# jac0626/Neighbor-Aware-Reinforcement-Learning-Fosters-Cooperation-in-Spatial-Public-Goods-Games-

Hardware: NVIDIA B200
Metric: site-updates/s (higher is better)
Workload: dtype f32

## Files before the change

### neighbor-aware-reinforcement-learning-fosters-cooperation-in-spatial-public-goods-games-_b200/csrc/spgg_capi.cu

```cuda
#include "../../include/spgg.h"
#include "spgg_kernels.cuh"
#include "spgg_dispatch.h"
#include "spgg_fast.cuh"
#include "spgg_resident.cuh"

#include <cudaTypedefs.h>

#include <algorithm>
#include <cmath>
#include <cstdarg>
#include <cstdio>
#include <cstdlib>
#include <cstring>
#include <string>
#include <vector>

using namespace spgg;

static thread_local std::string g_err;

static int fail(int code, const char *fmt, ...) {
  char buf[512];
  va_list ap;
  va_start(ap, fmt);
  vsnprintf(buf, sizeof(buf), fmt, ap);
  va_end(ap);
  g_err = buf;
  return code;
}

#define CUDA_TRY(expr)                                                                  \
  do {                                                                                  \
    cudaError_t e_ = (expr);                                                            \
    if (e_ != cudaSuccess)                                                              \
      return fail(SPGG_E_CUDA, "%s failed: %s (%s:%d)", #expr, cudaGetErrorString(e_),  \
                  __FILE__, __LINE__);                                                  \
  } while (0)


struct spgg_handle {
  int device = 0;
  int n_rep = 1;
  int mode = MODE_F32_I8;
  int M = 1;
  int action = 0;
  std::vector<spgg_params_t> params;
  std::vector<RepConst> rc_host;
  Geom g{};
  int threads = 256;
  int gmax_ctas = 1;
  size_t smem_step = 0, smem_gmax = 0;
  RepConst *d_rc = nullptr;
  double *d_valtab = nullptr;
  bool lean = false;
  int gmax_ctas_gen = 1;
  void *d_Qb[2] = {nullptr, nullptr};
  int qcur = 0;
  void *Qcur() const { return d_Qb[qcur]; }
  bool spec = false;
  bool carry_valid = false;
  float *d_gcarry = nullptr;
  int *d_bad = nullptr;
  CUtensorMap qmaps[2];
  bool spec_on = true;
  long long spec_launches = 0, spec_failures = 0;
  long long spec_iterations = 0;
  bool in_rerun = false;
  float *d_gvec = nullptr;
  void *peer_code[2][2] = {{nullptr, nullptr}, {nullptr, nullptr}};
  void *peer_R[2][2] = {{nullptr, nullptr}, {nullptr, nullptr}};
  uint32_t *peer_S[2][2] = {{nullptr, nullptr}, {nullptr, nullptr}};
  int peer_rows[2] = {0, 0};
  bool peer_on = false;
  std::vector<void *> ipc_opened;
  unsigned *d_ring = nullptr;
  unsigned *ring_peer[SPGG_MAX_RING] = {nullptr};
  int ring_world = 0;
  int gen = 0;
  int last_gen = -1;
  int last_rel = -1, last_upd = 0, last_spec = 0, last_sel = 0;
  int pend_qcur0 = 0;
  std::vector<char> pend_cur_after, pend_q_after;
  void *d_R[2] = {nullptr, nullptr};
  void *d_code[2] = {nullptr, nullptr};
  uint32_t *d_S[2] = {nullptr, nullptr};
  int cur = 0;
  void *d_gmax = nullptr;
  double *d_stats = nullptr;
  double *d_partials = nullptr;
  unsigned *d_tickets = nullptr;
  int *d_stop = nullptr;
  double *d_eps = nullptr;
  uint32_t *d_thr = nullptr;
  int cap = 0;
  double *d_u = nullptr;
  uint8_t *d_b = nullptr;
  uint8_t *d_sc_S = nullptr;
  double *d_sc_R = nullptr, *d_sc_Q = nullptr;
  unsigned long long *d_sc_info = nullptr;
  bool fast = false;
  bool r_wide = false;
  FastMaps fmaps[2];
  bool resident = false;
  ResGeom rgeo{};
  size_t smem_res = 0;
  bool pend_resident = false;
  bool res_grid = false;
  unsigned char *d_gimg = nullptr;
  double *d_gpart = nullptr;
  unsigned *d_gnsel = nullptr;
  int gnsel_cap = 0;
  std::vector<double> eps_host;
  std::vector<uint32_t> thr_host;
  int replay_pairs = 1;
  long long replay_first = 0, replay_n = 0;
  long long iter = 0;
  std::vector<double> eps_cur;
  std::vector<long long> stop_at;
  std::vector<char> stale;
  long long launches = 0;
  bool pending = false;
  long long pend_t0 = 0;
  int pend_n = 0, pend_cur0 = 0, pend_rel = 0;
  cudaStream_t pend_stream = nullptr;
  CclScratch ccl;
  bool ccl_valid = false;
  int64_t ccl_n = 0;
  size_t elem_code() const { return mode == MODE_F64 ? 4 : 1; }
  size_t elem_R() const { return mode == MODE_F64 ? 8 : (mode == MODE_F32_F ? 4 : 1); }
  size_t elem_Q() const { return mode == MODE_F64 ? 8 : 4; }
  size_t elem_val() const { return mode == MODE_F64 ? 8 : 4; }
  int nq() const { return params[0].algorithm == SPGG_ALGO_DOUBLE_QLEARNING ? 8 : 4; }
};

static bool int8_quantum(const spgg_params_t &p, double *rq, int *gi, int *li, int *mn, int *mx) {
  for (int k = 0; k <= 4; ++k) {
    const double s = (double)(1 << k);
    const double a = p.rep_gain_C * s, b = p.delta_R_D * s, c = p.R_min * s, d = p.R_max * s;
    if (a == std::floor(a) && b == std::floor(b) && c == std::floor(c) && d == std::floor(d) &&
        std::fabs(c) <= 127 && std::fabs(d) <= 127 && std::fabs(a) <= 127 && std::fabs(b) <= 127 &&
        c - b >= -128 && d + a <= 127) {
      *rq = 1.0 / s; *gi = (int)a; *li = (int)b; *mn = (int)c; *mx = (int)d;
      return true;
    }
  }
  return false;
}

static void build_repconst(const spgg_params_t &p, RepConst *rc) {
  memset(rc, 0, sizeof(*rc));
  rc->rc = p.r * p.c;
  for (int n = 0; n < 6; ++n) rc->g[n] = rc->rc * (double)n / 5.0;
  rc->cost = p.cost;
  rc->lo = p.r - 5.0;
  rc->span = 4.0 * p.r - rc->lo;
  rc->wP = p.wP;
  rc->wR = 1.0 - p.wP;
  rc->alpha = p.alpha; rc->gamma = p.gamma; rc->kappa = p.kappa; rc->leps = p.lambda_eps;
  rc->gainC = p.rep_gain_C; rc->lossD = p.delta_R_D; rc->rmin = p.R_min; rc->rmax = p.R_max;
  rc->alpha_f = (float)p.alpha; rc->gamma_f = (float)p.gamma; rc->kappa_f = (float)p.kappa;
  rc->leps_f = (float)p.lambda_eps;
  rc->gainC_f = (float)p.rep_gain_C; rc->lossD_f = (float)p.delta_R_D;
  rc->rmin_f = (float)p.R_min; rc->rmax_f = (float)p.R_max;
  rc->rq = 1.0;
  int8_quantum(p, &rc->rq, &rc->gain_i, &rc->loss_i, &rc->rmin_i, &rc->rmax_i);
  rc->seed_lo = (uint32_t)p.seed;
  rc->seed_hi = (uint32_t)(p.seed >> 32);
  for (uint32_t r = 0; r < 10; ++r) {
    rc->pkeys[2 * r] = rc->seed_lo + r * 0x9E3779B9u;
    rc->pkeys[2 * r + 1] = rc->seed_hi + r * 0xBB67AE85u;
  }
  rc->has_ratio = (rc->wR != 0.0);
  for (int code = 0; code < 128; ++code) {
    const int sn = code >> 2, C = (code >> 1) & 1, coop = code & 1;
    const double tot = rc->rc * (double)sn / 5.0 - (C ? 5.0 * p.cost : 0.0);
    const double P = (tot - rc->lo) / rc->span;
    const double rew = rc->wP * P + rc->wR * (coop ? 0.5 : 0.0);
    rc->rewtab[code] = (float)rew;
    rc->ratiotab[code] =
        coop ? (float)(std::fabs(rc->wR * 0.5) / (std::fabs(rew) + 1e-9) * 100.0) : 0.0f;
  }
}

static size_t step_smem(int mode, int TR) {
  switch (mode) {
    case MODE_F32_I8: return SmemLayout<ModeF32I8>(TR).total;
    case MODE_F32_F: return SmemLayout<ModeF32F>(TR).total;
    default: return SmemLayout<ModeF64>(TR).total;
  }
}

template <class... KArgsT, class... Args>
static cudaError_t launch_pdl(void (*kern)(KArgsT...), int grid, int block, size_t smem, cudaStream_t st,
                              Args... args) {
  static const bool use_pdl = getenv("SPGG_NO_PDL") == nullptr;
  cudaLaunchConfig_t cfg = {};
  cfg.gridDim = dim3((unsigned)grid);
  cfg.blockDim = dim3((unsigned)block);
  cfg.dynamicSmemBytes = smem;
  cfg.stream = st;
  cudaLaunchAttribute attr[1];
  attr[0].id = cudaLaunchAttributeProgrammaticStreamSerialization;
  attr[0].val.programmaticStreamSerializationAllowed = 1;
  cfg.attrs = attr;
  cfg.numAttrs = use_pdl ? 1 : 0;
  return cudaLaunchKernelEx(&cfg, kern, args...);
}

typedef void (*fast_fn_t)(const FastMaps, KArgs);
template <int M, bool ACTION, bool PART>
static fast_fn_t pick_fast3(int upd, int sel) {
  if (upd) return sel ? k_step_fast<M, ACTION, true, true, PART> : k_step_fast<M, ACTION, true, false, PART>;
  return k_step_fast<M, ACTION, false, true, PART>;
}
template <int M, bool ACTION>
static fast_fn_t pick_fast2(int upd, int sel, bool part) {
  return part ? pick_fast3<M, ACTION, true>(upd, sel) : pick_fast3<M, ACTION, false>(upd, sel);
}
static fast_fn_t pick_fast(int M, int action, int upd, int sel, bool part) {
  if (M == 2) return action ? pick_fast2<2, true>(upd, sel, part) : pick_fast2<2, false>(upd, sel, part);
  return action ? pick_fast2<1, true>(upd, sel, part) : pick_fast2<1, false>(upd, sel, part);
}
static size_t fast_smem(int M) { return M == 2 ? FastSmem<2>::kTotal : FastSmem<1>::kTotal; }
typedef void (*gfast_fn_t)(const CUtensorMap, GArgs);
static gfast_fn_t pick_gfast(int M) { return M == 2 ? k_gmax_fast<2> : k_gmax_fast<1>; }
static size_t gfast_smem(int M) { return M == 2 ? GmaxSmem<2>::kTotal : GmaxSmem<1>::kTotal; }

typedef void (*res_fn_t)(RArgs);
template <bool FULL>
static res_fn_t pick_res2(int M, int action) {
  if (M == 2) return action ? k_resident<2, true, FULL> : k_resident<2, false, FULL>;
  return action ? k_resident<1, true, FULL> : k_resident<1, false, FULL>;
}
static res_fn_t pick_res(int M, int action, int L) {
  return (L % 4 == 0) ? pick_res2<true>(M, action) : pick_res2<false>(M, action);
}
template <bool FULL>
static res_fn_t pick_resg2(int M, int action) {
  if (M == 2) return action ? k_resident<2, true, FULL, true> : k_resident<2, false, FULL, true>;
  return action ? k_resident<1, true, FULL, true> : k_resident<1, false, FULL, true>;
}
static res_fn_t pick_res_grid(int M, int action, int L) {
  return (L % 4 == 0) ? pick_resg2<true>(M, action) : pick_resg2<false>(M, action);
}
static ResGeom resident_geom(int L, int cs, size_t smem_limit, int grid = 0) {
  ResGeom rg{};
  rg.grid = grid;
  if (L < 2 * cs) cs = 1;
  rg.rows_max = (L + cs - 1) / cs;
  rg.prow = rg.rows_max + 4;
  rg.QR = (L + 3) / 4;
  rg.pitch = (RG + rg.QR * 4 + RG + 15) / 16 * 16;
  const int quads = rg.rows_max * rg.QR;
  int max_thr = RES_THREADS;
  if (const char *e = getenv("SPGG_RES_THREADS")) max_thr = std::max(64, std::min(RES_THREADS, atoi(e) / 32 * 32));
  rg.threads = std::max(64, std::min(max_thr, (quads + 31) / 32 * 32));
  rg.CS = (ResSmem(rg).total <= smem_limit) ? cs : 0;
  return rg;
}

static int make_map(CUtensorMap *map, void *base, uint64_t row_bytes, uint64_t n_rows, uint64_t n_rep,
                    uint64_t rep_stride_bytes, uint32_t box_bytes, uint32_t box_rows, uint64_t visible_bytes = 0) {
  static PFN_cuTensorMapEncodeTiled_v12000 encode = nullptr;
  if (!encode) {
    void *fn = nullptr;
    cudaDriverEntryPointQueryResult q;
    CUDA_TRY(cudaGetDriverEntryPoint("cuTensorMapEncodeTiled", &fn, cudaEnableDefault, &q));
    if (!fn || q != cudaDriverEntryPointSuccess) return fail(SPGG_E_CUDA, "cuTensorMapEncodeTiled not available");
    encode = (PFN_cuTensorMapEncodeTiled_v12000)fn;
  }
  const cuuint64_t dims[3] = {visible_bytes ? visible_bytes : row_bytes, n_rows, n_rep};
  const cuuint64_t strides[2] = {row_bytes, rep_stride_bytes};
  const cuuint32_t box[3] = {box_bytes, box_rows, 1};
  const cuuint32_t estr[3] = {1, 1, 1};
  CUresult r = encode(map, CU_TENSOR_MAP_DATA_TYPE_UINT8, 3, base, dims, strides, box, estr,
                      CU_TENSOR_MAP_INTERLEAVE_NONE, CU_TENSOR_MAP_SWIZZLE_NONE,
                      CU_TENSOR_MAP_L2_PROMOTION_L2_128B, CU_TENSOR_MAP_FLOAT_OOB_FILL_NONE);
  if (r != CUDA_SUCCESS) return fail(SPGG_E_CUDA, "cuTensorMapEncodeTiled failed (%d)", (int)r);
  return SPGG_OK;
}

static int make_map_q(CUtensorMap *map, void *base, uint64_t L, uint64_t n_rows, uint64_t n_rep) {
  static PFN_cuTensorMapEncodeTiled_v12000 encode = nullptr;
  if (!encode) {
    void *fn = nullptr;
    cudaDriverEntryPointQueryResult q;
    CUDA_TRY(cudaGetDriverEntryPoint("cuTensorMapEncodeTiled", &fn, cudaEnableDefault, &q));
    if (!fn || q != cudaDriverEntryPointSuccess) return fail(SPGG_E_CUDA, "cuTensorMapEncodeTiled not available");
    encode = (PFN_cuTensorMapEncodeTiled_v12000)fn;
  }
  const cuuint64_t dims[4] = {128, L / 8, n_rows, n_rep};
  const cuuint64_t strides[3] = {128, L * 16, n_rows * L * 16};
  const cuuint32_t box[4] = {128, TC / 8, (cuuint32_t)FastSmem<1>::kRowsPerWarp, 1};
  const cuuint32_t estr[4] = {1, 1, 1, 1};
  CUresult r = encode(map, CU_TENSOR_MAP_DATA_TYPE_UINT8, 4, base, dims, strides, box, estr,
                      CU_TENSOR_MAP_INTERLEAVE_NONE, CU_TENSOR_MAP_SWIZZLE_128B,
                      CU_TENSOR_MAP_L2_PROMOTION_L2_128B, CU_TENSOR_MAP_FLOAT_OOB_FILL_NONE);
  if (r != CUDA_SUCCESS) return fail(SPGG_E_CUDA, "cuTensorMapEncodeTiled (Q) failed (%d)", (int)r);
  return SPGG_OK;
}

extern "C" int spgg_abi_version(void) { return SPGG_ABI_VERSION; }
extern "C" const char *spgg_last_error(void) { return g_err.c_str(); }

static int free_all(spgg_handle *h) {
  for (void *p : h->ipc_opened) cudaIpcCloseMemHandle(p);
  h->ipc_opened.clear();
  cudaFree(h->d_rc); cudaFree(h->d_valtab); cudaFree(h->d_Qb[0]); cudaFree(h->d_Qb[1]); cudaFree(h->d_gcarry); cudaFree(h->d_bad); cudaFree(h->d_gvec); cudaFree(h->d_ring);
  for (int i = 0; i < 2; ++i) { cudaFree(h->d_R[i]); cudaFree(h->d_code[i]); cudaFree(h->d_S[i]); }
  cudaFree(h->d_gmax); cudaFree(h->d_stats); cudaFree(h->d_partials); cudaFree(h->d_tickets);
  cudaFree(h->d_stop); cudaFree(h->d_eps); cudaFree(h->d_thr); cudaFree(h->d_u); cudaFree(h->d_b);
  cudaFree(h->d_sc_S); cudaFree(h->d_sc_R); cudaFree(h->d_sc_Q); cudaFree(h->d_sc_info);
  cudaFree(h->d_gimg); cudaFree(h->d_gpart); cudaFree(h->d_gnsel);
  ccl_free(&h->ccl);
  return 0;
}

extern "C" void spgg_destroy(spgg_t *h) {
  if (!h) return;
  cudaSetDevice(h->device);
  cudaDeviceSynchronize();
  free_all(h);
  delete h;
}

extern "C" int spgg_create(const spgg_params_t *params, int n_replicas, int device, spgg_t **out) {
  if (!params || !out || n_replicas < 1) return fail(SPGG_E_INVALID, "spgg_create: null argument or n_replicas < 1");
  const spgg_params_t &p0 = params[0];
  if (p0.L < 4) return fail(SPGG_E_INVALID, "L must be >= 4 (got %d)", p0.L);
  if (p0.rows < 2 * GH || p0.rows > p0.L)
    return fail(SPGG_E_INVALID, "rows must be in [%d, L] (got %d)", 2 * GH, p0.rows);
  if (p0.M != 1 && p0.M != 2) return fail(SPGG_E_INVALID, "M must be 1 or 2 (got %d)", p0.M);
  if (p0.state_mode != SPGG_STATE_REPUTATION && p0.state_mode != SPGG_STATE_ACTION)
    return fail(SPGG_E_INVALID, "Unknown state_representation code %d", p0.state_mode);
  if (p0.precision != SPGG_PREC_FP32 && p0.precision != SPGG_PREC_FP64)
    return fail(SPGG_E_INVALID, "unknown precision %d", p0.precision);
  if (p0.algorithm != SPGG_ALGO_QLEARNING && p0.algorithm != SPGG_ALGO_SARSA &&
      p0.algorithm != SPGG_ALGO_EXPECTED_SARSA && p0.algorithm != SPGG_ALGO_DOUBLE_QLEARNING)
    return fail(SPGG_E_UNSUPPORTED, "algorithm code %d is not built into the fused kernel", p0.algorithm);
  if (p0.row0 < 0 || p0.row0 + p0.rows > p0.L) return fail(SPGG_E_INVALID, "row0/rows outside the lattice");
  for (int r = 1; r < n_replicas; ++r) {
    const spgg_params_t &p = params[r];
    if (p.L != p0.L || p.rows != p0.rows || p.row0 != p0.row0 || p.M != p0.M ||
        p.state_mode != p0.state_mode || p.precision != p0.precision ||
        p.algorithm != p0.algorithm || p.r_storage != p0.r_storage)
      return fail(SPGG_E_INVALID, "replica %d differs in a batch-invariant field (L, rows, M, state, precision)", r);
  }
  int ndev = 0;
  CUDA_TRY(cudaGetDeviceCount(&ndev));
  if (device < 0 || device >= ndev) return fail(SPGG_E_CUDA, "device %d not available (%d devices)", device, ndev);
  CUDA_TRY(cudaSetDevice(device));

  spgg_handle *h = new spgg_handle();
  h->device = device;
  h->n_rep = n_replicas;
  h->params.assign(params, params + n_replicas);
  h->M = p0.M;
  h->action = p0.state_mode == SPGG_STATE_ACTION;
  h->rc_host.resize(n_replicas);
  bool all_i8 = true;
  for (int r = 0; r < n_replicas; ++r) {
    build_repconst(params[r], &h->rc_host[r]);
    double rq; int a, b, c, d;
    all_i8 = all_i8 && int8_quantum(params[r], &rq, &a, &b, &c, &d);
  }
  if (p0.precision == SPGG_PREC_FP64) h->mode = MODE_F64;
  else if (p0.r_storage == SPGG_RSTORE_FP32) h->mode = MODE_F32_F;
  else if (p0.r_storage == SPGG_RSTORE_INT8) {
    if (!all_i8) { delete h; return fail(SPGG_E_INVALID, "reputation parameters are not representable in int8 units"); }
    h->mode = MODE_F32_I8;
  } else h->mode = all_i8 ? MODE_F32_I8 : MODE_F32_F;

  Geom &g = h->g;
  g.L = p0.L; g.rows = p0.rows; g.row0 = p0.row0; g.wrap_rows = (p0.rows == p0.L);
  g.pitchB = CPAD + (p0.L + 15) / 16 * 16 + CPAD;
  g.pitchW = WPAD + ((p0.L + 31) / 32 + 3) / 4 * 4 + WPAD;
  {
    const RepConst &r0 = h->rc_host[0];
    bool ok = (h->mode == MODE_F32_I8) && (g.L % 32 == 0) && (g.L >= TC) && (g.rows % FTR == 0) &&
              p0.algorithm == SPGG_ALGO_QLEARNING && getenv("SPGG_NO_FAST") == nullptr;
    for (int r = 0; r < n_replicas && ok; ++r)
      ok = h->rc_host[r].rmin_i >= -15 && h->rc_host[r].rmax_i <= 15 && h->rc_host[r].gain_i >= 0 &&
           h->rc_host[r].loss_i >= 0;
    (void)r0;
    h->fast = ok;
  }
  {
    cudaDeviceProp prop0;
    CUDA_TRY(cudaGetDeviceProperties(&prop0, device));
    res_fn_t rf = pick_res(h->M, h->action, h->g.L);
    cudaFuncAttributes fa;
    CUDA_TRY(cudaFuncGetAttributes(&fa, rf));
    const size_t lim = prop0.sharedMemPerBlockOptin - fa.sharedSizeBytes - 1024;
    const bool eligible = (h->mode == MODE_F32_I8) && g.wrap_rows && p0.row0 == 0 &&
                          p0.algorithm == SPGG_ALGO_QLEARNING && getenv("SPGG_NO_RESIDENT") == nullptr;
    ResGeom rg = resident_geom(g.L, 8, lim);
    if (eligible && g.L >= 32 && (rg.CS == 0 || n_replicas <= 4 || getenv("SPGG_RES_CS16") != nullptr) &&
        getenv("SPGG_RES_CS8") == nullptr) {
      const ResGeom rg16 = resident_geom(g.L, 16, lim);
      if (rg16.CS == 16 &&
          cudaFuncSetAttribute(rf, cudaFuncAttributeNonPortableClusterSizeAllowed, 1) == cudaSuccess &&
          cudaFuncSetAttribute(rf, cudaFuncAttributeMaxDynamicSharedMemorySize, (int)lim) == cudaSuccess) {
        cudaLaunchConfig_t cfg = {};
        cfg.gridDim = dim3(16u * (unsigned)n_replicas);
        cfg.blockDim = dim3((unsigned)rg16.threads);
        cfg.dynamicSmemBytes = ResSmem(rg16).total;
        cudaLaunchAttribute attr[1];
        attr[0].id = cudaLaunchAttributeClusterDimension;
        attr[0].val.clusterDim.x = 16; attr[0].val.clusterDim.y = 1; attr[0].val.clusterDim.z = 1;
        cfg.attrs = attr; cfg.numAttrs = 1;
        int n_clusters = 0;
        if (cudaOccupancyMaxActiveClusters(&n_clusters, rf, &cfg) == cudaSuccess && n_clusters >= 1) rg = rg16;
      }
      (void)cudaGetLastError();
    }
    h->resident = eligible && rg.CS > 0;
    if (h->resident) {
      h->rgeo = rg;
      h->smem_res = ResSmem(rg).total;
      CUDA_TRY(cudaFuncSetAttribute(rf, cudaFuncAttributeMaxDynamicSharedMemorySize, (int)lim));
    } else if (eligible && n_replicas == 1 && getenv("SPGG_NO_RESIDENT_GRID") == nullptr) {
      res_fn_t gf = pick_res_grid(h->M, h->action, h->g.L);
      cudaFuncAttributes gfa;
      CUDA_TRY(cudaFuncGetAttributes(&gfa, gf));
      const size_t glim = prop0.sharedMemPerBlockOptin - gfa.sharedSizeBytes - 1024;
      int coop = 0;
      CUDA_TRY(cudaDeviceGetAttribute(&coop, cudaDevAttrCooperativeLaunch, device));
      const int nb_ctas = std::min(prop0.multiProcessorCount, g.L / 2);
      ResGeom gg = resident_geom(g.L, nb_ctas, glim, 1);
      if (coop && nb_ctas >= RES_RING && gg.CS == nb_ctas &&
          cudaFuncSetAttribute(gf, cudaFuncAttributeMaxDynamicSharedMemorySize, (int)glim) == cudaSuccess) {
        int occ_g = 0;
        if (cudaOccupancyMaxActiveBlocksPerMultiprocessor(&occ_g, gf, gg.threads, ResSmem(gg).total) == cudaSuccess &&
            (long long)occ_g * prop0.multiProcessorCount >= nb_ctas) {
          h->resident = true;
          h->res_grid = true;
          h->rgeo = gg;
          h->smem_res = ResSmem(gg).total;
        }
      }
      (void)cudaGetLastError();
    }
  }
  g.TR = h->fast ? FTR : (g.rows >= 512 ? 16 : (g.rows >= 64 ? 8 : 4));
  h->threads = h->fast ? FTHREADS : 32 * std::min(8, g.TR);
  if (!h->fast && getenv("SPGG_GEN_TR") && getenv("SPGG_GEN_THREADS")) {
    g.TR = std::max(4, std::min(16, atoi(getenv("SPGG_GEN_TR"))));
    h->threads = std::max(32, std::min(256, atoi(getenv("SPGG_GEN_THREADS")) / 32 * 32));
  }
  g.n_tx = (g.L + TC - 1) / TC;
  g.n_ty = (g.rows + g.TR - 1) / g.TR;
  g.n_rep = n_replicas;
  g.plane_stride = (long long)(g.rows + 2 * GH) * g.pitchB;
  g.bits_stride = (long long)(g.rows + 2 * GH) * g.pitchW;
  g.site_stride = (long long)g.rows * g.L;
  h->smem_step = step_smem(h->mode, g.TR);
  h->smem_gmax = (h->elem_val() * (size_t)(g.TR + 2 * HR) * SMW + 15) / 16 * 16 + 512;

  cudaDeviceProp prop;
  CUDA_TRY(cudaGetDeviceProperties(&prop, device));
  int occ = 1;
  h->lean = !h->fast && p0.algorithm == 0 && getenv("SPGG_NO_LEAN") == nullptr;
  if (h->lean) h->smem_step = step_smem(h->mode, LEAN_TR_MAX);
  for (int replay = 0; replay < 2; ++replay) {
    step_fn_t f = pick_step(h->mode, h->M, h->action, replay);
    CUDA_TRY(cudaFuncSetAttribute(f, cudaFuncAttributeMaxDynamicSharedMemorySize, (int)h->smem_step));
    if (!replay)
      CUDA_TRY(cudaOccupancyMaxActiveBlocksPerMultiprocessor(&occ, f, h->threads, h->smem_step));
    if (h->lean) {
      step_fn_t fl = pick_lean(h->mode, h->M, h->action, replay);
      CUDA_TRY(cudaFuncSetAttribute(fl, cudaFuncAttributeMaxDynamicSharedMemorySize, (int)h->smem_step));
      if (!replay)
        CUDA_TRY(cudaOccupancyMaxActiveBlocksPerMultiprocessor(&occ, fl, h->threads, h->smem_step));
    }
  }
  if (h->fast) {
    for (int v = 0; v < 3; ++v) {
      fast_fn_t fv = pick_fast(h->M, h->action, v != 2, v != 1, g.L % TC != 0);
      CUDA_TRY(cudaFuncSetAttribute(fv, cudaFuncAttributeMaxDynamicSharedMemorySize, (int)fast_smem(h->M)));
    }
    fast_fn_t ff = pick_fast(h->M, h->action, 1, 1, g.L % TC != 0);
    CUDA_TRY(cudaOccupancyMaxActiveBlocksPerMultiprocessor(&occ, ff, FTHREADS, fast_smem(h->M)));
    CUDA_TRY(cudaFuncSetAttribute(pick_gfast(h->M), cudaFuncAttributeMaxDynamicSharedMemorySize, (int)gfast_smem(h->M)));
    int gocc = 1;
    CUDA_TRY(cudaOccupancyMaxActiveBlocksPerMultiprocessor(&gocc, pick_gfast(h->M), GWARPS * 32, gfast_smem(h->M)));
    const long long n_tiles_g = (long long)((p0.L + TC - 1) / TC) * (p0.rows / FTR);
    h->gmax_ctas = (int)std::max<long long>(1, std::min<long long>((n_tiles_g + GWARPS - 1) / GWARPS,
                       ((long long)prop.multiProcessorCount * std::max(1, gocc)) / n_replicas));
  }
  CUDA_TRY(cudaFuncSetAttribute(pick_gmax_lean(h->mode, h->M), cudaFuncAttributeMaxDynamicSharedMemorySize,
                                (int)h->smem_gmax));
  if (occ < 1) { delete h; return fail(SPGG_E_CUDA, "kernel does not fit on an SM (smem %zu)", h->smem_step); }
  const long long n_tiles = (long long)g.n_tx * g.n_ty;
  long long per_rep = std::max<long long>(1, ((long long)prop.multiProcessorCount * occ) / n_replicas);
  g.ctas_per_rep = (int)std::min<long long>(n_tiles, per_rep);
  {
    int gocc = 1;
    CUDA_TRY(cudaOccupancyMaxActiveBlocksPerMultiprocessor(&gocc, pick_gmax_lean(h->mode, h->M), h->threads, h->smem_gmax));
    h->gmax_ctas_gen = (int)std::min<long long>(n_tiles, std::max<long long>(1, ((long long)prop.multiProcessorCount * std::max(1, gocc)) / n_replicas));
  }
  if (h->fast && (g.site_stride / ((long long)g.ctas_per_rep * FTHREADS)) > 60000) h->fast = false;
  h->spec = h->fast && getenv("SPGG_NO_SPEC") == nullptr;

  const size_t nQ = (size_t)n_replicas * g.site_stride * h->nq() * h->elem_Q();
  const size_t nR = (size_t)n_replicas * g.plane_stride * h->elem_R();
  const size_t nC = (size_t)n_replicas * g.plane_stride * h->elem_code();
  const size_t nS = (size_t)n_replicas * g.bits_stride * 4;
#define ALLOC(ptr, bytes)                                                                   \
  do {                                                                                      \
    cudaError_t e_ = cudaMalloc((void **)&(ptr), (bytes));                                  \
    if (e_ != cudaSuccess) {                                                                \
      free_all(h); delete h;                                                                \
      return fail(SPGG_E_CUDA, "cudaMalloc(%zu bytes) failed: %s", (size_t)(bytes), cudaGetErrorString(e_)); \
    }                                                                                       \
    cudaMemset((ptr), 0, (bytes));                                                          \
  } while (0)
  ALLOC(h->d_rc, sizeof(RepConst) * n_replicas);
  ALLOC(h->d_Qb[0], nQ);
  if (h->spec) { ALLOC(h->d_Qb[1], nQ); ALLOC(h->d_gcarry, sizeof(float) * n_replicas); ALLOC(h->d_bad, sizeof(int)); }
  for (int i = 0; i < 2; ++i) { ALLOC(h->d_R[i], nR); ALLOC(h->d_code[i], nC); ALLOC(h->d_S[i], nS); }
  ALLOC(h->d_partials, sizeof(double) * (size_t)n_replicas * g.ctas_per_rep * NSTAT);
  ALLOC(h->d_tickets, sizeof(unsigned) * n_replicas);
  ALLOC(h->d_stop, sizeof(int) * n_replicas);
  if (h->res_grid) {
    ALLOC(h->d_gimg, (size_t)h->rgeo.CS * 6 * h->rgeo.prow * h->rgeo.pitch);
    ALLOC(h->d_gpart, sizeof(double) * (size_t)RES_RING * h->rgeo.CS * RES_NRED);
  }
#undef ALLOC
  if (h->fast) {
    const int rowsCR = FTR + 2 * h->M, rowsS = FTR + 4;
    const uint64_t nrows = (uint64_t)(g.rows + 2 * GH);
    for (int i = 0; i < 2; ++i) {
      FastMaps &fm = h->fmaps[i];
      int e = make_map(&fm.ld_code, h->d_code[i], (uint64_t)g.pitchB, nrows, n_replicas, (uint64_t)g.plane_stride, FROWB, rowsCR);
      if (!e) e = make_map(&fm.ld_R, h->d_R[i], (uint64_t)g.pitchB, nrows, n_replicas, (uint64_t)g.plane_stride, FROWB, rowsCR);
      if (!e) e = make_map(&fm.ld_S, h->d_S[i], (uint64_t)g.pitchW * 4, nrows, n_replicas, (uint64_t)g.bits_stride * 4, FSROWB, rowsS);
      if (!e) e = make_map(&fm.st_code, h->d_code[i ^ 1], (uint64_t)g.pitchB, nrows, n_replicas, (uint64_t)g.plane_stride, TC, FTR, (uint64_t)(CPAD + g.L));
      if (!e) e = make_map(&fm.st_R, h->d_R[i ^ 1], (uint64_t)g.pitchB, nrows, n_replicas, (uint64_t)g.plane_stride, TC, FTR, (uint64_t)(CPAD + g.L));
      if (!e) e = make_map(&fm.st_S, h->d_S[i ^ 1], (uint64_t)g.pitchW * 4, nrows, n_replicas, (uint64_t)g.bits_stride * 4, TC / 8, FTR);
      if (!e) e = make_map_q(&h->qmaps[i], h->d_Qb[(i == 1 && h->spec) ? 1 : 0], (uint64_t)g.L, (uint64_t)g.rows, (uint64_t)n_replicas);
      if (e) { free_all(h); delete h; return e; }
    }
  }
  CUDA_TRY(cudaMemcpy(h->d_rc, h->rc_host.data(), sizeof(RepConst) * n_replicas, cudaMemcpyHostToDevice));
  if (h->mode == MODE_F64) {
    const size_t vb = sizeof(double) * 2 * ((size_t)n_replicas << VALTAB_BITS);
    if (cudaMalloc((void **)&h->d_valtab, vb) != cudaSuccess) {
      free_all(h); delete h;
      return fail(SPGG_E_CUDA, "cudaMalloc(%zu bytes) failed (reward table)", vb);
    }
    CUDA_TRY(launch_build_valtab(h->d_rc, h->d_valtab, n_replicas));
  }
  std::vector<int> neg(n_replicas, -1);
  CUDA_TRY(cudaMemcpy(h->d_stop, neg.data(), sizeof(int) * n_replicas, cudaMemcpyHostToDevice));
  if (h->spec) {
    const int none = 0x7fffffff;
    CUDA_TRY(cudaMemcpy(h->d_bad, &none, sizeof(int), cudaMemcpyHostToDevice));
  }
  h->eps_cur.resize(n_replicas);
  for (int r = 0; r < n_replicas; ++r) h->eps_cur[r] = params[r].epsilon;
  h->stop_at.assign(n_replicas, -1);
  h->stale.assign(n_replicas, 0);
  *out = h;
  return SPGG_OK;
}

static int launch_step(spgg_handle *h, int do_update, int do_select, cudaStream_t st, bool allow_spec);

static int rewind_to_failed_launch(spgg_handle *h, int bad) {
  h->spec_failures += 1;
  if (h->spec_failures > 8 && h->spec_failures * 16 > h->spec_iterations) h->spec_on = false;
  const int none = 0x7fffffff;
  CUDA_TRY(cudaMemcpy(h->d_bad, &none, sizeof(int), cudaMemcpyHostToDevice));
  std::vector<int> stop(h->n_rep);
  CUDA_TRY(cudaMemcpy(stop.data(), h->d_stop, sizeof(int) * h->n_rep, cudaMemcpyDeviceToHost));
  for (int r = 0; r < h->n_rep; ++r)
    if (stop[r] == (int)(h->pend_t0 + bad) + 1) stop[r] = -1;
  CUDA_TRY(cudaMemcpy(h->d_stop, stop.data(), sizeof(int) * h->n_rep, cudaMemcpyHostToDevice));
  h->cur = h->pend_cur_after[bad - 1];
  h->qcur = h->pend_q_after[bad - 1];
  h->carry_valid = true;
  h->pend_rel = bad - 1;
  return SPGG_OK;
}

static int rerun_failed_speculation(spgg_handle *h) {
  for (;;) {
    int bad = 0x7fffffff;
    CUDA_TRY(cudaMemcpy(&bad, h->d_bad, sizeof(int), cudaMemcpyDeviceToHost));
    if (bad == 0x7fffffff) return SPGG_OK;
    if (getenv("SPGG_SPEC_DEBUG")) fprintf(stderr, "[spgg] speculation failed at launch %d of %d (t0 %lld), %lld speculative launches so far\n", bad, h->pend_n, h->pend_t0, h->spec_launches);
    if (bad < 1 || bad > h->pend_n) return fail(SPGG_E_STATE, "speculation bookkeeping out of range (%d of %d)", bad, h->pend_n);
    int rcode0 = rewind_to_failed_launch(h, bad);
    if (rcode0) return rcode0;
    h->in_rerun = true;
    const int n = h->pend_n;
    for (int s = bad; s <= n; ++s) {
      h->pend_rel += 1;
      int rcode = launch_step(h, 1, s < n ? 1 : 0, h->pend_stream, true);
      if (rcode) return rcode;
      if (!h->spec_on && s < n) {
        for (++s; s <= n; ++s) {
          rcode = spgg_phase_gmax(h, h->pend_stream);
          if (!rcode) rcode = launch_step(h, 1, s < n ? 1 : 0, h->pend_stream, false);
          if (rcode) return rcode;
        }
      }
    }
    h->in_rerun = false;
    CUDA_TRY(cudaStreamSynchronize(h->pend_stream));
    CUDA_TRY(cudaGetLastError());
  }
}

static int finish_pending(spgg_handle *h) {
  if (!h->pending) return SPGG_OK;
  CUDA_TRY(cudaSetDevice(h->device));
  CUDA_TRY(cudaStreamSynchronize(h->pend_stream));
  CUDA_TRY(cudaGetLastError());
  if (h->spec && h->g.wrap_rows && h->pend_rel == h->pend_n && !h->pend_resident) {
    int rcode = rerun_failed_speculation(h);
    if (rcode) return rcode;
  }
  std::vector<int> stop(h->n_rep);
  CUDA_TRY(cudaMemcpy(stop.data(), h->d_stop, sizeof(int) * h->n_rep, cudaMemcpyDeviceToHost));
  const long long t_end = h->pend_t0 + h->pend_rel;
  for (int r = 0; r < h->n_rep; ++r) {
    h->stop_at[r] = stop[r];
    const long long done = (stop[r] >= 0 && stop[r] < t_end) ? (long long)stop[r] : t_end;
    double e = h->eps_cur[r];
    for (long long t = h->pend_t0; t < done; ++t)
      e = std::max(e * h->params[r].epsilon_decay, h->params[r].epsilon_min);
    h->eps_cur[r] = e;
  }
  if (h->pend_resident) {
    h->iter = (h->n_rep == 1 && stop[0] >= 0 && stop[0] < t_end) ? (long long)stop[0] : t_end;
    h->pend_resident = false;
  } else if (h->n_rep == 1 && stop[0] >= 0 && stop[0] < t_end) {
    h->cur = h->pend_cur0 ^ (int)((stop[0] - h->pend_t0) & 1);
    h->qcur = h->pend_q_after[(size_t)(stop[0] - h->pend_t0)];
    h->iter = stop[0];
  } else {
    if (h->n_rep > 1) {
      for (int r = 0; r < h->n_rep; ++r) {
        if (stop[r] >= 0 && stop[r] < t_end) {
          const long long k = (long long)stop[r] - h->pend_t0;
          const int src = k >= 0 ? (h->pend_cur0 ^ (int)(k & 1)) : h->pend_cur0;
          if (src != h->cur) {
            const Geom &g = h->g;
            CUDA_TRY(cudaMemcpy((char *)h->d_R[h->cur] + (size_t)r * g.plane_stride * h->elem_R(),
                                (char *)h->d_R[src] + (size_t)r * g.plane_stride * h->elem_R(),
                                (size_t)g.plane_stride * h->elem_R(), cudaMemcpyDeviceToDevice));
            CUDA_TRY(cudaMemcpy(h->d_S[h->cur] + (size_t)r * g.bits_stride,
                                h->d_S[src] + (size_t)r * g.bits_stride,
                                (size_t)g.bits_stride * 4, cudaMemcpyDeviceToDevice));
          }
          const int qsrc = k >= 0 ? h->pend_q_after[(size_t)k] : h->pend_qcur0;
          if (qsrc != h->qcur) {
            const size_t qb = (size_t)h->g.site_stride * h->nq() * h->elem_Q();
            CUDA_TRY(cudaMemcpy((char *)h->d_Qb[h->qcur] + (size_t)r * qb, (char *)h->d_Qb[qsrc] + (size_t)r * qb, qb,
                                cudaMemcpyDeviceToDevice));
          }
        }
      }
    }
    h->iter = t_end;
  }
  h->pending = false;
  return SPGG_OK;
}

extern "C" int spgg_sync(spgg_t *h) {
  if (!h) return fail(SPGG_E_INVALID, "null handle");
  return finish_pending(h);
}

static int stage_rows(const spgg_handle *h) {
  const long long budget = 32ll << 20;
  return (int)std::max<long long>(1, std::min<long long>(h->g.rows, budget / h->g.L));
}

static int ensure_scratch(spgg_handle *h, bool want_q) {
  const size_t n = (size_t)stage_rows(h) * h->g.L;
  if (!h->d_sc_S) {
    CUDA_TRY(cudaMalloc((void **)&h->d_sc_S, n));
    CUDA_TRY(cudaMalloc((void **)&h->d_sc_R, n * sizeof(double)));
    CUDA_TRY(cudaMalloc((void **)&h->d_sc_info, 3 * sizeof(unsigned long long)));
  }
  if (want_q && !h->d_sc_Q) CUDA_TRY(cudaMalloc((void **)&h->d_sc_Q, n * h->nq() * sizeof(double)));
  return SPGG_OK;
}

static void begin_new_run(spgg_handle *h, int rep) {
  if (h->iter != 0) {
    h->iter = 0;
    std::fill(h->stale.begin(), h->stale.end(), 1);
  }
  h->stale[rep] = 0;
  h->carry_valid = false;
  if (h->d_ring) {
    cudaMemset(h->d_ring, 0, sizeof(unsigned) * RING_SLOTS * RING_WORDS);
    h->gen = 0;
    h->last_gen = -1;
  }
}

extern "C" int spgg_set_state(spgg_t *h, int rep, const uint8_t *S, const double *R, const double *Q) {
  if (!h || !S || !R || !Q) return fail(SPGG_E_INVALID, "spgg_set_state: null argument");
  if (rep < 0 || rep >= h->n_rep) return fail(SPGG_E_INVALID, "replica %d out of range", rep);
  int rcode = finish_pending(h);
  if (rcode) return rcode;
  h->ccl_valid = false;
  CUDA_TRY(cudaSetDevice(h->device));
  rcode = ensure_scratch(h, true);
  if (rcode) return rcode;
  const Geom &g = h->g;
  const RepConst &rc = h->rc_host[rep];
  CUDA_TRY(cudaMemset(h->d_sc_info, 0, 3 * sizeof(unsigned long long)));
  const int chunk = stage_rows(h);
  for (int i0 = 0; i0 < g.rows; i0 += chunk) {
    const int nr = std::min(chunk, g.rows - i0);
    const size_t n = (size_t)nr * g.L, off = (size_t)i0 * g.L;
    CUDA_TRY(cudaMemcpyAsync(h->d_sc_S, S + off, n, cudaMemcpyHostToDevice, 0));
    CUDA_TRY(cudaMemcpyAsync(h->d_sc_R, R + off, n * sizeof(double), cudaMemcpyHostToDevice, 0));
    CUDA_TRY(cudaMemcpyAsync(h->d_sc_Q, Q + off * h->nq(), n * h->nq() * sizeof(double), cudaMemcpyHostToDevice, 0));
    const int grid = (int)std::min<long long>(148 * 16, ((long long)nr * ((g.L + 31) / 32) * 32 + 255) / 256);
#define IMPORT(Md) k_import_rows<Md><<<std::max(1, grid), 256>>>(g, rep, i0, nr, h->d_sc_S, h->d_sc_R, h->d_sc_Q, \
                       h->Qcur(), h->d_R[h->cur], h->d_S[h->cur], rc.rq, h->d_sc_info, h->nq())
    if (h->mode == MODE_F32_I8) IMPORT(ModeF32I8);
    else if (h->mode == MODE_F32_F) IMPORT(ModeF32F);
    else IMPORT(ModeF64);
#undef IMPORT
    CUDA_TRY(cudaGetLastError());
    h->launches += 1;
  }
  unsigned long long info[3];
  CUDA_TRY(cudaMemcpy(info, h->d_sc_info, sizeof(info), cudaMemcpyDeviceToHost));
  if (info[0] == 1) return fail(SPGG_E_INVALID, "strategy array holds values other than 0/1");
  if (info[0] == 2)
    return fail(SPGG_E_INVALID, "R is not representable in int8 units of %g; use r_storage=FP32", rc.rq);
  if (info[2] && h->fast) {
    if (!g.wrap_rows)
      return fail(SPGG_E_INVALID, "R outside [%g, %g] (int8 units -16..15 of %g): a strip on the fast path "
                  "cannot hold it", -16.0 * rc.rq, 15.0 * rc.rq, rc.rq);
    h->r_wide = true;
  }
  begin_new_run(h, rep);
  h->eps_cur[rep] = h->params[rep].epsilon;
  int stop = -1;
  if (g.wrap_rows && (info[1] == 0 || info[1] == (unsigned long long)g.site_stride))
    stop = (int)h->iter;
  h->stop_at[rep] = stop;
  CUDA_TRY(cudaMemcpy(h->d_stop + rep, &stop, sizeof(int), cudaMemcpyHostToDevice));
  return SPGG_OK;
}

extern "C" int spgg_get_state(spgg_t *h, int rep, uint8_t *S, double *R, double *Q) {
  if (!h) return fail(SPGG_E_INVALID, "null handle");
  if (rep < 0 || rep >= h->n_rep) return fail(SPGG_E_INVALID, "replica %d out of range", rep);
  int rcode = finish_pending(h);
  if (rcode) return rcode;
  CUDA_TRY(cudaSetDevice(h->device));
  rcode = ensure_scratch(h, Q != nullptr);
  if (rcode) return rcode;
  const Geom &g = h->g;
  const RepConst &rc = h->rc_host[rep];
  const int chunk = stage_rows(h);
  for (int i0 = 0; i0 < g.rows; i0 += chunk) {
    const int nr = std::min(chunk, g.rows - i0);
    const size_t n = (size_t)nr * g.L, off = (size_t)i0 * g.L;
    const int grid = (int)std::min<long long>(148 * 16, ((long long)n + 255) / 256);
#define EXPORT(Md) k_export_rows<Md><<<std::max(1, grid), 256>>>(g, rep, i0, nr, S ? h->d_sc_S : nullptr, \
                       R ? h->d_sc_R : nullptr, Q ? h->d_sc_Q : nullptr, h->Qcur(), h->d_R[h->cur], h->d_S[h->cur], rc.rq, h->nq())
    if (h->mode == MODE_F32_I8) EXPORT(ModeF32I8);
    else if (h->mode == MODE_F32_F) EXPORT(ModeF32F);
    else EXPORT(ModeF64);
#undef EXPORT
    CUDA_TRY(cudaGetLastError());
    h->launches += 1;
    if (S) CUDA_TRY(cudaMemcpyAsync(S + off, h->d_sc_S, n, cudaMemcpyDeviceToHost, 0));
    if (R) CUDA_TRY(cudaMemcpyAsync(R + off, h->d_sc_R, n * sizeof(double), cudaMemcpyDeviceToHost, 0));
    if (Q) CUDA_TRY(cudaMemcpyAsync(Q + off * h->nq(), h->d_sc_Q, n * h->nq() * sizeof(double), cudaMemcpyDeviceToHost, 0));
    CUDA_TRY(cudaStreamSynchronize(0));
  }
  return SPGG_OK;
}

extern "C" int spgg_set_replay(spgg_t *h, int n_steps, const double *u, const uint8_t *b) {
  return spgg_set_replay_pairs(h, n_steps, 1, u, b);
}

extern "C" int spgg_set_replay_pairs(spgg_t *h, int n_steps, int n_pairs, const double *u, const uint8_t *b) {
  if (!h) return fail(SPGG_E_INVALID, "null handle");
  const int want_pairs = h->params[0].algorithm == SPGG_ALGO_SARSA ? 3
                         : (h->params[0].algorithm == SPGG_ALGO_DOUBLE_QLEARNING ? 2 : 1);
  if (n_steps > 0 && n_pairs != want_pairs)
    return fail(SPGG_E_INVALID, "this TD rule consumes %d draw pair(s) per iteration, got %d", want_pairs, n_pairs);
  if (h->n_rep != 1) return fail(SPGG_E_UNSUPPORTED, "replay draws are supported for a single replica");
  int rcode = finish_pending(h);
  if (rcode) return rcode;
  CUDA_TRY(cudaSetDevice(h->device));
  cudaFree(h->d_u); cudaFree(h->d_b);
  h->d_u = nullptr; h->d_b = nullptr; h->replay_n = 0;
  if (n_steps <= 0) return SPGG_OK;
  if (!u || !b) return fail(SPGG_E_INVALID, "spgg_set_replay: null draw arrays");
  const size_t n = (size_t)n_steps * n_pairs * h->g.site_stride;
  h->replay_pairs = n_pairs;
  CUDA_TRY(cudaMalloc((void **)&h->d_u, n * sizeof(double)));
  CUDA_TRY(cudaMalloc((void **)&h->d_b, n));
  CUDA_TRY(cudaMemcpy(h->d_u, u, n * sizeof(double), cudaMemcpyHostToDevice));
  CUDA_TRY(cudaMemcpy(h->d_b, b, n, cudaMemcpyHostToDevice));
  h->replay_first = h->iter;
// ... 711 lines not shown
```

### neighbor-aware-reinforcement-learning-fosters-cooperation-in-spatial-public-goods-games-_b200/csrc/spgg_fast.cuh

```cuda
#pragma once
#include <cuda.h>

#include "spgg_kernels.cuh"

namespace spgg {

#ifndef SPGG_FTR
#define SPGG_FTR 16
#endif
#ifndef SPGG_FTHREADS
#define SPGG_FTHREADS 256
#endif
constexpr int FTR = SPGG_FTR;
constexpr int FROWB = 160;
constexpr int FROWW = FROWB / 4;
constexpr int FSROWB = 48;
constexpr int FTHREADS = SPGG_FTHREADS;

template <int M>
struct FastSmem {
  static constexpr int kRowsCR = FTR + 2 * M;
  static constexpr int kRowsS = FTR + 4;
  static constexpr int kStageCode = 0;
  static constexpr int kStageR = (kRowsCR * FROWB + 127) / 128 * 128;
  static constexpr int kStageS = kStageR + (kRowsCR * FROWB + 127) / 128 * 128;
  static constexpr int kStageBytes = kStageS + (kRowsS * FSROWB + 127) / 128 * 128;
  static constexpr int kTxBytes = 2 * kRowsCR * FROWB + kRowsS * FSROWB;
  static constexpr int kOutCode = 2 * kStageBytes;
  static constexpr int kOutR = kOutCode + FTR * TC;
  static constexpr int kOutS = kOutR + FTR * TC;
  static constexpr int kOffC = kOutS + 256 + FROWB;
  static constexpr int kOffVal = kOffC + (FTR + 4) * FROWB + FROWB;
  static constexpr int kOffTab = kOffVal + kRowsCR * FROWB * 4;
  static constexpr int kOffBar = kOffTab + 256 * 4;
  static constexpr int kOffFlag = kOffBar + 40 * 8;
  static constexpr int kOffRc = kOffFlag + 16;
  static constexpr int kOffRed = (kOffRc + (int)sizeof(RepConst) + 127) / 128 * 128;
  static constexpr int kRowsPerWarp = FTR / (FTHREADS / 32);
  static constexpr int kQBufs = 2;
  static constexpr int kQBufBytes = kRowsPerWarp * TC * 16;
  static constexpr int kOffQ = (kOffRed + 8 * NSTAT * 8 + 1023) / 1024 * 1024;
  static constexpr int kTotal = kOffQ + (FTHREADS / 32) * kQBufs * kQBufBytes + 1024;
};

__device__ __forceinline__ uint32_t smem_u32(const void *p) {
  return (uint32_t)__cvta_generic_to_shared(p);
}
__device__ __forceinline__ void mbar_init(uint64_t *bar, uint32_t count) {
  asm volatile("mbarrier.init.shared::cta.b64 [%0], %1;" ::"r"(smem_u32(bar)), "r"(count));
}
__device__ __forceinline__ void mbar_expect_tx(uint64_t *bar, uint32_t bytes) {
  asm volatile("mbarrier.arrive.expect_tx.shared::cta.b64 _, [%0], %1;" ::"r"(smem_u32(bar)), "r"(bytes)
               : "memory");
}
__device__ __forceinline__ void mbar_wait(uint64_t *bar, uint32_t parity) {
  uint32_t done;
  uint32_t spins = 0;
  do {
    asm volatile(
        "{\n"
        ".reg .pred p;\n"
        "mbarrier.try_wait.parity.shared::cta.b64 p, [%1], %2;\n"
        "selp.u32 %0, 1, 0, p;\n"
        "}\n"
        : "=r"(done)
        : "r"(smem_u32(bar)), "r"(parity)
        : "memory");
    if (!done && ++spins > (1u << 28)) __trap();
  } while (!done);
}
__device__ __forceinline__ void tma_load_3d(void *dst, const CUtensorMap *map, uint64_t *bar, int c0,
                                            int c1, int c2) {
  asm volatile(
      "cp.async.bulk.tensor.3d.shared::cluster.global.mbarrier::complete_tx::bytes [%0], [%1, {%3, %4, %5}], [%2];"
      ::"r"(smem_u32(dst)), "l"(map), "r"(smem_u32(bar)), "r"(c0), "r"(c1), "r"(c2)
      : "memory");
}

__device__ __forceinline__ void bulk_load_1d(void *dst, const void *src, uint32_t bytes, uint64_t *bar) {
  asm volatile(
      "cp.async.bulk.shared::cluster.global.mbarrier::complete_tx::bytes [%0], [%1], %2, [%3];"
      ::"r"(smem_u32(dst)), "l"(src), "r"(bytes), "r"(smem_u32(bar))
      : "memory");
}
__device__ __forceinline__ void tma_store_3d(const CUtensorMap *map, const void *src, int c0, int c1, int c2) {
  asm volatile("cp.async.bulk.tensor.3d.global.shared::cta.bulk_group [%0, {%2, %3, %4}], [%1];"
               ::"l"(map), "r"(smem_u32(src)), "r"(c0), "r"(c1), "r"(c2)
               : "memory");
}
__device__ __forceinline__ uint64_t l2_evict_first_policy() {
  uint64_t pol;
  asm volatile("createpolicy.fractional.L2::evict_first.b64 %0, 1.0;" : "=l"(pol));
  return pol;
}
__device__ __forceinline__ void tma_load_4d_hint(void *dst, const CUtensorMap *map, uint64_t *bar, int c0,
                                                 int c1, int c2, int c3, uint64_t pol) {
  asm volatile(
      "cp.async.bulk.tensor.4d.shared::cluster.global.mbarrier::complete_tx::bytes.L2::cache_hint"
      " [%0], [%1, {%3, %4, %5, %6}], [%2], %7;"
      ::"r"(smem_u32(dst)), "l"(map), "r"(smem_u32(bar)), "r"(c0), "r"(c1), "r"(c2), "r"(c3), "l"(pol)
      : "memory");
}
__device__ __forceinline__ void tma_store_4d_hint(const CUtensorMap *map, const void *src, int c0, int c1,
                                                  int c2, int c3, uint64_t pol) {
  asm volatile(
      "cp.async.bulk.tensor.4d.global.shared::cta.bulk_group.L2::cache_hint [%0, {%2, %3, %4, %5}], [%1], %6;"
      ::"l"(map), "r"(smem_u32(src)), "r"(c0), "r"(c1), "r"(c2), "r"(c3), "l"(pol)
      : "memory");
}
template <int N>
__device__ __forceinline__ void tma_store_wait_read_n() {
  asm volatile("cp.async.bulk.wait_group.read %0;" ::"n"(N) : "memory");
}
__device__ __forceinline__ void tma_store_commit() { asm volatile("cp.async.bulk.commit_group;" ::: "memory"); }
__device__ __forceinline__ void tma_store_wait_read() { asm volatile("cp.async.bulk.wait_group.read 0;" ::: "memory"); }
__device__ __forceinline__ void tma_store_wait_all() { asm volatile("cp.async.bulk.wait_group 0;" ::: "memory"); }
__device__ __forceinline__ void fence_proxy_async() { asm volatile("fence.proxy.async.shared::cta;" ::: "memory"); }

__device__ __forceinline__ uint32_t sh_l1(uint32_t prev, uint32_t cur) { return __byte_perm(prev, cur, 0x6543); }
__device__ __forceinline__ uint32_t sh_r1(uint32_t cur, uint32_t next) { return __byte_perm(cur, next, 0x4321); }
__device__ __forceinline__ uint32_t sh_2(uint32_t a, uint32_t b) { return __byte_perm(a, b, 0x5432); }

struct FastMaps {
  CUtensorMap ld_code, ld_R, ld_S;
  CUtensorMap st_code, st_R, st_S;
  CUtensorMap q_ld, q_st;
};

#ifndef SPGG_FAST_MINBLOCKS
#define SPGG_FAST_MINBLOCKS 2
#endif
template <int M, bool ACTION, bool UPD, bool SEL, bool PART = false>
__device__ __forceinline__ void step_fast_body(const FastMaps &tm, const KArgs &a) {
  typedef FastSmem<M> SM;
  constexpr int NK = (M == 2) ? 12 : 4;
  constexpr bool upd = UPD, sel = SEL;
  const Geom &g = a.g;
  const int rep = blockIdx.x / g.ctas_per_rep, cta = blockIdx.x % g.ctas_per_rep;

  extern __shared__ __align__(1024) unsigned char smem_fast[];
  unsigned char *smem = smem_fast + ((1024u - (smem_u32(smem_fast) & 1023u)) & 1023u);
  uint32_t *wC = reinterpret_cast<uint32_t *>(smem + SM::kOffC);
  float *sm_val = reinterpret_cast<float *>(smem + SM::kOffVal);
  float *sm_tab = reinterpret_cast<float *>(smem + SM::kOffTab);
  float *sm_ratio = sm_tab + 128;
  double *sm_red = reinterpret_cast<double *>(smem + SM::kOffRed);
  uint64_t *bars = reinterpret_cast<uint64_t *>(smem + SM::kOffBar);
  uint8_t *out_code = smem + SM::kOutCode;
  int8_t *out_R = reinterpret_cast<int8_t *>(smem + SM::kOutR);
  uint32_t *out_S = reinterpret_cast<uint32_t *>(smem + SM::kOutS);
  RepConst &s_rc = *reinterpret_cast<RepConst *>(smem + SM::kOffRc);
  int &s_is_last = *reinterpret_cast<int *>(smem + SM::kOffFlag);

  const int tid = threadIdx.x, lane = tid & 31, warp = tid >> 5;
#ifdef SPGG_TRACE
  unsigned long long t_start = 0;
  if (tid == 0) asm volatile("mov.u64 %0, %%globaltimer;" : "=l"(t_start));
#endif
  for (int i = tid; i < (int)(sizeof(RepConst) / 4); i += FTHREADS)
    reinterpret_cast<uint32_t *>(&s_rc)[i] = reinterpret_cast<const uint32_t *>(a.rc + rep)[i];
  if (tid == 0) {
    mbar_init(&bars[0], 1);
    mbar_init(&bars[1], 1);
    asm volatile("fence.mbarrier_init.release.cluster;" ::: "memory");
  }
  __syncthreads();
  for (int i = tid; i < 128; i += FTHREADS) {
    sm_tab[i] = s_rc.rewtab[i];
    sm_ratio[i] = s_rc.ratiotab[i];
  }
  const RepConst &rc = s_rc;

  float4 *Qp = reinterpret_cast<float4 *>(a.Q) + (long long)rep * g.site_stride;

  float inv_den = 0.f, gm_used = 0.f;
  if (upd) {
    gm_used = a.spec ? a.gcarry[rep] : reinterpret_cast<const float *>(a.gmax)[(long long)rep * a.cap + a.rel];
    if (a.spec == 2) gm_used = 123.0f;
    inv_den = __fdiv_rn(1.0f, __fadd_rn(gm_used, rc.leps_f));
  }
  float gbest = 0.f;
  const uint32_t thr = sel ? a.thr_tab[(long long)(a.rel + 1) * g.n_rep + rep] : 0u;
  const float alpha = rc.alpha_f, gamma = rc.gamma_f, kappa = rc.kappa_f;
  const int g31 = min(rc.gain_i, 31), l31 = min(rc.loss_i, 31);
  const uint32_t r_dsum = (uint32_t)(g31 + l31);
  const uint32_t r_k = (uint32_t)(32 - l31) * 0x01010101u;
  const uint32_t r_lo = (uint32_t)(rc.rmin_i + 48) * 0x01010101u, r_hi = (uint32_t)(rc.rmax_i + 48) * 0x01010101u;
  const bool has_ratio = rc.has_ratio != 0;

  uint32_t cls_n[4] = {0, 0, 0, 0}, cls_sn[4] = {0, 0, 0, 0};
  uint32_t grp[6] = {0, 0, 0, 0, 0, 0};
  uint32_t pk_best = 0;
  uint32_t n_sel = 0;
  int sum_r = 0;
  float sq0 = 0.f, sq1 = 0.f, sq2 = 0.f, sq3 = 0.f, sc0 = 0.f, sc1 = 0.f, sc2 = 0.f, sc3 = 0.f;
  float s_ni = 0.f, s_ratio = 0.f;

  const int n_tiles = g.n_tx * g.n_ty;
  const int d_ty = g.ctas_per_rep / g.n_tx, d_tx = g.ctas_per_rep - d_ty * g.n_tx;
  const int d_skew = (d_tx + d_ty) % g.n_tx;
  auto issue = [&](int ty_, int tx_, int st) {
    const int r0 = ty_ * FTR, c0 = tx_ * TC;
    unsigned char *base = smem + st * SM::kStageBytes;
    mbar_expect_tx(&bars[st], SM::kTxBytes);
    tma_load_3d(base + SM::kStageCode, &tm.ld_code, &bars[st], c0, r0 + GH - M, rep);
    tma_load_3d(base + SM::kStageR, &tm.ld_R, &bars[st], c0, r0 + GH - M, rep);
    tma_load_3d(base + SM::kStageS, &tm.ld_S, &bars[st], c0 >> 3, r0 + GH - 2, rep);
  };
  int ty = cta / g.n_tx, txs = cta - ty * g.n_tx;
  int tx = (txs + ty) % g.n_tx;
  if (tid == 0 && cta < n_tiles) issue(ty, tx, 0);

  uint64_t *qbar = bars + 2 + warp * SM::kQBufs;
  unsigned char *sQ = smem + SM::kOffQ + warp * (SM::kQBufs * SM::kQBufBytes);
  const uint64_t pol = l2_evict_first_policy();
  if (lane == 0) {
#pragma unroll
    for (int b = 0; b < SM::kQBufs; ++b) mbar_init(&qbar[b], 1);
    asm volatile("fence.mbarrier_init.release.cluster;" ::: "memory");
  }
  __syncwarp();
  auto q_issue = [&](int col8, int row, int buf) {
    mbar_expect_tx(&qbar[buf], SM::kQBufBytes);
    tma_load_4d_hint(sQ + buf * SM::kQBufBytes, &tm.q_ld, &qbar[buf], 0, col8, row, rep, pol);
  };
  int qoff[4];
#pragma unroll
  for (int k = 0; k < 4; ++k)
    qoff[k] = (lane >> 1) * 128 + ((((lane & 1) * 4 + k) ^ ((lane >> 1) & 7)) << 4);
  if (lane == 0 && cta < n_tiles) q_issue((tx * TC) >> 3, ty * FTR + warp * SM::kRowsPerWarp, 0);

  int tiles_done = 0, stage = 0;
  for (int tile = cta; tile < n_tiles; tile += g.ctas_per_rep, ++tiles_done, stage ^= 1) {
    const int r0 = ty * FTR, c0 = tx * TC;
    int nty = ty + d_ty, ntxs = txs + d_tx, ntx = tx + d_skew;
    if (ntxs >= g.n_tx) { ntxs -= g.n_tx; ++nty; ++ntx; }
    if (ntx >= g.n_tx) ntx -= g.n_tx;
    const bool has_next = tile + g.ctas_per_rep < n_tiles;
    if (tid == 0) {
      if (has_next) issue(nty, ntx, stage ^ 1);
      if (sel) tma_store_wait_read();
    }
    mbar_wait(&bars[stage], (uint32_t)(tiles_done >> 1) & 1u);
    const bool lv = !PART || (c0 + 4 * lane < g.L);
    const uint32_t vm = lv ? 0x01010101u : 0u;
    const unsigned char *st_base = smem + stage * SM::kStageBytes;
    const uint32_t *st_code = reinterpret_cast<const uint32_t *>(st_base + SM::kStageCode);
    const uint32_t *st_R = reinterpret_cast<const uint32_t *>(st_base + SM::kStageR);
    const uint32_t *st_S = reinterpret_cast<const uint32_t *>(st_base + SM::kStageS);

    const int t1 = tid - (FTHREADS - 128);
    if (t1 >= 0 && t1 < (FTR + 4) * 6) {
      const int row = t1 / 6, bw = t1 - row * 6 + 3;
      const uint32_t bits = ~st_S[row * (FSROWB / 4) + bw];
      uint32_t *dst = wC + row * FROWW + (bw - 4) * 8 + 4;
      if (bw == 3) {
        dst[7] = ((bits >> 28) * 0x00204081u) & 0x01010101u;
      } else if (bw == 8) {
        dst[0] = ((bits & 0xFu) * 0x00204081u) & 0x01010101u;
      } else {
        uint4 lo, hi;
        lo.x = (((bits >> 0) & 0xFu) * 0x00204081u) & 0x01010101u;
        lo.y = (((bits >> 4) & 0xFu) * 0x00204081u) & 0x01010101u;
        lo.z = (((bits >> 8) & 0xFu) * 0x00204081u) & 0x01010101u;
        lo.w = (((bits >> 12) & 0xFu) * 0x00204081u) & 0x01010101u;
        hi.x = (((bits >> 16) & 0xFu) * 0x00204081u) & 0x01010101u;
        hi.y = (((bits >> 20) & 0xFu) * 0x00204081u) & 0x01010101u;
        hi.z = (((bits >> 24) & 0xFu) * 0x00204081u) & 0x01010101u;
        hi.w = ((bits >> 28) * 0x00204081u) & 0x01010101u;
        *reinterpret_cast<uint4 *>(dst) = lo;
        *reinterpret_cast<uint4 *>(dst + 4) = hi;
      }
    }
    if (upd) {
      for (int e = tid; e < SM::kRowsCR * FROWW; e += FTHREADS) {
        const uint32_t cw = st_code[e];
        float4 v;
        v.x = sm_tab[(cw >> 1) & 0x7Fu];
        v.y = sm_tab[(cw >> 9) & 0x7Fu];
        v.z = sm_tab[(cw >> 17) & 0x7Fu];
        v.w = sm_tab[(cw >> 25) & 0x7Fu];
        *reinterpret_cast<float4 *>(sm_val + e * 4) = v;
      }
    }
    if (upd) {
      const int t2 = tid - 64;
      if (t2 >= 0 && t2 < FTR * 4 && (!PART || (c0 >> 5) + (t2 & 3) < ((g.L + 31) >> 5))) {
        const int row = (t2 >> 2) + 2, bw = (t2 & 3) + 4;
        const uint32_t *bp = st_S + row * (FSROWB / 4) + bw;
        const uint32_t c = bp[0], u = bp[-(FSROWB / 4)], d = bp[FSROWB / 4];
        const uint32_t l = (c << 1) | (bp[-1] >> 31), r = (c >> 1) | (bp[1] << 31);
        const uint32_t s1 = c ^ u ^ d, c1 = (c & u) | (d & (c | u));
        const uint32_t b0 = s1 ^ l ^ r, c2 = (s1 & l) | (r & (s1 | l));
        const uint32_t b1 = c1 ^ c2, b2 = c1 & c2;
        grp[0] += __popc(~b0 & ~b1 & ~b2); grp[1] += __popc(b0 & ~b1 & ~b2);
        grp[2] += __popc(~b0 & b1 & ~b2);  grp[3] += __popc(b0 & b1 & ~b2);
        grp[4] += __popc(~b0 & ~b1 & b2);  grp[5] += __popc(b0 & ~b1 & b2);
      }
    }
    __syncthreads();
    const uint8_t *bCode = reinterpret_cast<const uint8_t *>(st_code);
    const int qb = stage;
    __syncwarp();
    if (lane == 0) {
      if (upd) tma_store_wait_read_n<0>();
      if (has_next) q_issue((ntx * TC) >> 3, nty * FTR + warp * SM::kRowsPerWarp, qb ^ 1);
    }
    mbar_wait(&qbar[qb], (uint32_t)(tiles_done >> 1) & 1u);
#pragma unroll
    for (int r2 = 0; r2 < SM::kRowsPerWarp; ++r2) {
      const int rr = warp * SM::kRowsPerWarp + r2;
      uint32_t w4[4] = {0, 0, 0, 0};
      if (sel) {
        philox4x32_10_keys((uint32_t)((c0 >> 2) + lane), (uint32_t)(g.row0 + r0 + rr),
                           (uint32_t)(a.j + 1), 0u, s_rc.pkeys, w4);
      }
      const int wo = rr * FROWW + (CPAD / 4) + lane;
      const uint32_t RW = st_R[wo + M * FROWW];
      const uint32_t CW = wC[wo + 2 * FROWW];
      uint32_t StW;
      if constexpr (ACTION) {
        StW = CW;
      } else {
        const uint32_t *rp = st_R + wo + M * FROWW;
        auto bias = [](uint32_t x) { return (x ^ 0x10101010u) & 0x1F1F1F1Fu; };
        const uint32_t c = bias(RW), l = bias(rp[-1]), r = bias(rp[1]);
        const uint32_t u1 = bias(rp[-FROWW]), d1 = bias(rp[FROWW]);
        uint32_t sumA = c + u1 + d1 + sh_l1(l, c) + sh_r1(c, r);
        if constexpr (M == 1) {
          StW = ((sumA + 0x2F2F2F2Fu) >> 7) & 0x01010101u;
        } else {
          const uint32_t ul = bias(rp[-FROWW - 1]), ur = bias(rp[-FROWW + 1]);
          const uint32_t dl = bias(rp[FROWW - 1]), dr = bias(rp[FROWW + 1]);
          const uint32_t sumB = bias(rp[-2 * FROWW]) + bias(rp[2 * FROWW]) + sh_2(l, c) + sh_2(c, r) +
                                sh_l1(ul, u1) + sh_r1(u1, ur) + sh_l1(dl, d1);
          sumA += sh_r1(d1, dr);
          const uint32_t lo = (sumA & 0x00FF00FFu) + (sumB & 0x00FF00FFu);
          const uint32_t hi = ((sumA >> 8) & 0x00FF00FFu) + ((sumB >> 8) & 0x00FF00FFu);
          const uint32_t flo = ((lo + (0x8000u - 209u) * 0x00010001u) >> 15) & 0x00010001u;
          const uint32_t fhi = ((hi + (0x8000u - 209u) * 0x00010001u) >> 15) & 0x00010001u;
          StW = flo | (fhi << 8);
        }
      }
      sum_r = __dp4a((int)RW, (int)vm, sum_r);
      uint32_t codeW = 0;
      float vc[4], vu[4], vd[4], vl[2], vr[2], vu2[4], vd2[4], vul = 0.f, vur = 0.f, vdl = 0.f, vdr = 0.f;
      const int vb = (rr + M) * FROWB + CPAD + 4 * lane;
      if (upd) {
        codeW = st_code[wo + M * FROWW];
        {
          const uint32_t Cb = (codeW >> 2) & 0x01010101u, Ab = (codeW >> 1) & 0x01010101u;
          const uint32_t m3 = Cb & Ab & vm, m2 = (Cb & vm) ^ m3, m1 = (Ab & vm) ^ m3, m0 = vm & ~(Cb | Ab);
          const uint32_t sn = (codeW >> 3) & 0x1F1F1F1Fu;
          cls_n[0] = __dp4a(m0, 0x01010101u, cls_n[0]); cls_sn[0] = __dp4a(sn, m0, cls_sn[0]);
          cls_n[1] = __dp4a(m1, 0x01010101u, cls_n[1]); cls_sn[1] = __dp4a(sn, m1, cls_sn[1]);
          cls_n[2] = __dp4a(m2, 0x01010101u, cls_n[2]); cls_sn[2] = __dp4a(sn, m2, cls_sn[2]);
          cls_n[3] = __dp4a(m3, 0x01010101u, cls_n[3]); cls_sn[3] = __dp4a(sn, m3, cls_sn[3]);
        }
        const float4 c4 = *reinterpret_cast<const float4 *>(sm_val + vb);
        const float4 u4 = *reinterpret_cast<const float4 *>(sm_val + vb - FROWB);
        const float4 d4 = *reinterpret_cast<const float4 *>(sm_val + vb + FROWB);
        vc[0] = c4.x; vc[1] = c4.y; vc[2] = c4.z; vc[3] = c4.w;
        vu[0] = u4.x; vu[1] = u4.y; vu[2] = u4.z; vu[3] = u4.w;
        vd[0] = d4.x; vd[1] = d4.y; vd[2] = d4.z; vd[3] = d4.w;
        if constexpr (M == 2) {
          const float2 l2 = *reinterpret_cast<const float2 *>(sm_val + vb - 2);
          const float2 r2 = *reinterpret_cast<const float2 *>(sm_val + vb + 4);
          vl[0] = l2.x; vl[1] = l2.y; vr[0] = r2.x; vr[1] = r2.y;
          const float4 uu = *reinterpret_cast<const float4 *>(sm_val + vb - 2 * FROWB);
          const float4 dd = *reinterpret_cast<const float4 *>(sm_val + vb + 2 * FROWB);
          vu2[0] = uu.x; vu2[1] = uu.y; vu2[2] = uu.z; vu2[3] = uu.w;
          vd2[0] = dd.x; vd2[1] = dd.y; vd2[2] = dd.z; vd2[3] = dd.w;
          vul = sm_val[vb - FROWB - 1]; vur = sm_val[vb - FROWB + 4];
          vdl = sm_val[vb + FROWB - 1]; vdr = sm_val[vb + FROWB + 4];
        } else {
          vl[0] = 0.f; vl[1] = sm_val[vb - 1]; vr[0] = sm_val[vb + 4]; vr[1] = 0.f;
        }
      }
      unsigned char *qbuf = sQ + qb * SM::kQBufBytes + r2 * (TC * 16);
      uint32_t coopW = 0, rnewW = 0;
      float qfin[4];
      int eidx[4];
      const uint32_t rowoffW = StW << 3;
      const uint32_t coopCW = (codeW >> 1) & 0x01010101u;
      const uint32_t hitW = ~(StW ^ codeW) & 0x01010101u;
      const uint32_t hitCW = hitW & coopCW, hitDW = hitW ^ hitCW;
      if (upd) {
        float qe[4], na[4], nb_[4];
        const uint32_t eoffW = ((codeW & 0x01010101u) << 3) | ((((codeW >> 1) & 0x01010101u) ^ 0x01010101u) << 2);
#pragma unroll
        for (int k = 0; k < 4; ++k) {
          const unsigned char *qs = qbuf + qoff[k];
          eidx[k] = (int)__byte_perm(eoffW, 0, 0x4440 + k);
          qe[k] = *reinterpret_cast<const float *>(qs + eidx[k]);
          const float2 nrow = *reinterpret_cast<const float2 *>(qs + __byte_perm(rowoffW, 0, 0x4440 + k));
          na[k] = nrow.x; nb_[k] = nrow.y;
        }
#pragma unroll
        for (int k = 0; k < 4; ++k) {
          const uint32_t code = (codeW >> (8 * k)) & 0xFFu;
          const float vx = vc[k];
          float nv[NK];
          int no[NK];
          nv[0] = vu[k]; no[0] = -FROWB;
          nv[1] = vd[k]; no[1] = FROWB;
          nv[2] = (k == 0) ? vl[1] : vc[(k + 3) & 3]; no[2] = -1;
          nv[3] = (k == 3) ? vr[0] : vc[(k + 1) & 3]; no[3] = 1;
          if constexpr (M == 2) {
            nv[4] = vu2[k]; no[4] = -2 * FROWB;
            nv[5] = vd2[k]; no[5] = 2 * FROWB;
            nv[6] = (k == 0) ? vl[0] : (k == 1) ? vl[1] : vc[(k + 2) & 3]; no[6] = -2;
            nv[7] = (k == 2) ? vr[0] : (k == 3) ? vr[1] : vc[(k + 2) & 3]; no[7] = 2;
            nv[8] = (k == 0) ? vul : vu[(k + 3) & 3]; no[8] = -FROWB - 1;
            nv[9] = (k == 3) ? vur : vu[(k + 1) & 3]; no[9] = -FROWB + 1;
            nv[10] = (k == 0) ? vdl : vd[(k + 3) & 3]; no[10] = FROWB - 1;
            nv[11] = (k == 3) ? vdr : vd[(k + 1) & 3]; no[11] = FROWB + 1;
          }
          float best = __fsub_rn(nv[0], vx);
          int boff = no[0];
          bool second = false;
#pragma unroll
          for (int q = 1; q < NK; ++q) {
            const float d = __fsub_rn(nv[q], vx);
            if (d > best) { best = d; boff = no[q]; if constexpr (M == 2) second = (q >= 4); }
          }
          if (lv) gbest = fmaxf(gbest, best);
          const bool same = ((((uint32_t)bCode[vb + k + boff] ^ code) >> 1) & 1u) == 0u;
          const float td = __fsub_rn(__fmaf_rn(gamma, fmaxf(na[k], nb_[k]), vx), qe[k]);
          const float qtd = __fmaf_rn(alpha, td, qe[k]);
          const float lam = __fmul_rn(__fmul_rn(kappa, fmaxf(0.0f, best)), inv_den);
          const float nu = same ? lam : -lam;
          const float na2 = ((hitCW >> (8 * k)) & 1u) ? qtd : na[k];
          const float nb2 = ((hitDW >> (8 * k)) & 1u) ? qtd : nb_[k];
          const float td2 = __fsub_rn(__fmaf_rn(gamma, fmaxf(na2, nb2), vx), qtd);
          qfin[k] = __fadd_rn(qtd, nu);
          const float an = fabsf(nu);
          if (lv) {
            s_ni += __fdividef(an, fabsf(alpha * td2) + an + 1e-8f);
            if (has_ratio) s_ratio += sm_ratio[code >> 1];
            if (best > 0.f) pk_best += second ? 0x10001u : 1u;
          }
        }
#pragma unroll
        for (int k = 0; k < 4; ++k) *reinterpret_cast<float *>(qbuf + qoff[k] + eidx[k]) = qfin[k];
#pragma unroll
        for (int k = 0; k < 4; ++k) {
          const float4 qn = *reinterpret_cast<const float4 *>(qbuf + qoff[k]);
          const float m = ((codeW >> (8 * k + 2)) & 1u) ? 1.0f : 0.0f;
          if (lv) {
            sq0 += qn.x; sq1 += qn.y; sq2 += qn.z; sq3 += qn.w;
            sc0 = fmaf(m, qn.x, sc0); sc1 = fmaf(m, qn.y, sc1); sc2 = fmaf(m, qn.z, sc2); sc3 = fmaf(m, qn.w, sc3);
          }
        }
      }
      if (sel) {
#pragma unroll
        for (int k = 0; k < 4; ++k) {
          const float2 grow = *reinterpret_cast<const float2 *>(
              qbuf + qoff[k] + __byte_perm(rowoffW, 0, 0x4440 + k));
          const bool explore = (w4[k] >> 8) < thr;
          const int rnd = (int)(w4[k] & 1u);
          const int greedy = (grow.y > grow.x) ? 1 : 0;
          const int a_new = explore ? rnd : greedy;
          coopW |= (uint32_t)(a_new ^ 1) << (8 * k);
        }
        uint32_t x = ((RW ^ 0x10101010u) & 0x1F1F1F1Fu) + coopW * r_dsum + r_k;
        uint32_t m = ((((x | 0x80808080u) - r_lo) >> 7) & 0x01010101u) * 0xFFu;
        x = (x & m) | (r_lo & ~m);
        m = ((((r_hi | 0x80808080u) - x) >> 7) & 0x01010101u) * 0xFFu;
        x = (x & m) | (r_hi & ~m);
        rnewW = (x + 0x50505050u) ^ 0x80808080u;
      }
      if (sel) {
        const uint32_t *cp = wC + wo + 2 * FROWW;
        const uint32_t cl = cp[-1], cr = cp[1];
        const uint32_t u1 = cp[-FROWW], ul = cp[-FROWW - 1], ur = cp[-FROWW + 1];
        const uint32_t d1 = cp[FROWW], dl = cp[FROWW - 1], dr = cp[FROWW + 1];
        const uint32_t ring = u1 + d1 + sh_l1(cl, CW) + sh_r1(CW, cr) + sh_l1(ul, u1) + sh_r1(u1, ur) +
                              sh_l1(dl, d1) + sh_r1(d1, dr);
        const uint32_t far4 = cp[-2 * FROWW] + cp[2 * FROWW] + sh_2(cl, CW) + sh_2(CW, cr);
        const uint32_t SNW = 5u * CW + 2u * ring + far4;
        const int oo = rr * (TC / 4) + lane;
        reinterpret_cast<uint32_t *>(out_code)[oo] = (SNW << 3) | (CW << 2) | (coopW << 1) | StW;
        reinterpret_cast<uint32_t *>(out_R)[oo] = rnewW;
        const uint32_t nib = lv ? (((coopW * 0x01020408u) >> 24) & 0xFu) : 0u;
        uint32_t coopbits = nib << ((lane & 7) * 4);
        coopbits |= __shfl_xor_sync(0xffffffffu, coopbits, 1);
        coopbits |= __shfl_xor_sync(0xffffffffu, coopbits, 2);
        coopbits |= __shfl_xor_sync(0xffffffffu, coopbits, 4);
        if ((lane & 7) == 0) {
          out_S[rr * 4 + (lane >> 3)] = ~coopbits;
          n_sel += __popc(coopbits);
        }
      }
    }
    if (upd) {
      fence_proxy_async();
      __syncwarp();
      if (lane == 0) {
        tma_store_4d_hint(&tm.q_st, sQ + qb * SM::kQBufBytes, 0, c0 >> 3, r0 + warp * SM::kRowsPerWarp, rep, pol);
        tma_store_commit();
      }
    }
    if (sel) fence_proxy_async();
    __syncthreads();
    if (sel) {
      if (tid == 0) {
        tma_store_3d(&tm.st_code, out_code, CPAD + c0, r0 + GH, rep);
        tma_store_3d(&tm.st_R, out_R, CPAD + c0, r0 + GH, rep);
        if (!PART || c0 + TC <= g.L) tma_store_3d(&tm.st_S, out_S, (WPAD * 4) + (c0 >> 3), r0 + GH, rep);
        tma_store_commit();
      }
      const bool ecol0 = tx == 0, ecol1 = tx == g.n_tx - 1;
      const bool erow0 = g.wrap_rows && ty == 0, erow1 = g.wrap_rows && ty == g.n_ty - 1;
      const bool prow0 = a.peer_code[0] != nullptr && ty == 0, prow1 = a.peer_code[1] != nullptr && ty == g.n_ty - 1;
      const bool edge = ecol0 || ecol1 || erow0 || erow1 || prow0 || prow1;
      if (edge) {
        uint8_t *code_out = reinterpret_cast<uint8_t *>(a.code_out) + (long long)rep * g.plane_stride;
        int8_t *R_out = reinterpret_cast<int8_t *>(a.R_out) + (long long)rep * g.plane_stride;
        uint32_t *S_out = a.S_out + (long long)rep * g.bits_stride;
        for (int e = tid; e < 2 * FTR * GC + 2 * GH * TC; e += FTHREADS) {
          int rr, cc;
          bool on, peer = false;
          int side = 0;
          if (e < 2 * FTR * GC) {
            side = e >= FTR * GC;
            const int q = side ? e - FTR * GC : e;
            rr = q / GC;
            const int wl = PART ? min(TC, g.L - c0) : TC;
            cc = side ? wl - GC + (q % GC) : q % GC;
            on = side ? ecol1 : ecol0;
          } else {
            const int q0 = e - 2 * FTR * GC;
            side = q0 >= GH * TC;
            const int q = side ? q0 - GH * TC : q0;
            rr = side ? FTR - GH + q / TC : q / TC;
            cc = q % TC;
            const bool exists = !PART || c0 + cc < g.L;
            on = exists && (side ? erow1 : erow0);
            peer = exists && (side ? prow1 : prow0);
          }
          const int o = rr * TC + cc;
          if (on) {
            store_cell<uint8_t>(code_out, g, r0 + rr, c0 + cc, out_code[o]);
            store_cell<int8_t>(R_out, g, r0 + rr, c0 + cc, out_R[o]);
          }
          if (peer) {
            const int pi = side ? (rr - FTR) : (a.peer_rows[0] + rr);
            store_cell<uint8_t>(reinterpret_cast<uint8_t *>(a.peer_code[side]), g, pi, c0 + cc, out_code[o]);
            store_cell<int8_t>(reinterpret_cast<int8_t *>(a.peer_R[side]), g, pi, c0 + cc, out_R[o]);
          }
        }
        for (int e = tid; e < FTR * 4; e += FTHREADS) {
          const int rr = e >> 2, wi = (c0 >> 5) + (e & 3);
          if (PART && wi >= ((g.L + 31) >> 5)) continue;
          if (ecol0 || ecol1 || erow0 || erow1) store_bits_word(S_out, g, r0 + rr, wi, out_S[e]);
          if (prow0 && rr < GH) store_bits_word(a.peer_S[0], g, a.peer_rows[0] + rr, wi, out_S[e]);
          if (prow1 && rr >= FTR - GH) store_bits_word(a.peer_S[1], g, rr - FTR, wi, out_S[e]);
        }
        __syncthreads();
      }
    }
    ty = nty; txs = ntxs; tx = ntx;
  }

#ifdef SPGG_TRACE
  if (tid == 0 && a.trace) {
    unsigned long long t_end; unsigned smid;
    asm volatile("mov.u64 %0, %%globaltimer;" : "=l"(t_end));
    asm volatile("mov.u32 %0, %%smid;" : "=r"(smid));
    unsigned long long *tr = a.trace + (size_t)blockIdx.x * 4;
    tr[0] = t_start; tr[1] = t_end; tr[2] = smid; tr[3] = (unsigned long long)tiles_done;
  }
#endif
  double v[NSTAT];
#pragma unroll
  for (int z = 0; z < NSTAT; ++z) v[z] = 0.0;
  const double n0 = (double)cls_n[0], n1 = (double)cls_n[1], n2 = (double)cls_n[2], n3 = (double)cls_n[3];
  v[ST_NC_OLD] = n2 + n3; v[ST_N_CD] = n2; v[ST_N_DC] = n1; v[ST_NC_NEW] = n1 + n3;
  v[ST_SUM_P] = n0; v[ST_SUM_P_C] = n1; v[ST_SUM_P_D] = n2; v[ST_SUM_WP_P] = n3;
#pragma unroll
  for (int z = 0; z < 4; ++z) v[ST_X_SN0 + z] = (double)cls_sn[z];
  v[ST_SUM_RATIO] = (double)s_ratio;
#pragma unroll
  for (int z = 0; z < 6; ++z) v[ST_GROUP0 + z] = (double)grp[z];
  v[ST_SUM_R] = (double)sum_r;
  v[ST_SUM_Q + 0] = (double)sq0; v[ST_SUM_Q + 1] = (double)sq1; v[ST_SUM_Q + 2] = (double)sq2; v[ST_SUM_Q + 3] = (double)sq3;
  v[ST_SUM_Q_C + 0] = (double)sc0; v[ST_SUM_Q_C + 1] = (double)sc1; v[ST_SUM_Q_C + 2] = (double)sc2; v[ST_SUM_Q_C + 3] = (double)sc3;
  v[ST_SUM_NI] = (double)s_ni * 100.0;
  v[ST_N_BEST_POS] = (double)(pk_best & 0xffffu);
  v[ST_N_BEST_2ND] = (double)(pk_best >> 16);
  v[ST_X_NSEL] = (double)n_sel;
  __syncthreads();
  block_reduce_bfly<NSTAT>(v, sm_red);
  double *part = a.partials + ((long long)rep * g.ctas_per_rep + cta) * NSTAT;
  if (tid < NSTAT) part[tid] = sm_red[tid];
  if (a.peer_code[0] != nullptr || a.peer_code[1] != nullptr) __threadfence_system();
  if (upd) {
#pragma unroll
    for (int o = 16; o > 0; o >>= 1) gbest = fmaxf(gbest, __shfl_down_sync(0xffffffffu, gbest, o));
    if (lane == 0) atomicMax(reinterpret_cast<unsigned int *>(const_cast<void *>(a.gmax)) + (long long)rep * a.cap + a.rel,
                             __float_as_uint(gbest));
  }
  __threadfence();
  if (lane == 0 && (upd || (tid == 0 && sel))) tma_store_wait_all();
  __syncthreads();
  if (tid == 0) {
    const unsigned t = atomicInc(a.tickets + rep, (unsigned)g.ctas_per_rep - 1u);
    s_is_last = (t == (unsigned)g.ctas_per_rep - 1u);
  }
  __syncthreads();
  if (!s_is_last) return;
// ... 190 lines not shown
```

### neighbor-aware-reinforcement-learning-fosters-cooperation-in-spatial-public-goods-games-_b200/csrc/spgg_kernels.cuh

```cuda
#pragma once
#include <cuda_runtime.h>
#include <stdint.h>

namespace spgg {

constexpr int GH = 2;
constexpr int CPAD = 16;
constexpr int WPAD = 4;
constexpr int GC = 2;
constexpr int TC = 128;
constexpr int HP = 4;
constexpr int SMW = TC + 2 * HP;
constexpr int HR = 2;
constexpr int NSTAT = 40;
constexpr int MAX_THREADS = 256;

enum {
  ST_NC_OLD = 0, ST_N_CD = 1, ST_N_DC = 2, ST_NC_NEW = 3, ST_SUM_P = 4, ST_SUM_P_C = 5,
  ST_SUM_P_D = 6, ST_SUM_WP_P = 7, ST_SUM_REW_C = 8, ST_SUM_REW_D = 9, ST_SUM_RATIO = 10,
  ST_GROUP0 = 11, ST_SUM_R = 17, ST_SUM_Q = 18, ST_SUM_Q_C = 22, ST_SUM_Q_D = 26,
  ST_SUM_NI = 30, ST_N_BEST_POS = 31, ST_N_BEST_2ND = 32, ST_GMAX = 33,
  ST_X_SN0 = 34,
  ST_X_NSEL = 38
};

__device__ __constant__ const int8_t c_off[12][2] = {
    {1, 0}, {-1, 0}, {0, 1}, {0, -1}, {2, 0}, {-2, 0},
    {0, 2}, {0, -2}, {1, 1}, {1, -1}, {-1, 1}, {-1, -1}};

struct RepConst {
  float rewtab[128];
  float ratiotab[128];
  uint32_t pkeys[20];
  double g[6];
  double cost, lo, span, wP, wR, rc;
  double alpha, gamma, kappa, leps;
  double gainC, lossD, rmin, rmax;
  double rq;
  float alpha_f, gamma_f, kappa_f, leps_f;
  float gainC_f, lossD_f, rmin_f, rmax_f;
  int gain_i, loss_i, rmin_i, rmax_i;
  uint32_t seed_lo, seed_hi;
  int has_ratio;
  int pad_;
};

struct Geom {
  int L, rows, row0, wrap_rows;
  int pitchB;
  int pitchW;
  int n_tx, n_ty, TR;
  int ctas_per_rep, n_rep;
  long long plane_stride;
  long long bits_stride;
  long long site_stride;
};

#ifndef SPGG_MAX_RING
#define SPGG_MAX_RING 16
#endif
constexpr int RING_SLOTS = 4, RING_WORDS = 4;

struct KArgs {
  Geom g;
  const RepConst *rc;
  void *Q;
  const void *R_in;
  void *R_out;
  const void *code_in;
  void *code_out;
  const uint32_t *S_in;
  uint32_t *S_out;
  const void *gmax;
  const double *valtab;
  double *stats;
  double *partials;
  unsigned *tickets;
  int *stop_at;
  const double *eps_tab;
  const uint32_t *thr_tab;
  const double *u;
  const uint8_t *b;
  int algo;
  const double *u2, *u3;
  const uint8_t *b2, *b3;
  int j;
  int rel;
  int cap;
  int do_update, do_select;
  int spec;
  float *gcarry;
  int *bad_at;
  float *gvec;
  void *peer_code[2];
  void *peer_R[2];
  uint32_t *peer_S[2];
  int peer_rows[2];
  unsigned *ring_peer[SPGG_MAX_RING];
  int ring_world, gen;
#ifdef SPGG_TRACE
  unsigned long long *trace;
#endif
};

__device__ __forceinline__ void pdl_launch_dependents() { asm volatile("griddepcontrol.launch_dependents;" ::: "memory"); }
__device__ __forceinline__ void pdl_wait() { asm volatile("griddepcontrol.wait;" ::: "memory"); }

__device__ __forceinline__ void philox4x32_10(uint32_t c0, uint32_t c1, uint32_t c2, uint32_t c3,
                                              uint32_t k0, uint32_t k1, uint32_t (&out)[4]) {
#pragma unroll
  for (int r = 0; r < 10; ++r) {
    const uint32_t hi0 = __umulhi(0xD2511F53u, c0), lo0 = 0xD2511F53u * c0;
    const uint32_t hi1 = __umulhi(0xCD9E8D57u, c2), lo1 = 0xCD9E8D57u * c2;
    c0 = hi1 ^ c1 ^ k0;
    c1 = lo1;
    c2 = hi0 ^ c3 ^ k1;
    c3 = lo0;
    k0 += 0x9E3779B9u;
    k1 += 0xBB67AE85u;
  }
  out[0] = c0; out[1] = c1; out[2] = c2; out[3] = c3;
}

__device__ __forceinline__ void philox4x32_10_keys(uint32_t c0, uint32_t c1, uint32_t c2, uint32_t c3,
                                                   const uint32_t *keys, uint32_t (&out)[4]) {
  uint32_t k[20];
#pragma unroll
  for (int q = 0; q < 5; ++q) {
    const uint4 v = reinterpret_cast<const uint4 *>(keys)[q];
    k[4 * q] = v.x; k[4 * q + 1] = v.y; k[4 * q + 2] = v.z; k[4 * q + 3] = v.w;
  }
#pragma unroll
  for (int r = 0; r < 10; ++r) {
    const uint32_t hi0 = __umulhi(0xD2511F53u, c0), lo0 = 0xD2511F53u * c0;
    const uint32_t hi1 = __umulhi(0xCD9E8D57u, c2), lo1 = 0xCD9E8D57u * c2;
    c0 = hi1 ^ c1 ^ k[2 * r];
    c1 = lo1;
    c2 = hi0 ^ c3 ^ k[2 * r + 1];
    c3 = lo0;
  }
  out[0] = c0; out[1] = c1; out[2] = c2; out[3] = c3;
}

struct ModeF32I8 {
  typedef float Q; typedef int8_t R; typedef uint8_t Code; typedef float Val;
  static constexpr bool kFp64 = false;
};
struct ModeF32F {
  typedef float Q; typedef float R; typedef uint8_t Code; typedef float Val;
  static constexpr bool kFp64 = false;
};
struct ModeF64 {
  typedef double Q; typedef double R; typedef uint32_t Code; typedef double Val;
  static constexpr bool kFp64 = true;
};

template <class Md>
__device__ __forceinline__ typename Md::Code pack_code(const int (&n)[5], int C, int coop, int s) {
  if constexpr (Md::kFp64) {
    return (typename Md::Code)((n[0] << 15) | (n[1] << 12) | (n[2] << 9) | (n[3] << 6) |
                               (n[4] << 3) | (C << 2) | (coop << 1) | s);
  } else {
    return (typename Md::Code)(((n[0] + n[1] + n[2] + n[3] + n[4]) << 3) | (C << 2) |
                               (coop << 1) | s);
  }
}

__device__ __forceinline__ double payoff_f64(uint32_t code, const RepConst &rc) {
  const double C = (double)((code >> 2) & 1u), D = 1.0 - C;
  double tot = 0.0;
#pragma unroll
  for (int q = 0; q < 5; ++q) {
    const double share = rc.g[(code >> (15 - 3 * q)) & 7u];
    const double term =
        __dadd_rn(__dmul_rn(__dsub_rn(share, rc.cost), C), __dmul_rn(share, D));
    tot = (q == 0) ? term : __dadd_rn(tot, term);
  }
  return __ddiv_rn(__dsub_rn(tot, rc.lo), rc.span);
}
__device__ __forceinline__ double reward_f64(uint32_t code, double P, const RepConst &rc) {
  const double rr = ((code >> 1) & 1u) ? 0.5 : 0.0;
  return __dadd_rn(__dmul_rn(rc.wP, P), __dmul_rn(rc.wR, rr));
}

constexpr int VALTAB_BITS = 17;

__device__ __forceinline__ uint32_t sigma_n_of_code(uint32_t code) {
  const uint32_t x = code >> 3;
  const uint32_t a = x & 070707u, b = (x >> 3) & 0707u;
  return (((a * 010101u) >> 12) & 63u) + (((b * 0101u) >> 6) & 63u);
}

template <class Md>
__device__ __forceinline__ typename Md::Val val_of_code(typename Md::Code code, const RepConst &rc,
                                                        const float *sm_tab, const double *valtab = nullptr) {
  if constexpr (Md::kFp64) {
    if (valtab) return __ldg(valtab + 2 * (size_t)(code >> 1));
    return reward_f64(code, payoff_f64(code, rc), rc);
  } else {
    return sm_tab[code >> 1];
  }
}

__device__ __forceinline__ double opaque(double x) {
  asm("" : "+d"(x));
  return x;
}
__device__ __forceinline__ double ddiv_zero_safe(double num, double den) {
  const bool z = (num == 0.0) && (den > 0.0);
  const double q = __ddiv_rn(opaque(z ? 1.0 : num), den);
  return z ? num : q;
}

template <class RT, int M>
__device__ __forceinline__ int rep_state(const RT *smR, int sr, int sc) {
  constexpr int NK = (M == 2) ? 12 : 4;
  if constexpr (sizeof(RT) == 1) {
    int acc = smR[sr * SMW + sc];
#pragma unroll
    for (int k = 0; k < NK; ++k) acc += smR[(sr - c_off[k][0]) * SMW + (sc - c_off[k][1])];
    return acc > 0;
  } else if constexpr (sizeof(RT) == 4) {
    float acc = smR[sr * SMW + sc];
#pragma unroll
    for (int k = 0; k < NK; ++k)
      acc = __fadd_rn(acc, smR[(sr - c_off[k][0]) * SMW + (sc - c_off[k][1])]);
    return __fdiv_rn(acc, (float)(NK + 1)) > 0.0f;
  } else {
    double acc = smR[sr * SMW + sc];
#pragma unroll
    for (int k = 0; k < NK; ++k)
      acc = __dadd_rn(acc, smR[(sr - c_off[k][0]) * SMW + (sc - c_off[k][1])]);
    const bool plain = fabs(acc) > 1e-300 || acc == 0.0;
    int st = acc > 0.0;
    if (!plain) {
      asm volatile("");
      st = __ddiv_rn(acc, (double)(NK + 1)) > 0.0;
    }
    return st;
  }
}

__device__ __forceinline__ int wrap_col(int col, int L) {
  if (col < 0) {
    col += L;
    if (col < 0) col = ((col % L) + L) % L;
  } else if (col >= L) {
    col -= L;
    if (col >= L) col %= L;
  }
  return col;
}

template <class T, int H>
__device__ __forceinline__ void load_tile(T *sm, const T *plane, const Geom &g, int r0, int c0,
                                          int TR) {
  constexpr int NC = TC + 2 * H;
  const int nr = TR + 2 * H;
  for (int e = threadIdx.x; e < nr * NC; e += blockDim.x) {
    const int rr = e / NC - H, cc = e % NC - H;
    const int prow = r0 + rr + GH;
    T v = T(0);
    if (prow >= 0 && prow < g.rows + 2 * GH) {
      const int col = wrap_col(c0 + cc, g.L);
      v = plane[(long long)prow * g.pitchB + CPAD + col];
    }
    sm[(rr + HR) * SMW + cc + HP] = v;
  }
}

__device__ __forceinline__ void load_coop_tile(uint8_t *sm, const uint32_t *bits, const Geom &g,
                                               int r0, int c0, int TR) {
  constexpr int H = 2, NC = TC + 2 * H;
  const int nr = TR + 2 * H;
  for (int e = threadIdx.x; e < nr * NC; e += blockDim.x) {
    const int rr = e / NC - H, cc = e % NC - H;
    const int prow = r0 + rr + GH;
    uint8_t v = 0;
    if (prow >= 0 && prow < g.rows + 2 * GH) {
      const int col = wrap_col(c0 + cc, g.L);
      const uint32_t w = bits[(long long)prow * g.pitchW + WPAD + (col >> 5)];
      v = (uint8_t)(((w >> (col & 31)) & 1u) ^ 1u);
    }
    sm[(rr + HR) * SMW + cc + HP] = v;
  }
}

template <int NV>
__device__ __forceinline__ void block_reduce_bfly(double (&v)[NV], double *sm_red ) {
  const int lane = threadIdx.x & 31, warp = threadIdx.x >> 5, nw = blockDim.x >> 5;
  constexpr int NG = NV / 32;
#pragma unroll
  for (int gI = 0; gI < NG; ++gI) {
    double w[32];
#pragma unroll
    for (int i = 0; i < 32; ++i) w[i] = v[32 * gI + i];
#pragma unroll
    for (int lvl = 0; lvl < 5; ++lvl) {
      const int o = 16 >> lvl, half = 16 >> lvl;
      const bool hi = (lane & o) != 0;
#pragma unroll
      for (int i = 0; i < half; ++i) {
        const double keep = hi ? w[i + half] : w[i];
        const double send = hi ? w[i] : w[i + half];
        w[i] = keep + __shfl_xor_sync(0xffffffffu, send, o);
      }
    }
// ... 250 lines not shown
  if (threadIdx.x == 0) {
    const unsigned tk = atomicInc(a.tickets + rep, (unsigned)g.ctas_per_rep - 1u);
    *s_is_last = (tk == (unsigned)g.ctas_per_rep - 1u);
  }
  __syncthreads();
  if (!*s_is_last) return;
  __threadfence();
  fold_partials(a.partials + (long long)rep * g.ctas_per_rep * NSTAT, g.ctas_per_rep, sm_red);
  if (threadIdx.x == 0) {
    double *row = a.stats + ((long long)rep * a.cap + a.rel) * NSTAT;
    double *s = sm_red;
    if constexpr (kI8) s[ST_SUM_R] *= rc.rq;
    if (upd) {
      double Pc[4];
      const double nc[4] = {s[ST_SUM_P], s[ST_SUM_P_C], s[ST_SUM_P_D], s[ST_SUM_WP_P]};
      for (int z = 0; z < 4; ++z) {
        const double C = (z >> 1) ? 1.0 : 0.0;
        Pc[z] = ((rc.rc * s[ST_X_SN0 + z] / 5.0 - 5.0 * rc.cost * C * nc[z]) - rc.lo * nc[z]) /
                rc.span;
      }
      s[ST_SUM_P] = Pc[0] + Pc[1] + Pc[2] + Pc[3];
      s[ST_SUM_P_C] = Pc[2] + Pc[3];
      s[ST_SUM_P_D] = Pc[0] + Pc[1];
      s[ST_SUM_WP_P] = rc.wP * s[ST_SUM_P];
      s[ST_SUM_REW_C] = rc.wP * (Pc[1] + Pc[3]) + rc.wR * 0.5 * (nc[1] + nc[3]);
      s[ST_SUM_REW_D] = rc.wP * (Pc[0] + Pc[2]);
      for (int z = 0; z < 4; ++z) s[ST_SUM_Q_D + z] = s[ST_SUM_Q + z] - s[ST_SUM_Q_C + z];
      s[ST_GMAX] = (double)reinterpret_cast<const Val *>(a.gmax)[(long long)rep * a.cap + a.rel];
      for (int z = 0; z < ST_X_SN0; ++z) row[z] = s[z];
    } else {
      row[ST_SUM_R] = s[ST_SUM_R];
    }
    if (sel && g.wrap_rows) {
      const double nsel = s[ST_X_NSEL];
      if (nsel == 0.0 || nsel == (double)g.site_stride) a.stop_at[rep] = a.j + 1;
    }
  }
}


template <int NTAB>
__device__ __forceinline__ void load_rep_const(RepConst &s_rc, const RepConst *src, float *sm_tab) {
  for (int i = threadIdx.x; i < (int)(sizeof(RepConst) / 4); i += blockDim.x)
    reinterpret_cast<uint32_t *>(&s_rc)[i] = reinterpret_cast<const uint32_t *>(src)[i];
  __syncthreads();
  if constexpr (NTAB > 0) {
    for (int i = threadIdx.x; i < 128; i += blockDim.x) {
      sm_tab[i] = s_rc.rewtab[i];
      if constexpr (NTAB > 1) sm_tab[128 + i] = s_rc.ratiotab[i];
    }
  }
}

template <class Md>
__device__ __forceinline__ void lambda_den(const KArgs &a, int rep, const RepConst &rc, typename Md::Val &den,
                                           typename Md::Val &inv_den) {
  const typename Md::Val gm = reinterpret_cast<const typename Md::Val *>(a.gmax)[(long long)rep * a.cap + a.rel];
  if constexpr (Md::kFp64) den = __dadd_rn(gm, rc.leps);
  else inv_den = __fdiv_rn(1.0f, __fadd_rn(gm, rc.leps_f));
}

__device__ __forceinline__ void philox_row(int c0, int row, uint32_t ctr2, uint32_t ctr3, const RepConst &rc, int lane,
                                           uint32_t w4[4]) {
  uint32_t wc[4];
  philox4x32_10((uint32_t)((c0 >> 2) + lane), (uint32_t)row, ctr2, ctr3, rc.seed_lo, rc.seed_hi, wc);
#pragma unroll
  for (int k4 = 0; k4 < 4; ++k4) {
    const int src = 8 * k4 + (lane >> 2);
    const uint32_t x0 = __shfl_sync(0xffffffffu, wc[0], src), x1 = __shfl_sync(0xffffffffu, wc[1], src);
    const uint32_t x2 = __shfl_sync(0xffffffffu, wc[2], src), x3 = __shfl_sync(0xffffffffu, wc[3], src);
    w4[k4] = sel4<uint32_t>(lane & 3, x0, x1, x2, x3);
  }
}

template <class Val>
struct BestNeighbour {
  Val d;
  int idx, k;
};
template <class Md, int M>
__device__ __forceinline__ BestNeighbour<typename Md::Val> best_neighbour(const typename Md::Val *sm_val, int sr, int sc,
                                                                          typename Md::Val vx) {
  typedef typename Md::Val Val;
  constexpr int NK = (M == 2) ? 12 : 4;
  Val best = Val(0);
  int bidx = sr * SMW + sc, kstar = 0;
#pragma unroll
  for (int k = 0; k < NK; ++k) {
    const int nidx = (sr - c_off[k][0]) * SMW + (sc - c_off[k][1]);
    const Val vk = sm_val[nidx];
    Val d;
    if constexpr (Md::kFp64) d = __dsub_rn(vk, vx);
    else d = __fsub_rn(vk, vx);
    if (k == 0 || d > best) { best = d; bidx = nidx; kstar = k; }
  }
  return {best, bidx, kstar};
}

template <class NextF>
__device__ __forceinline__ float td_update_f32(const RepConst &rc, float vx, float qe, float na, float nb, int s,
                                               int s_new, int act, float best, bool same, float inv_den, NextF next,
                                               float &tni) {
  const float mx = next(na, nb, false);
  const float td = __fsub_rn(__fmaf_rn(rc.gamma_f, mx, vx), qe);
  const float qtd = __fmaf_rn(rc.alpha_f, td, qe);
  const float lam = __fmul_rn(__fmul_rn(rc.kappa_f, fmaxf(0.0f, best)), inv_den);
  const float nu = same ? lam : -lam;
  const float na2 = (s_new == s && act == 0) ? qtd : na;
  const float nb2 = (s_new == s && act == 1) ? qtd : nb;
  const float td2 = __fsub_rn(__fmaf_rn(rc.gamma_f, next(na2, nb2, true), vx), qtd);
  const float qfin = __fadd_rn(qtd, nu);
  const float an = fabsf(nu);
  tni = __fmaf_rn(__fdividef(an, __fadd_rn(__fadd_rn(fabsf(__fmul_rn(rc.alpha_f, td2)), an), 1e-8f)), 100.0f, tni);
  return qfin;
}


#ifndef SPGG_GEN_MINBLOCKS
#define SPGG_GEN_MINBLOCKS 3
#endif
template <class Md, int M, bool ACTION, bool REPLAY>
__global__ void __launch_bounds__(MAX_THREADS, SPGG_GEN_MINBLOCKS) k_step(KArgs a) {
  typedef typename Md::Q QT;
  typedef typename Md::R RT;
  typedef typename Md::Code Code;
  typedef typename Md::Val Val;
  constexpr bool kI8 = (sizeof(RT) == 1);
  const Geom &g = a.g;
  const int rep = blockIdx.x / g.ctas_per_rep, cta = blockIdx.x % g.ctas_per_rep;
  pdl_launch_dependents();
  pdl_wait();
  const int stop = a.stop_at[rep];
  if (stop >= 0 && a.j > stop) return;
  const bool upd = a.do_update != 0;
  const bool sel = (a.do_select != 0) && !(stop >= 0 && a.j == stop);

  extern __shared__ __align__(16) unsigned char smem[];
  const SmemLayout<Md> lay(g.TR);
  Val *sm_val = reinterpret_cast<Val *>(smem + lay.off_val);
  RT *sm_R = reinterpret_cast<RT *>(smem + lay.off_R);
  Code *sm_code = reinterpret_cast<Code *>(smem + lay.off_code);
  uint8_t *sm_C = smem + lay.off_C;
  uint8_t *sm_N = smem + lay.off_N;
  float *sm_tab = reinterpret_cast<float *>(smem + lay.off_tab);
  float *sm_ratio = sm_tab + 128;
  double *sm_red = reinterpret_cast<double *>(smem + lay.off_red);
  __shared__ RepConst s_rc;
  __shared__ int s_is_last;
  load_rep_const<2>(s_rc, a.rc + rep, sm_tab);
  const RepConst &rc = s_rc;

  const double *vtab = a.valtab ? a.valtab + ((size_t)rep << (VALTAB_BITS + 1)) : nullptr;
  const bool dq = (a.algo == 3);
  QT *Qp = reinterpret_cast<QT *>(a.Q) + (long long)rep * g.site_stride * (dq ? 8 : 4);
  const RT *R_in = reinterpret_cast<const RT *>(a.R_in) + (long long)rep * g.plane_stride;
  RT *R_out = reinterpret_cast<RT *>(a.R_out) + (long long)rep * g.plane_stride;
  const Code *code_in = reinterpret_cast<const Code *>(a.code_in) + (long long)rep * g.plane_stride;
  Code *code_out = reinterpret_cast<Code *>(a.code_out) + (long long)rep * g.plane_stride;
  const uint32_t *S_in = a.S_in + (long long)rep * g.bits_stride;
  uint32_t *S_out = a.S_out + (long long)rep * g.bits_stride;
  auto q_add = [](QT x, QT y) -> QT { if constexpr (Md::kFp64) return __dadd_rn(x, y); else return __fadd_rn(x, y); };
  auto q_sub = [](QT x, QT y) -> QT { if constexpr (Md::kFp64) return __dsub_rn(x, y); else return __fsub_rn(x, y); };
  auto q_mul = [](QT x, QT y) -> QT { if constexpr (Md::kFp64) return __dmul_rn(x, y); else return __fmul_rn(x, y); };
  auto q_div = [](QT x, QT y) -> QT { if constexpr (Md::kFp64) return __ddiv_rn(x, y); else return __fdiv_rn(x, y); };
  auto q_max = [](QT x, QT y) -> QT { return x > y ? x : (y > x ? y : x); };
  auto q_mean = [&](QT x, QT y) -> QT { return q_div(q_add(x, y), QT(2)); };

  Val inv_den = Val(0), den = Val(1);
  if (upd) lambda_den<Md>(a, rep, rc, den, inv_den);
  const long long tab_idx = (long long)(a.rel + 1) * g.n_rep + rep;
  const double eps_u = (upd && a.algo != 0) ? a.eps_tab[(long long)a.rel * g.n_rep + rep] : 0.0;
  const uint32_t thr_u = (upd && a.algo == 1) ? a.thr_tab[(long long)a.rel * g.n_rep + rep] : 0u;
  const uint32_t thr = sel ? a.thr_tab[tab_idx] : 0u;
  const double eps = (sel && REPLAY) ? a.eps_tab[tab_idx] : 0.0;

  const int lane = threadIdx.x & 31, warp = threadIdx.x >> 5, nw = blockDim.x >> 5;

  unsigned long long cls_n[4] = {0, 0, 0, 0};
  unsigned long long cls_sn[4] = {0, 0, 0, 0};
  unsigned long long grp[6] = {0, 0, 0, 0, 0, 0};
  unsigned long long n_best = 0, n_best2 = 0, n_sel_coop = 0;
  double sumQ[4] = {0, 0, 0, 0}, sumQC[4] = {0, 0, 0, 0};
  double sumNI = 0.0, sumR = 0.0, sumRatio = 0.0;

  const int n_tiles = g.n_tx * g.n_ty;
  for (int tile = cta; tile < n_tiles; tile += g.ctas_per_rep) {
    const int r0 = (tile / g.n_tx) * g.TR, c0 = (tile % g.n_tx) * TC;
    __syncthreads();
    stage_tile<Md, M, true>(g, r0, c0, code_in, R_in, S_in, rc, sm_tab, vtab, sm_val, sm_code, sm_R, sm_C);
    __syncthreads();
    {
      const int nr = g.TR + 2;
      for (int r = warp; r < nr; r += nw) {
        const int base = (r - 1 + HR) * SMW + HP;
#pragma unroll
        for (int q = 0; q < (TC + 2 + 31) / 32; ++q) {
          const int cc = q * 32 + lane - 1;
          if (cc < TC + 1) {
            const int idx = base + cc;
            sm_N[idx] = (uint8_t)(sm_C[idx] + sm_C[idx + SMW] + sm_C[idx - SMW] + sm_C[idx + 1] + sm_C[idx - 1]);
          }
        }
      }
    }
    __syncthreads();

    unsigned pk_n = 0;
    unsigned long long pk_sn = 0, pk_grp = 0;
    float tq[4] = {0.f, 0.f, 0.f, 0.f}, tqc[4] = {0.f, 0.f, 0.f, 0.f};
    float tni = 0.f, tratio = 0.f, trf = 0.f;
    int tri = 0;

    for (int rr = warp; rr < g.TR; rr += nw) {
      const int i = r0 + rr;
      if (i >= g.rows) break;
      const int sr = rr + HR;
      uint32_t w4[4] = {0, 0, 0, 0};
      if (sel && !REPLAY) philox_row(c0, g.row0 + i, (uint32_t)(a.j + 1), 0u, rc, lane, w4);
      uint32_t wS1[4] = {0, 0, 0, 0}, wS2[4] = {0, 0, 0, 0};
      if (upd && (a.algo == 1 || a.algo == 3) && a.u2 == nullptr) {
        philox_row(c0, g.row0 + i, (uint32_t)a.j, 1u, rc, lane, wS1);
        philox_row(c0, g.row0 + i, (uint32_t)a.j, 2u, rc, lane, wS2);
      }
#pragma unroll
      for (int k4 = 0; k4 < 4; ++k4) {
        const int cc = k4 * 32 + lane;
        const int col = c0 + cc;
        const bool valid = col < g.L;
        const int sc = cc + HP;
        const int sidx = sr * SMW + sc;
        int a_new = 0;
        if (valid) {
          const long long site = (long long)i * g.L + col;
          QT q0_, q1_, q2_, q3_;
          QT t1[4], t2[4];
          if (dq) {
#pragma unroll
            for (int z = 0; z < 4; ++z) { t1[z] = Qp[site * 8 + z]; t2[z] = Qp[site * 8 + 4 + z]; }
            q0_ = q_mean(t1[0], t2[0]); q1_ = q_mean(t1[1], t2[1]);
            q2_ = q_mean(t1[2], t2[2]); q3_ = q_mean(t1[3], t2[3]);
          } else if constexpr (Md::kFp64) {
            const double2 lo2 = reinterpret_cast<const double2 *>(Qp)[site * 2];
            const double2 hi2 = reinterpret_cast<const double2 *>(Qp)[site * 2 + 1];
            q0_ = lo2.x; q1_ = lo2.y; q2_ = hi2.x; q3_ = hi2.y;
          } else {
            const float4 v = reinterpret_cast<const float4 *>(Qp)[site];
            q0_ = v.x; q1_ = v.y; q2_ = v.z; q3_ = v.w;
          }
          const RT r_old = sm_R[sidx];
          const int Ccur = sm_C[sidx];
          const int s_new = ACTION ? Ccur : rep_state<RT, M>(sm_R, sr, sc);
          if constexpr (kI8) tri += (int)r_old;
          else if constexpr (sizeof(RT) == 4) trf += r_old;
          else sumR += r_old;

          if (upd) {
            const Code code = sm_code[sidx];
            const int s = code & 1u, coop = (code >> 1) & 1u, wasC = (code >> 2) & 1u;
            const int act = coop ^ 1;
            const Val vx = sm_val[sidx];
            const auto bn = best_neighbour<Md, M>(sm_val, sr, sc, vx);
            const Val best = bn.d;
            const bool same = (((sm_code[bn.idx] >> 1) & 1u) == (unsigned)coop);
            const int e = 2 * s + act;
            const QT qe = sel4<QT>(e, q0_, q1_, q2_, q3_);
            const QT na = s_new ? q2_ : q0_, nb = s_new ? q3_ : q1_;
            QT qtd, qfin;
            bool ex1 = false, ex2 = false;
            int rn1 = 0, rn2 = 0;
            if (a.algo == 1) {
              if (a.u2 != nullptr) {
                ex1 = a.u2[site] < eps_u; rn1 = a.b2[site];
                ex2 = a.u3[site] < eps_u; rn2 = a.b3[site];
              } else {
                ex1 = (wS1[k4] >> 8) < thr_u; rn1 = (int)(wS1[k4] & 1u);
                ex2 = (wS2[k4] >> 8) < thr_u; rn2 = (int)(wS2[k4] & 1u);
              }
            }
            bool dq_done = false;
            if (dq) {
              const bool upd1 = (a.u2 != nullptr) ? (a.u2[site] < 0.5) : ((wS1[k4] >> 8) < (1u << 23));
              const int r0i = 2 * s_new;
              const QT nx1 = q_max(t2[r0i], t2[r0i + 1]), nx2 = q_max(t1[r0i], t1[r0i + 1]);
              const QT g_ = Md::kFp64 ? (QT)rc.gamma : (QT)rc.gamma_f, al_ = Md::kFp64 ? (QT)rc.alpha : (QT)rc.alpha_f;
              if (upd1) t1[e] = q_add(t1[e], q_mul(al_, q_sub(q_add(vx, q_mul(g_, nx1)), t1[e])));
              else t2[e] = q_add(t2[e], q_mul(al_, q_sub(q_add(vx, q_mul(g_, nx2)), t2[e])));
              QT cq[4];
#pragma unroll
              for (int z = 0; z < 4; ++z) cq[z] = q_mean(t1[z], t2[z]);
              qtd = cq[e];
              const QT td2 = q_sub(q_add(vx, q_mul(g_, q_max(cq[r0i], cq[r0i + 1]))), qtd);
              QT lam;
              if constexpr (Md::kFp64) lam = ddiv_zero_safe(__dmul_rn(rc.kappa, fmax(0.0, best)), den);
              else lam = __fmul_rn(__fmul_rn(rc.kappa_f, fmaxf(0.0f, best)), inv_den);
              const QT nu = same ? lam : -lam;
              t1[e] = q_add(t1[e], nu);
              t2[e] = q_add(t2[e], nu);
              q0_ = q_mean(t1[0], t2[0]); q1_ = q_mean(t1[1], t2[1]);
              q2_ = q_mean(t1[2], t2[2]); q3_ = q_mean(t1[3], t2[3]);
              qfin = sel4<QT>(e, q0_, q1_, q2_, q3_);
              const QT an = nu < QT(0) ? -nu : nu;
              const QT atd = q_mul(al_, td2);
              const QT pct = q_mul(q_div(an, q_add(q_add(atd < QT(0) ? -atd : atd, an), (QT)1e-8)), (QT)100.0);
              if constexpr (Md::kFp64) {
                sumNI += pct;
                pk_sn += (unsigned long long)sigma_n_of_code(code) << (16 * (wasC * 2 + coop));
                if (coop)
                  sumRatio += __dmul_rn(
                      __ddiv_rn(fabs(__dmul_rn(rc.wR, 0.5)), __dadd_rn(fabs(vx), 1e-9)), 100.0);
              } else {
                tni += pct;
                pk_sn += (unsigned long long)(code >> 3) << (16 * (wasC * 2 + coop));
                if (rc.has_ratio && coop) tratio += sm_ratio[code >> 1];
              }
              dq_done = true;
            }
            if (dq_done) {
            } else if constexpr (Md::kFp64) {
              auto next_value = [&](double x0, double x1, bool ex, int rn) -> double {
                if (a.algo == 0) return fmax(x0, x1);
                const int greedy = (x1 > x0) ? 1 : 0;
                if (a.algo == 1) return (ex ? rn : greedy) ? x1 : x0;
                const double po = __ddiv_rn(eps_u, 2.0);
                const double pg = __dadd_rn(__dsub_rn(1.0, eps_u), po);
                return __dadd_rn(__dmul_rn(greedy ? po : pg, x0), __dmul_rn(greedy ? pg : po, x1));
              };
              const double mx = next_value(na, nb, ex1, rn1);
              const double td = __dsub_rn(__dadd_rn(vx, __dmul_rn(rc.gamma, mx)), qe);
              qtd = __dadd_rn(qe, __dmul_rn(rc.alpha, td));
              const double lam = ddiv_zero_safe(__dmul_rn(rc.kappa, fmax(0.0, best)), den);
              const double nu = same ? lam : -lam;
              const double na2 = (s_new == s && act == 0) ? qtd : na;
              const double nb2 = (s_new == s && act == 1) ? qtd : nb;
              const double td2 = __dsub_rn(__dadd_rn(vx, __dmul_rn(rc.gamma, next_value(na2, nb2, ex2, rn2))), qtd);
              qfin = __dadd_rn(qtd, nu);
              const double an = fabs(nu);
              sumNI += __dmul_rn(
                  ddiv_zero_safe(an, __dadd_rn(__dadd_rn(fabs(__dmul_rn(rc.alpha, td2)), an), 1e-8)),
                  100.0);
              pk_sn += (unsigned long long)sigma_n_of_code(code) << (16 * (wasC * 2 + coop));
              if (coop)
                sumRatio += __dmul_rn(
                    __ddiv_rn(fabs(__dmul_rn(rc.wR, 0.5)), __dadd_rn(fabs(vx), 1e-9)), 100.0);
            } else {
              auto next_value = [&](float x0, float x1, bool after) -> float {
                if (a.algo == 0) return fmaxf(x0, x1);
                const int greedy = (x1 > x0) ? 1 : 0;
                if (a.algo == 1) return ((after ? ex2 : ex1) ? (after ? rn2 : rn1) : greedy) ? x1 : x0;
                const float e = (float)eps_u, po = __fmul_rn(e, 0.5f), pg = __fadd_rn(__fsub_rn(1.0f, e), po);
                return __fmaf_rn(greedy ? pg : po, x1, __fmul_rn(greedy ? po : pg, x0));
              };
              qfin = td_update_f32(rc, vx, qe, na, nb, s, s_new, act, best, same, inv_den, next_value, tni);
              pk_sn += (unsigned long long)(code >> 3) << (16 * (wasC * 2 + coop));
              if (rc.has_ratio && coop) tratio += sm_ratio[code >> 1];
            }
            if (!dq) {
              q0_ = (e == 0) ? qfin : q0_;
              q1_ = (e == 1) ? qfin : q1_;
              q2_ = (e == 2) ? qfin : q2_;
              q3_ = (e == 3) ? qfin : q3_;
            }
            pk_n += 1u << (8 * (wasC * 2 + coop));
            if (best > Val(0)) { n_best += 1u; n_best2 += (bn.k >= 4); }
            pk_grp += 1ull << (10 * (5 - (int)sm_N[sidx]));
            if constexpr (Md::kFp64) {
              sumQ[0] += q0_; sumQ[1] += q1_; sumQ[2] += q2_; sumQ[3] += q3_;
              if (wasC) { sumQC[0] += q0_; sumQC[1] += q1_; sumQC[2] += q2_; sumQC[3] += q3_; }
            } else {
              const float m = wasC ? 1.0f : 0.0f;
              tq[0] += q0_; tq[1] += q1_; tq[2] += q2_; tq[3] += q3_;
              tqc[0] = fmaf(m, q0_, tqc[0]); tqc[1] = fmaf(m, q1_, tqc[1]);
              tqc[2] = fmaf(m, q2_, tqc[2]); tqc[3] = fmaf(m, q3_, tqc[3]);
            }
          }

          if (sel) {
            int explore, rnd;
            if constexpr (REPLAY) {
              explore = a.u[site] < eps;
              rnd = a.b[site];
            } else {
              explore = (w4[k4] >> 8) < thr;
              rnd = (int)(w4[k4] & 1u);
            }
            const QT ga = s_new ? q2_ : q0_, gb = s_new ? q3_ : q1_;
            const int greedy = (gb > ga) ? 1 : 0;
            a_new = explore ? rnd : greedy;
            n_sel_coop += (a_new == 0);
            RT r_new;
            if constexpr (kI8) {
              int t = (int)r_old + (a_new == 0 ? rc.gain_i : -rc.loss_i);
              t = max(t, rc.rmin_i);
              t = min(t, rc.rmax_i);
              r_new = (RT)t;
            } else if constexpr (sizeof(RT) == 4) {
              const float t = __fadd_rn(r_old, a_new == 0 ? rc.gainC_f : -rc.lossD_f);
              r_new = fminf(fmaxf(t, rc.rmin_f), rc.rmax_f);
            } else {
              const double t = __dadd_rn(r_old, a_new == 0 ? rc.gainC : -rc.lossD);
              r_new = fmin(fmax(t, rc.rmin), rc.rmax);
            }
            const int n5[5] = {sm_N[sidx], sm_N[sidx - SMW], sm_N[sidx + SMW], sm_N[sidx - 1],
                               sm_N[sidx + 1]};
            const Code cnew = pack_code<Md>(n5, Ccur, a_new ^ 1, s_new);
            store_cell<Code>(code_out, g, i, col, cnew);
            store_cell<RT>(R_out, g, i, col, r_new);
          }
          if (upd) {
            if (dq) {
#pragma unroll
              for (int z = 0; z < 4; ++z) { Qp[site * 8 + z] = t1[z]; Qp[site * 8 + 4 + z] = t2[z]; }
            } else if constexpr (Md::kFp64) {
              reinterpret_cast<double2 *>(Qp)[site * 2] = make_double2(q0_, q1_);
              reinterpret_cast<double2 *>(Qp)[site * 2 + 1] = make_double2(q2_, q3_);
            } else {
              reinterpret_cast<float4 *>(Qp)[site] = make_float4(q0_, q1_, q2_, q3_);
            }
          }
        }
        if (sel) {
          const uint32_t word = __ballot_sync(0xffffffffu, valid && a_new);
          const int wi = (c0 >> 5) + k4;
          if (lane == 0 && wi * 32 < g.L) store_bits_word(S_out, g, i, wi, word);
        }
      }
    }
#pragma unroll
    for (int z = 0; z < 4; ++z) {
      cls_n[z] += (pk_n >> (8 * z)) & 0xffu;
      cls_sn[z] += (pk_sn >> (16 * z)) & 0xffffull;
      sumQ[z] += (double)tq[z];
      sumQC[z] += (double)tqc[z];
    }
#pragma unroll
    for (int z = 0; z < 6; ++z) grp[z] += (pk_grp >> (10 * z)) & 0x3ffull;
    sumNI += (double)tni;
    sumRatio += (double)tratio;
    sumR += (double)tri + (double)trf;
  }

  StepSums sums;
#pragma unroll
  for (int z = 0; z < 4; ++z) { sums.cls_n[z] = cls_n[z]; sums.cls_sn[z] = cls_sn[z]; sums.sumQ[z] = sumQ[z]; sums.sumQC[z] = sumQC[z]; }
#pragma unroll
  for (int z = 0; z < 6; ++z) sums.grp[z] = grp[z];
  sums.n_best = n_best; sums.n_best2 = n_best2; sums.n_sel_coop = n_sel_coop;
  sums.sumNI = sumNI; sums.sumR = sumR; sums.sumRatio = sumRatio;
  step_epilogue<Md>(a, rep, cta, rc, sums, sm_red, &s_is_last, upd, sel);
}

template <class Md>
__global__ void k_halo_pack(Geom g, const void *code, const void *R, const uint32_t *S,
                            unsigned char *to_up, unsigned char *to_down, long long rep_bytes) {
  typedef typename Md::Code Code;
  typedef typename Md::R RT;
  const int rep = blockIdx.y;
  const long long nB = (long long)GH * g.pitchB, nW = (long long)GH * g.pitchW;
  const Code *cp = reinterpret_cast<const Code *>(code) + (long long)rep * g.plane_stride;
  const RT *rp = reinterpret_cast<const RT *>(R) + (long long)rep * g.plane_stride;
  const uint32_t *sp = S + (long long)rep * g.bits_stride;
  unsigned char *up = to_up + rep * rep_bytes, *dn = to_down + rep * rep_bytes;
  Code *upc = reinterpret_cast<Code *>(up), *dnc = reinterpret_cast<Code *>(dn);
  RT *upr = reinterpret_cast<RT *>(up + sizeof(Code) * nB), *dnr = reinterpret_cast<RT *>(dn + sizeof(Code) * nB);
  uint32_t *ups = reinterpret_cast<uint32_t *>(up + (sizeof(Code) + sizeof(RT)) * nB);
  uint32_t *dns = reinterpret_cast<uint32_t *>(dn + (sizeof(Code) + sizeof(RT)) * nB);
  const long long top = (long long)GH * g.pitchB, bot = (long long)g.rows * g.pitchB;
  for (long long e = blockIdx.x * (long long)blockDim.x + threadIdx.x; e < nB;
       e += (long long)gridDim.x * blockDim.x) {
    upc[e] = cp[top + e]; upr[e] = rp[top + e];
    dnc[e] = cp[bot + e]; dnr[e] = rp[bot + e];
  }
  const long long topw = (long long)GH * g.pitchW, botw = (long long)g.rows * g.pitchW;
  for (long long e = blockIdx.x * (long long)blockDim.x + threadIdx.x; e < nW;
       e += (long long)gridDim.x * blockDim.x) {
    ups[e] = sp[topw + e];
    dns[e] = sp[botw + e];
  }
}

template <class Md>
__global__ void k_halo_unpack(Geom g, void *code, void *R, uint32_t *S, const unsigned char *from_up,
                              const unsigned char *from_down, long long rep_bytes) {
  typedef typename Md::Code Code;
  typedef typename Md::R RT;
  const int rep = blockIdx.y;
  const long long nB = (long long)GH * g.pitchB, nW = (long long)GH * g.pitchW;
  Code *cp = reinterpret_cast<Code *>(code) + (long long)rep * g.plane_stride;
  RT *rp = reinterpret_cast<RT *>(R) + (long long)rep * g.plane_stride;
  uint32_t *sp = S + (long long)rep * g.bits_stride;
  const unsigned char *up = from_up + rep * rep_bytes, *dn = from_down + rep * rep_bytes;
  const Code *upc = reinterpret_cast<const Code *>(up), *dnc = reinterpret_cast<const Code *>(dn);
  const RT *upr = reinterpret_cast<const RT *>(up + sizeof(Code) * nB);
  const RT *dnr = reinterpret_cast<const RT *>(dn + sizeof(Code) * nB);
  const uint32_t *ups = reinterpret_cast<const uint32_t *>(up + (sizeof(Code) + sizeof(RT)) * nB);
  const uint32_t *dns = reinterpret_cast<const uint32_t *>(dn + (sizeof(Code) + sizeof(RT)) * nB);
  const long long botg = (long long)(g.rows + GH) * g.pitchB;
  for (long long e = blockIdx.x * (long long)blockDim.x + threadIdx.x; e < nB;
       e += (long long)gridDim.x * blockDim.x) {
    cp[e] = upc[e]; rp[e] = upr[e];
    cp[botg + e] = dnc[e]; rp[botg + e] = dnr[e];
  }
  const long long botgw = (long long)(g.rows + GH) * g.pitchW;
  for (long long e = blockIdx.x * (long long)blockDim.x + threadIdx.x; e < nW;
       e += (long long)gridDim.x * blockDim.x) {
    sp[e] = ups[e];
    sp[botgw + e] = dns[e];
  }
}

template <class Md>
__global__ void k_init_random(Geom g, int rep, void *Q, void *R, uint32_t *S, uint32_t seed_lo,
                              uint32_t seed_hi, int nq) {
  typedef typename Md::Q QT;
  typedef typename Md::R RT;
  QT *Qp = reinterpret_cast<QT *>(Q) + (long long)rep * g.site_stride * nq;
  RT *Rp = reinterpret_cast<RT *>(R) + (long long)rep * g.plane_stride;
  uint32_t *Sp = S + (long long)rep * g.bits_stride;
  const long long n_sites = g.site_stride;
  for (long long x = blockIdx.x * (long long)blockDim.x + threadIdx.x; x < n_sites;
       x += (long long)gridDim.x * blockDim.x) {
    const int i = (int)(x / g.L), j = (int)(x % g.L);
    for (int t = 0; t < nq / 4; ++t) {
      uint32_t w[4];
      philox4x32_10((uint32_t)j, (uint32_t)(g.row0 + i), (uint32_t)t, 1u, seed_lo, seed_hi, w);
#pragma unroll
      for (int z = 0; z < 4; ++z) {
        const double uu = (double)(w[z] >> 8) * (1.0 / 16777216.0);
        Qp[x * nq + 4 * t + z] = (QT)(-0.01 + 0.02 * uu);
      }
    }
  }
  const int nW = (g.L + 31) >> 5;
  const long long n_words = (long long)g.rows * nW;
  for (long long e = blockIdx.x * (long long)blockDim.x + threadIdx.x; e < n_words;
       e += (long long)gridDim.x * blockDim.x) {
    const int i = (int)(e / nW), wi = (int)(e % nW);
    uint32_t w[4];
    philox4x32_10((uint32_t)(wi >> 2), (uint32_t)(g.row0 + i), 0u, 2u, seed_lo, seed_hi, w);
    uint32_t word = w[wi & 3];
    const int rem = g.L - wi * 32;
    if (rem < 32) word &= (1u << rem) - 1u;
    store_bits_word(Sp, g, i, wi, word);
  }
  const long long n_plane = (long long)(g.rows + 2 * GH) * g.pitchB;
  for (long long e = blockIdx.x * (long long)blockDim.x + threadIdx.x; e < n_plane;
       e += (long long)gridDim.x * blockDim.x)
    Rp[e] = RT(0);
}

template <class Md>
__global__ void k_import_rows(Geom g, int rep, int i0, int nrows, const uint8_t *S, const double *R,
                              const double *Q, void *Qd, void *Rd, uint32_t *Sd, double rq,
                              unsigned long long *info, int nq) {
  typedef typename Md::Q QT;
  typedef typename Md::R RT;
  QT *Qp = reinterpret_cast<QT *>(Qd) + (long long)rep * g.site_stride * nq;
  RT *Rp = reinterpret_cast<RT *>(Rd) + (long long)rep * g.plane_stride;
  uint32_t *Sp = Sd + (long long)rep * g.bits_stride;
  const int lane = threadIdx.x & 31;
  const int words = (g.L + 31) / 32;
  const long long n_items = (long long)nrows * words;
  const long long warp0 = (blockIdx.x * (long long)blockDim.x + threadIdx.x) >> 5;
  const long long n_warps = ((long long)gridDim.x * blockDim.x) >> 5;
  unsigned long long coop = 0;
  bool wide = false;
  for (long long it = warp0; it < n_items; it += n_warps) {
    const int ii = (int)(it / words), w = (int)(it % words);
    const int i = i0 + ii, col = w * 32 + lane;
    const bool valid = col < g.L;
    int bit = 0;
    RT rv = RT(0);
    if (valid) {
      const long long src = (long long)ii * g.L + col;
      const uint8_t sv = S[src];
      if (sv > 1) atomicExch(info, 1ull);
      bit = sv & 1;
      const double r = R[src];
      if constexpr (sizeof(RT) == 1) {
        const double q = r / rq;
        if (q != floor(q) || q < -128.0 || q > 127.0) atomicExch(info, 2ull);
        wide = wide || q < -16.0 || q > 15.0;
        rv = (RT)(int)q;
      } else {
        rv = (RT)r;
      }
      const long long site = (long long)i * g.L + col;
      for (int z = 0; z < nq; ++z) Qp[site * nq + z] = (QT)Q[src * nq + z];
    }
    const uint32_t word = __ballot_sync(0xffffffffu, valid && bit);
    const uint32_t vmask = __ballot_sync(0xffffffffu, valid);
    if (lane == 0) coop += __popc(vmask & ~word);
    if (valid) store_cell<RT>(Rp, g, i, col, rv);
    if (lane == 0) store_bits_word(Sp, g, i, w, word);
  }
  if (lane == 0 && coop) atomicAdd(info + 1, coop);
  if (wide) atomicExch(info + 2, 1ull);
}

template <class Md>
__global__ void k_export_rows(Geom g, int rep, int i0, int nrows, uint8_t *S, double *R, double *Q,
                              const void *Qd, const void *Rd, const uint32_t *Sd, double rq, int nq) {
  typedef typename Md::Q QT;
  typedef typename Md::R RT;
  const QT *Qp = reinterpret_cast<const QT *>(Qd) + (long long)rep * g.site_stride * nq;
  const RT *Rp = reinterpret_cast<const RT *>(Rd) + (long long)rep * g.plane_stride;
  const uint32_t *Sp = Sd + (long long)rep * g.bits_stride;
  const long long n = (long long)nrows * g.L;
  for (long long e = blockIdx.x * (long long)blockDim.x + threadIdx.x; e < n;
       e += (long long)gridDim.x * blockDim.x) {
    const int ii = (int)(e / g.L), col = (int)(e % g.L);
    const int i = i0 + ii;
    if (S) S[e] = (uint8_t)((Sp[(long long)(i + GH) * g.pitchW + WPAD + (col >> 5)] >> (col & 31)) & 1u);
    if (R) {
      const RT rv = Rp[(long long)(i + GH) * g.pitchB + CPAD + col];
      R[e] = (sizeof(RT) == 1) ? (double)rv * rq : (double)rv;
    }
    if (Q) {
      const long long site = (long long)i * g.L + col;
      for (int z = 0; z < nq; ++z) Q[e * nq + z] = (double)Qp[site * nq + z];
    }
  }
}

__device__ __forceinline__ unsigned long long digest_mix(unsigned long long x) {
  x ^= x >> 33; x *= 0xff51afd7ed558ccdull; x ^= x >> 33; x *= 0xc4ceb9fe1a85ec53ull; x ^= x >> 33;
  return x;
}
template <class Md>
__global__ void k_state_digest(Geom g, int rep, const void *Qd, const void *Rd, const uint32_t *Sd, int nq,
                               double rq, unsigned long long *out) {
  typedef typename Md::Q QT;
  typedef typename Md::R RT;
  const QT *Qp = reinterpret_cast<const QT *>(Qd) + (long long)rep * g.site_stride * nq;
  const RT *Rp = reinterpret_cast<const RT *>(Rd) + (long long)rep * g.plane_stride;
  const uint32_t *Sp = Sd + (long long)rep * g.bits_stride;
  unsigned long long dS = 0, dR = 0, dQ = 0;
  const long long n = g.site_stride;
  for (long long e = blockIdx.x * (long long)blockDim.x + threadIdx.x; e < n;
       e += (long long)gridDim.x * blockDim.x) {
    const int i = (int)(e / g.L), col = (int)(e % g.L);
    const unsigned long long key = ((unsigned long long)(unsigned)(g.row0 + i) << 32) | (unsigned)col;
    const unsigned long long hS = digest_mix(key * 3 + 1), hR = digest_mix(key * 3 + 2);
    const unsigned bit = (Sp[(long long)(i + GH) * g.pitchW + WPAD + (col >> 5)] >> (col & 31)) & 1u;
    dS += hS * (unsigned long long)(bit + 1u);
    double rv = (double)Rp[(long long)(i + GH) * g.pitchB + CPAD + col];
    if (sizeof(RT) == 1) rv *= rq;
    dR += hR * ((unsigned long long)__double_as_longlong(rv) + 1ull);
    for (int z = 0; z < nq; ++z) {
      const double qv = (double)Qp[e * nq + z];
      dQ += digest_mix(key * 3 + 3 + ((unsigned long long)(z + 1) << 58)) * ((unsigned long long)__double_as_longlong(qv) + 1ull);
    }
  }
  for (int o = 16; o > 0; o >>= 1) {
    dS += __shfl_down_sync(0xffffffffu, dS, o);
    dR += __shfl_down_sync(0xffffffffu, dR, o);
    dQ += __shfl_down_sync(0xffffffffu, dQ, o);
  }
  if ((threadIdx.x & 31) == 0) {
    atomicAdd(out + 0, dS);
    atomicAdd(out + 1, dR);
    atomicAdd(out + 2, dQ);
  }
}

static __global__ void k_strip_verify(float *gvec, int rel, int j, int was_upd, int was_spec, int was_sel, float *gcarry,
                               float *gmax_tab, int *bad_at, int *stop_at) {
  if (threadIdx.x != 0 || blockIdx.x != 0) return;
  if (*bad_at < rel) return;
  if (stop_at[0] >= 0 && (j > stop_at[0] || (j == stop_at[0] && !was_upd))) return;
  if (was_upd) {
    const float g_exact = gvec[4 * rel + 0];
    const float guess = gcarry[0];
    gmax_tab[rel] = g_exact;
    gcarry[0] = g_exact;
    if (was_spec == 2 || (was_spec && g_exact != guess)) { atomicMin(bad_at, rel); return; }
  }
  if (was_sel && (gvec[4 * rel + 1] == 0.0f || gvec[4 * rel + 2] == 0.0f) && stop_at[0] < 0) stop_at[0] = j + 1;
}

template <class Md>
__global__ void k_r_histogram(Geom g, int rep, const void *Rd, double rq, int nb, const double *edges,
                              unsigned long long *counts) {
  typedef typename Md::R RT;
  __shared__ unsigned int s_cnt[64];
  __shared__ double s_edge[65];
  const RT *Rp = reinterpret_cast<const RT *>(Rd) + (long long)rep * g.plane_stride;
  if (threadIdx.x < 64) s_cnt[threadIdx.x] = 0u;
  if (threadIdx.x <= nb) s_edge[threadIdx.x] = edges[threadIdx.x];
  __syncthreads();
  const double lo = s_edge[0], hi = s_edge[nb];
  const double norm = (double)nb / (hi - lo);
  const long long n = g.site_stride;
  for (long long e = blockIdx.x * (long long)blockDim.x + threadIdx.x; e < n;
       e += (long long)gridDim.x * blockDim.x) {
    const int i = (int)(e / g.L), col = (int)(e % g.L);
    double v = (double)Rp[(long long)(i + GH) * g.pitchB + CPAD + col];
    if (sizeof(RT) == 1) v *= rq;
    if (!(v >= lo && v <= hi)) continue;
    int idx = (int)((v - lo) * norm);
    if (idx == nb) idx -= 1;
    if (v < s_edge[idx]) idx -= 1;
    else if (v >= s_edge[idx + 1] && idx != nb - 1) idx += 1;
    atomicAdd(&s_cnt[idx], 1u);
  }
  __syncthreads();
  if (threadIdx.x < nb && s_cnt[threadIdx.x]) atomicAdd(counts + threadIdx.x, (unsigned long long)s_cnt[threadIdx.x]);
}

static __global__ void k_ring_verify(unsigned *ring, int gen, int world, float *gvec, int rel, int j, int was_upd, int was_spec,
                              int was_sel, float *gcarry, float *gmax_tab, int *bad_at, int *stop_at) {
  if (threadIdx.x != 0 || blockIdx.x != 0) return;
  if (*bad_at < rel) return;
  if (stop_at[0] >= 0 && (j > stop_at[0] || (j == stop_at[0] && !was_upd))) return;
  volatile unsigned *slot = ring + (gen & (RING_SLOTS - 1)) * RING_WORDS;
  const long long t0 = clock64();
  while (slot[3] < (unsigned)world) {
    if (clock64() - t0 > 20000000000ll) __trap();
    __nanosleep(200);
  }
  __threadfence_system();
  const float g_exact = __uint_as_float(slot[0]);
  const float anyD = slot[1] ? 1.0f : 0.0f, anyC = slot[2] ? 1.0f : 0.0f;
  gvec[4 * rel + 0] = g_exact; gvec[4 * rel + 1] = anyD; gvec[4 * rel + 2] = anyC;
  unsigned *nxt = ring + ((gen + 2) & (RING_SLOTS - 1)) * RING_WORDS;
  nxt[0] = 0u; nxt[1] = 0u; nxt[2] = 0u; nxt[3] = 0u;
  __threadfence_system();
  if (was_upd) {
    const float guess = gcarry[0];
    gmax_tab[rel] = g_exact;
    gcarry[0] = g_exact;
    if (was_spec == 2 || (was_spec && g_exact != guess)) { atomicMin(bad_at, rel); return; }
  }
  if (was_sel && (anyD == 0.0f || anyC == 0.0f) && stop_at[0] < 0) stop_at[0] = j + 1;
}

}
```

### neighbor-aware-reinforcement-learning-fosters-cooperation-in-spatial-public-goods-games-_b200/csrc/spgg_lean.cuh

```cuda
#pragma once
#include "spgg_dispatch.h"
#include "spgg_kernels.cuh"

namespace spgg {

__global__ void k_build_valtab(const RepConst *rc_all, double *tab) {
  const int rep = blockIdx.y;
  const uint32_t idx = blockIdx.x * blockDim.x + threadIdx.x;
  if (idx >= (1u << VALTAB_BITS)) return;
  const RepConst &rc = rc_all[rep];
  const uint32_t code = idx << 1;
  double v = 0.0, ratio = 0.0;
  bool ok = true;
#pragma unroll
  for (int q = 0; q < 5; ++q) ok = ok && (((code >> (15 - 3 * q)) & 7u) <= 5u);
  if (ok) {
    v = reward_f64(code, payoff_f64(code, rc), rc);
    if ((code >> 1) & 1u)
      ratio = __dmul_rn(__ddiv_rn(fabs(__dmul_rn(rc.wR, 0.5)), __dadd_rn(fabs(v), 1e-9)), 100.0);
  }
  double *dst = tab + (((size_t)rep << VALTAB_BITS) + idx) * 2;
  dst[0] = v;
  dst[1] = ratio;
}

template <bool B>
struct BoolC { static constexpr bool value = B; };

template <class Md, int M>
__global__ void __launch_bounds__(MAX_THREADS) k_gmax_lean(GArgs a) {
  typedef typename Md::Code Code;
  typedef typename Md::Val Val;
  const Geom &g = a.g;
  const int rep = blockIdx.x / g.ctas_per_rep, cta = blockIdx.x % g.ctas_per_rep;
  pdl_launch_dependents();
  pdl_wait();
  const int stop = a.stop_at[rep];
  if (stop >= 0 && a.j > stop) return;

  extern __shared__ __align__(16) unsigned char smem[];
  Val *sm_val = reinterpret_cast<Val *>(smem);
  float *sm_tab = reinterpret_cast<float *>(smem + align_up(sizeof(Val) * (g.TR + 2 * HR) * SMW, 16));
  __shared__ RepConst s_rc;
  load_rep_const<Md::kFp64 ? 0 : 1>(s_rc, a.rc + rep, sm_tab);

  const Code *code_in = reinterpret_cast<const Code *>(a.code_in) + (long long)rep * g.plane_stride;
  const double *vtab = a.valtab ? a.valtab + ((size_t)rep << (VALTAB_BITS + 1)) : nullptr;
  const int lane = threadIdx.x & 31, warp = threadIdx.x >> 5, nw = blockDim.x >> 5;
  Val lmax = Val(0);
  constexpr int NP = (M == 2) ? 6 : 2;
  constexpr int kPair[6] = {1, 3, 5, 7, 11, 10};

  const int n_tiles = g.n_tx * g.n_ty;
  for (int tile = cta; tile < n_tiles; tile += g.ctas_per_rep) {
    const int ty = tile / g.n_tx, tx = tile - ty * g.n_tx;
    const int r0 = ty * g.TR, c0 = tx * TC;
    __syncthreads();
    stage_tile<Md, M, false>(g, r0, c0, code_in, nullptr, nullptr, s_rc, sm_tab, vtab, sm_val, nullptr, nullptr, nullptr);
    __syncthreads();
    for (int rr = warp; rr < g.TR; rr += nw) {
      if (r0 + rr >= g.rows) break;
#pragma unroll
      for (int k4 = 0; k4 < 4; ++k4) {
        const int cc = k4 * 32 + lane;
        if (c0 + cc >= g.L) continue;
        const int sr = rr + HR, sc = cc + HP;
        const Val vx = sm_val[sr * SMW + sc];
#pragma unroll
        for (int k = 0; k < NP; ++k) {
          const Val vk = sm_val[(sr - c_off[kPair[k]][0]) * SMW + (sc - c_off[kPair[k]][1])];
          Val d;
          if constexpr (Md::kFp64) d = fabs(__dsub_rn(vk, vx));
          else d = fabsf(__fsub_rn(vk, vx));
          lmax = d > lmax ? d : lmax;
        }
      }
    }
  }
#pragma unroll
  for (int o = 16; o > 0; o >>= 1) {
    const Val other = __shfl_down_sync(0xffffffffu, lmax, o);
    lmax = other > lmax ? other : lmax;
  }
  __shared__ Val s_wmax[MAX_THREADS / 32];
  if (lane == 0) s_wmax[warp] = lmax;
  __syncthreads();
  if (threadIdx.x == 0) {
    Val m = s_wmax[0];
    for (int w = 1; w < nw; ++w) m = s_wmax[w] > m ? s_wmax[w] : m;
    Val *dst = reinterpret_cast<Val *>(a.gmax) + (long long)rep * a.cap + a.rel;
    if constexpr (Md::kFp64)
      atomicMax(reinterpret_cast<unsigned long long *>(dst), (unsigned long long)__double_as_longlong(m));
    else
      atomicMax(reinterpret_cast<unsigned int *>(dst), __float_as_uint(m));
  }
}

#ifndef SPGG_LEAN_MINBLOCKS
#define SPGG_LEAN_MINBLOCKS 2
#endif

template <class Md, int M, bool ACTION, bool REPLAY>
__global__ void __launch_bounds__(MAX_THREADS, SPGG_LEAN_MINBLOCKS) k_step_lean(KArgs a) {
  typedef typename Md::Q QT;
  typedef typename Md::R RT;
  typedef typename Md::Code Code;
  typedef typename Md::Val Val;
  constexpr bool kI8 = (sizeof(RT) == 1);
  const Geom &g = a.g;
  const int rep = blockIdx.x / g.ctas_per_rep, cta = blockIdx.x % g.ctas_per_rep;
  pdl_launch_dependents();
  pdl_wait();
  const int stop = a.stop_at[rep];
  if (stop >= 0 && a.j > stop) return;
  constexpr bool upd = true;
  const bool sel = (a.do_select != 0) && !(stop >= 0 && a.j == stop);

  extern __shared__ __align__(16) unsigned char smem[];
  constexpr SmemLayout<Md> lay(LEAN_TR_MAX);
  Val *sm_val = reinterpret_cast<Val *>(smem + lay.off_val);
  RT *sm_R = reinterpret_cast<RT *>(smem + lay.off_R);
  Code *sm_code = reinterpret_cast<Code *>(smem + lay.off_code);
  uint8_t *sm_C = smem + lay.off_C;
  uint8_t *sm_N = smem + lay.off_N;
  float *sm_tab = reinterpret_cast<float *>(smem + lay.off_tab);
  float *sm_ratio = sm_tab + 128;
  double *sm_red = reinterpret_cast<double *>(smem + lay.off_red);
  __shared__ RepConst s_rc;
  __shared__ int s_is_last;

  load_rep_const<2>(s_rc, a.rc + rep, sm_tab);
  const RepConst &rc = s_rc;
  const double *vtab = a.valtab ? a.valtab + ((size_t)rep << (VALTAB_BITS + 1)) : nullptr;

  QT *Qp = reinterpret_cast<QT *>(a.Q) + (long long)rep * g.site_stride * 4;
  const RT *R_in = reinterpret_cast<const RT *>(a.R_in) + (long long)rep * g.plane_stride;
  RT *R_out = reinterpret_cast<RT *>(a.R_out) + (long long)rep * g.plane_stride;
  const Code *code_in = reinterpret_cast<const Code *>(a.code_in) + (long long)rep * g.plane_stride;
  Code *code_out = reinterpret_cast<Code *>(a.code_out) + (long long)rep * g.plane_stride;
  const uint32_t *S_in = a.S_in + (long long)rep * g.bits_stride;
  uint32_t *S_out = a.S_out + (long long)rep * g.bits_stride;

  Val inv_den = Val(0), den = Val(1);
  lambda_den<Md>(a, rep, rc, den, inv_den);
  const long long tab_idx = (long long)(a.rel + 1) * g.n_rep + rep;
  const uint32_t thr = sel ? a.thr_tab[tab_idx] : 0u;
  const double eps = (sel && REPLAY) ? a.eps_tab[tab_idx] : 0.0;

  const int lane = threadIdx.x & 31, warp = threadIdx.x >> 5, nw = blockDim.x >> 5;

  uint32_t cls_n[4] = {0, 0, 0, 0}, cls_sn[4] = {0, 0, 0, 0};
  uint32_t grp[6] = {0, 0, 0, 0, 0, 0};
  uint32_t n_best = 0, n_best2 = 0, n_sel_coop = 0;
  double sumQ[4] = {0, 0, 0, 0}, sumQC[4] = {0, 0, 0, 0};
  double sumNI = 0.0, sumR = 0.0, sumRatio = 0.0;

  const int n_tiles = g.n_tx * g.n_ty;
  for (int tile = cta; tile < n_tiles; tile += g.ctas_per_rep) {
    const int ty = tile / g.n_tx, tx = tile - ty * g.n_tx;
    const int r0 = ty * g.TR, c0 = tx * TC;
    const bool full = (c0 + TC <= g.L) && (r0 + g.TR <= g.rows);
    const bool interior = full && c0 >= GC && c0 + TC <= g.L - GC &&
                          (!g.wrap_rows || (r0 >= GH && r0 + g.TR <= g.rows - GH));
    __syncthreads();
    {
      const int nt = tile + g.ctas_per_rep;
      if (nt < n_tiles) {
        const int nty = nt / g.n_tx, ntx = nt - nty * g.n_tx;
        const int nrow = nty * g.TR, ncol = ntx * TC;
        constexpr int kLineSites = 128 / (int)(4 * sizeof(QT));
        const int lines = TC / kLineSites;
        for (int e = threadIdx.x; e < g.TR * lines; e += blockDim.x) {
          const int rr = e / lines, cs = ncol + (e - rr * lines) * kLineSites;
          if (nrow + rr < g.rows && cs < g.L)
            asm volatile("prefetch.global.L2 [%0];" ::"l"(Qp + ((long long)(nrow + rr) * g.L + cs) * 4));
        }
      }
    }
    stage_tile<Md, M, true>(g, r0, c0, code_in, R_in, S_in, rc, sm_tab, vtab, sm_val, sm_code, sm_R, sm_C);
    __syncthreads();
    {
      const int nr = g.TR + 2;
      for (int r = warp; r < nr; r += nw) {
        const int base = (r - 1 + HR) * SMW + HP;
#pragma unroll
        for (int q = 0; q < (TC + 2 + 31) / 32; ++q) {
          const int cc = q * 32 + lane - 1;
          if (cc < TC + 1) {
            const int idx = base + cc;
            sm_N[idx] = (uint8_t)(sm_C[idx] + sm_C[idx + SMW] + sm_C[idx - SMW] + sm_C[idx + 1] + sm_C[idx - 1]);
          }
        }
      }
    }
    __syncthreads();

    unsigned pk_n = 0;
    unsigned long long pk_sn = 0, pk_grp = 0;
    float tq[4] = {0.f, 0.f, 0.f, 0.f}, tqc[4] = {0.f, 0.f, 0.f, 0.f};
    float tni = 0.f, tratio = 0.f, trf = 0.f;
    int tri = 0;

    auto do_row = [&](auto fullc, auto interiorc, int rr) {
      constexpr bool FULL = decltype(fullc)::value;
      constexpr bool INTERIOR = decltype(interiorc)::value;
      const int i = r0 + rr;
      const int sr = rr + HR;
      uint32_t w4[4] = {0, 0, 0, 0};
      if (sel && !REPLAY) philox_row(c0, g.row0 + i, (uint32_t)(a.j + 1), 0u, rc, lane, w4);
#ifndef SPGG_LEAN_BATCH
#define SPGG_LEAN_BATCH 2
#endif
#pragma unroll
      for (int kb = 0; kb < 4; kb += SPGG_LEAN_BATCH) {
      QT q[4][4];
      [[maybe_unused]] double ru[4] = {0, 0, 0, 0};
      [[maybe_unused]] uint8_t rb[4] = {0, 0, 0, 0};
      [[maybe_unused]] double rat[4] = {0, 0, 0, 0};
      const long long site_row = (long long)i * g.L + c0 + lane;
#pragma unroll
      for (int k4 = kb; k4 < kb + SPGG_LEAN_BATCH; ++k4) {
        const bool valid = FULL || (c0 + 32 * k4 + lane < g.L);
        const long long site = site_row + 32 * k4;
        if (valid) {
          if constexpr (Md::kFp64) {
            const double2 lo2 = reinterpret_cast<const double2 *>(Qp)[site * 2];
            const double2 hi2 = reinterpret_cast<const double2 *>(Qp)[site * 2 + 1];
            q[k4][0] = lo2.x; q[k4][1] = lo2.y; q[k4][2] = hi2.x; q[k4][3] = hi2.y;
          } else {
            const float4 v = reinterpret_cast<const float4 *>(Qp)[site];
            q[k4][0] = v.x; q[k4][1] = v.y; q[k4][2] = v.z; q[k4][3] = v.w;
          }
          if constexpr (REPLAY) {
            if (sel) { ru[k4] = a.u[site]; rb[k4] = a.b[site]; }
          }
          if constexpr (Md::kFp64)
            rat[k4] = __ldg(vtab + 2 * (size_t)(sm_code[sr * SMW + 32 * k4 + lane + HP] >> 1) + 1);
        } else {
          q[k4][0] = q[k4][1] = q[k4][2] = q[k4][3] = QT(0);
        }
      }
#pragma unroll
      for (int k4 = kb; k4 < kb + SPGG_LEAN_BATCH; ++k4) {
        const int cc = k4 * 32 + lane;
        const int col = c0 + cc;
        const bool valid = FULL || (col < g.L);
        const int sc = cc + HP;
        const int sidx = sr * SMW + sc;
        int a_new = 0;
        if (valid) {
          const long long site = site_row + 32 * k4;
          QT q0_ = q[k4][0], q1_ = q[k4][1], q2_ = q[k4][2], q3_ = q[k4][3];
          const RT r_old = sm_R[sidx];
          const int Ccur = sm_C[sidx];
          const int s_new = ACTION ? Ccur : rep_state<RT, M>(sm_R, sr, sc);
          if constexpr (kI8) tri += (int)r_old;
          else if constexpr (sizeof(RT) == 4) trf += r_old;
          else sumR += r_old;

          const Code code = sm_code[sidx];
          const int s = code & 1u, coop = (code >> 1) & 1u, wasC = (code >> 2) & 1u;
          const int act = coop ^ 1;
          const Val vx = sm_val[sidx];
          const auto bn = best_neighbour<Md, M>(sm_val, sr, sc, vx);
          const Val best = bn.d;
          const int bidx = bn.idx, kstar = bn.k;
          const bool same = (((sm_code[bidx] >> 1) & 1u) == (unsigned)coop);
          const int e = 2 * s + act;
          const QT qe = sel4<QT>(e, q0_, q1_, q2_, q3_);
          const QT na = s_new ? q2_ : q0_, nb = s_new ? q3_ : q1_;
          QT qfin;
          if constexpr (Md::kFp64) {
            const double mx = fmax(na, nb);
            const double td = __dsub_rn(__dadd_rn(vx, __dmul_rn(rc.gamma, mx)), qe);
            const double qtd = __dadd_rn(qe, __dmul_rn(rc.alpha, td));
            const double num = __dmul_rn(rc.kappa, fmax(0.0, best));
            const double na2 = (s_new == s && act == 0) ? qtd : na;
            const double nb2 = (s_new == s && act == 1) ? qtd : nb;
            const double td2 = __dsub_rn(__dadd_rn(vx, __dmul_rn(rc.gamma, fmax(na2, nb2))), qtd);
            double lam = num;
            if (!(num == 0.0 && den > 0.0)) {
              asm volatile("");
              lam = __ddiv_rn(num, den);
              const double an = fabs(lam);
              sumNI += __dmul_rn(ddiv_zero_safe(an, __dadd_rn(__dadd_rn(fabs(__dmul_rn(rc.alpha, td2)), an), 1e-8)), 100.0);
            }
            const double nu = same ? lam : -lam;
            qfin = __dadd_rn(qtd, nu);
            pk_sn += (unsigned long long)sigma_n_of_code(code) << (16 * (wasC * 2 + coop));
            if (coop) sumRatio += rat[k4];
          } else {
            auto next_value = [](float x0, float x1, bool) { return fmaxf(x0, x1); };
            qfin = td_update_f32(rc, vx, qe, na, nb, s, s_new, act, best, same, inv_den, next_value, tni);
            pk_sn += (unsigned long long)(code >> 3) << (16 * (wasC * 2 + coop));
            if (rc.has_ratio && coop) tratio += sm_ratio[code >> 1];
          }
          q0_ = (e == 0) ? qfin : q0_;
          q1_ = (e == 1) ? qfin : q1_;
          q2_ = (e == 2) ? qfin : q2_;
          q3_ = (e == 3) ? qfin : q3_;
          pk_n += 1u << (8 * (wasC * 2 + coop));
          if (best > Val(0)) { n_best += 1u; n_best2 += (kstar >= 4); }
          pk_grp += 1ull << (10 * (5 - (int)sm_N[sidx]));
          if constexpr (Md::kFp64) {
            sumQ[0] += q0_; sumQ[1] += q1_; sumQ[2] += q2_; sumQ[3] += q3_;
            if (wasC) { sumQC[0] += q0_; sumQC[1] += q1_; sumQC[2] += q2_; sumQC[3] += q3_; }
          } else {
            const float m = wasC ? 1.0f : 0.0f;
            tq[0] += q0_; tq[1] += q1_; tq[2] += q2_; tq[3] += q3_;
            tqc[0] = fmaf(m, q0_, tqc[0]); tqc[1] = fmaf(m, q1_, tqc[1]);
            tqc[2] = fmaf(m, q2_, tqc[2]); tqc[3] = fmaf(m, q3_, tqc[3]);
          }

          if (sel) {
            int explore, rnd;
            if constexpr (REPLAY) {
              explore = ru[k4] < eps;
              rnd = rb[k4];
            } else {
              explore = (w4[k4] >> 8) < thr;
              rnd = (int)(w4[k4] & 1u);
            }
            const QT ga = s_new ? q2_ : q0_, gb = s_new ? q3_ : q1_;
            const int greedy = (gb > ga) ? 1 : 0;
            a_new = explore ? rnd : greedy;
            n_sel_coop += (a_new == 0);
            RT r_new;
            if constexpr (kI8) {
              int t = (int)r_old + (a_new == 0 ? rc.gain_i : -rc.loss_i);
              t = max(t, rc.rmin_i);
              t = min(t, rc.rmax_i);
              r_new = (RT)t;
            } else if constexpr (sizeof(RT) == 4) {
              const float t = __fadd_rn(r_old, a_new == 0 ? rc.gainC_f : -rc.lossD_f);
              r_new = fminf(fmaxf(t, rc.rmin_f), rc.rmax_f);
            } else {
              const double t = __dadd_rn(r_old, a_new == 0 ? rc.gainC : -rc.lossD);
              r_new = fmin(fmax(t, rc.rmin), rc.rmax);
            }
            const int n5[5] = {sm_N[sidx], sm_N[sidx - SMW], sm_N[sidx + SMW], sm_N[sidx - 1], sm_N[sidx + 1]};
            const Code cnew = pack_code<Md>(n5, Ccur, a_new ^ 1, s_new);
            if constexpr (INTERIOR) {
              const long long o = (long long)(i + GH) * g.pitchB + CPAD + col;
              code_out[o] = cnew;
              R_out[o] = r_new;
            } else {
              store_cell<Code>(code_out, g, i, col, cnew);
              store_cell<RT>(R_out, g, i, col, r_new);
            }
          }
          if constexpr (Md::kFp64) {
            reinterpret_cast<double2 *>(Qp)[site * 2] = make_double2(q0_, q1_);
            reinterpret_cast<double2 *>(Qp)[site * 2 + 1] = make_double2(q2_, q3_);
          } else {
            reinterpret_cast<float4 *>(Qp)[site] = make_float4(q0_, q1_, q2_, q3_);
          }
        }
        if (sel) {
          const uint32_t word = __ballot_sync(0xffffffffu, valid && a_new);
          const int wi = (c0 >> 5) + k4;
          if (lane == 0) {
            if constexpr (INTERIOR) S_out[(long long)(i + GH) * g.pitchW + WPAD + wi] = word;
            else if (wi * 32 < g.L) store_bits_word(S_out, g, i, wi, word);
          }
        }
      }
      }
    };

    if (interior) {
      for (int rr = warp; rr < g.TR; rr += nw) do_row(BoolC<true>{}, BoolC<true>{}, rr);
    } else {
      for (int rr = warp; rr < g.TR; rr += nw) {
        if (r0 + rr >= g.rows) break;
        do_row(BoolC<false>{}, BoolC<false>{}, rr);
      }
    }
#pragma unroll
    for (int z = 0; z < 4; ++z) {
      cls_n[z] += (pk_n >> (8 * z)) & 0xffu;
      cls_sn[z] += (uint32_t)((pk_sn >> (16 * z)) & 0xffffull);
      sumQ[z] += (double)tq[z];
      sumQC[z] += (double)tqc[z];
    }
#pragma unroll
    for (int z = 0; z < 6; ++z) grp[z] += (uint32_t)((pk_grp >> (10 * z)) & 0x3ffull);
    sumNI += (double)tni;
    sumRatio += (double)tratio;
    sumR += (double)tri + (double)trf;
  }

  StepSums sums;
#pragma unroll
  for (int z = 0; z < 4; ++z) { sums.cls_n[z] = cls_n[z]; sums.cls_sn[z] = cls_sn[z]; sums.sumQ[z] = sumQ[z]; sums.sumQC[z] = sumQC[z]; }
#pragma unroll
  for (int z = 0; z < 6; ++z) sums.grp[z] = grp[z];
  sums.n_best = n_best; sums.n_best2 = n_best2; sums.n_sel_coop = n_sel_coop;
  sums.sumNI = sumNI; sums.sumR = sumR; sums.sumRatio = sumRatio;
  step_epilogue<Md>(a, rep, cta, rc, sums, sm_red, &s_is_last, upd, sel);
}

}
```

### neighbor-aware-reinforcement-learning-fosters-cooperation-in-spatial-public-goods-games-_b200/csrc/spgg_resident.cuh

```cuda
#pragma once
#include <cooperative_groups.h>

#include <type_traits>

#include "spgg_kernels.cuh"

namespace spgg {
namespace cg = cooperative_groups;

#ifdef SPGG_RES_TRACE
#define RES_STAMP(slot)                                                     \
  do {                                                                      \
    if (tid == 0) {                                                         \
      const long long now_ = clock64();                                     \
      trace_acc[slot] += now_ - trace_t;                                    \
      trace_t = now_;                                                       \
    }                                                                       \
  } while (0)
#else
#define RES_STAMP(slot) do {} while (0)
#endif

constexpr int RES_THREADS = 512;
constexpr int RES_CS_MAX = 16;
// ... 39 lines not shown
  }
};

struct RArgs {
  Geom g;
  ResGeom rg;
  const RepConst *rc;
  void *Q;
  void *R;
  uint32_t *S;
  double *stats;
  int *stop_at;
  const uint32_t *thr_tab;
  int t0;
  int n_steps;
  int cap;
  unsigned char *gimg;
  double *gpart;
  unsigned *gnsel;
  float *gmaxtab;
#ifdef SPGG_RES_TRACE
  long long *trace;
#endif
};

template <int M>
struct ValWin {
  float c[8], u[6], d[6], u2[4], d2[4];
};
template <int M, bool BELOW>
__device__ __forceinline__ void load_win(ValWin<M> &w, const float *V, int base, int pitch) {
  const float4 c4 = *reinterpret_cast<const float4 *>(V + base);
  w.c[2] = c4.x; w.c[3] = c4.y; w.c[4] = c4.z; w.c[5] = c4.w;
  w.c[1] = V[base - 1];
  const float4 u4 = *reinterpret_cast<const float4 *>(V + base - pitch);
  w.u[1] = u4.x; w.u[2] = u4.y; w.u[3] = u4.z; w.u[4] = u4.w;
  if constexpr (M == 2) {
    w.c[0] = V[base - 2];
    w.u[0] = V[base - pitch - 1];
    w.u[5] = V[base - pitch + 4];
    const float4 t4 = *reinterpret_cast<const float4 *>(V + base - 2 * pitch);
    w.u2[0] = t4.x; w.u2[1] = t4.y; w.u2[2] = t4.z; w.u2[3] = t4.w;
  }
  if constexpr (BELOW) {
    w.c[6] = V[base + 4];
    const float4 d4 = *reinterpret_cast<const float4 *>(V + base + pitch);
    w.d[1] = d4.x; w.d[2] = d4.y; w.d[3] = d4.z; w.d[4] = d4.w;
    if constexpr (M == 2) {
      w.c[7] = V[base + 5];
      w.d[0] = V[base + pitch - 1];
      w.d[5] = V[base + pitch + 4];
      const float4 t4 = *reinterpret_cast<const float4 *>(V + base + 2 * pitch);
      w.d2[0] = t4.x; w.d2[1] = t4.y; w.d2[2] = t4.z; w.d2[3] = t4.w;
    }
  }
}
template <int M, bool BELOW>
__device__ __forceinline__ void load_win_code(ValWin<M> &w, const uint8_t *code, const float *tab, int base,
                                              int pitch) {
  auto row4 = [&](int at, float *dst) {
    const uint32_t c = *reinterpret_cast<const uint32_t *>(code + at);
    dst[0] = tab[(c >> 1) & 127u]; dst[1] = tab[(c >> 9) & 127u];
    dst[2] = tab[(c >> 17) & 127u]; dst[3] = tab[c >> 25];
  };
  auto one = [&](int at) { return tab[code[at] >> 1]; };
  row4(base, &w.c[2]);
  w.c[1] = one(base - 1);
  row4(base - pitch, &w.u[1]);
  if constexpr (M == 2) {
    w.c[0] = one(base - 2);
    w.u[0] = one(base - pitch - 1);
    w.u[5] = one(base - pitch + 4);
    row4(base - 2 * pitch, &w.u2[0]);
  }
  if constexpr (BELOW) {
    w.c[6] = one(base + 4);
    row4(base + pitch, &w.d[1]);
    if constexpr (M == 2) {
      w.c[7] = one(base + 5);
      w.d[0] = one(base + pitch - 1);
      w.d[5] = one(base + pitch + 4);
      row4(base + 2 * pitch, &w.d2[0]);
    }
  }
}
template <int M>
__device__ __forceinline__ float win_nbr(const ValWin<M> &w, int k, int z) {
  switch (z) {
    case 0: return w.u[1 + k];
    case 1: return w.d[1 + k];
    case 2: return w.c[1 + k];
    case 3: return w.c[3 + k];
    case 4: return w.u2[k];
    case 5: return w.d2[k];
    case 6: return w.c[k];
    case 7: return w.c[4 + k];
    case 8: return w.u[k];
    case 9: return w.u[2 + k];
    case 10: return w.d[k];
    default: return w.d[2 + k];
  }
}

template <int M, bool ACTION, bool FULL, bool GRID = false>
__global__ void __launch_bounds__(RES_THREADS) k_resident(RArgs a) {
  constexpr int NK = (M == 2) ? 12 : 4;
  cg::cluster_group cluster = cg::this_cluster();
  const Geom &g = a.g;
  const ResGeom &rg = a.rg;
  const int CS = rg.CS;
  const int rep = blockIdx.x / CS;
  const int rank = GRID ? (int)(blockIdx.x % CS) : (int)cluster.block_rank();
  cg::grid_group grid = cg::this_grid();
  const int L = g.L, pitch = rg.pitch, QR = rg.QR;
  const int W = pitch >> 2;
  const int base_rows = L / CS, rem = L % CS;
  const int nrow = base_rows + (rank < rem ? 1 : 0);
  const int row_start = rank * base_rows + min(rank, rem);
  const int up = (rank + CS - 1) % CS, down = (rank + 1) % CS;
  const int nrow_up = base_rows + (up < rem ? 1 : 0);
  const int tid = threadIdx.x, nthr = blockDim.x;
  const int lane = tid & 31, warp = tid >> 5, nwarp = nthr >> 5;

  extern __shared__ __align__(16) unsigned char smem[];
  const ResSmem lay(rg);
  float4 *sQ = reinterpret_cast<float4 *>(smem + lay.q);
  const int q_plane = rg.rows_max * QR;
  float *s_val = reinterpret_cast<float *>(smem + lay.val);
  uint8_t *s_N = smem + lay.N;
  float *s_tab = reinterpret_cast<float *>(smem + lay.tab);
  float *s_ratio = s_tab + 128;
  float *s_redf = reinterpret_cast<float *>(smem + lay.redf);
  unsigned *s_redi = reinterpret_cast<unsigned *>(smem + lay.redi);
  float *s_gmx = reinterpret_cast<float *>(smem + lay.gmx);
  unsigned *s_nsel = reinterpret_cast<unsigned *>(smem + lay.nsel);
  double *s_part = reinterpret_cast<double *>(smem + lay.part);
  const int o_code0 = (int)lay.code[0], o_R0 = (int)lay.R[0], o_C0 = (int)lay.C[0];
  const int nb = rg.prow * pitch;
  __shared__ RepConst s_rc;
  __shared__ int s_noff[12];
  if (threadIdx.x < 12) s_noff[threadIdx.x] = c_off[threadIdx.x][0] * pitch + c_off[threadIdx.x][1];

  for (size_t i = (size_t)tid * 16; i < lay.total; i += (size_t)nthr * 16)
    *reinterpret_cast<uint4 *>(smem + i) = make_uint4(0u, 0u, 0u, 0u);
  for (int i = tid; i < (int)(sizeof(RepConst) / 4); i += nthr)
    reinterpret_cast<uint32_t *>(&s_rc)[i] = reinterpret_cast<const uint32_t *>(a.rc + rep)[i];
  __syncthreads();
  for (int i = tid; i < 128; i += nthr) {
    s_tab[i] = s_rc.rewtab[i];
    s_ratio[i] = s_rc.ratiotab[i];
  }
  const RepConst &rc = s_rc;

  float4 *Qg = reinterpret_cast<float4 *>(a.Q) + (long long)rep * g.site_stride;
  int8_t *Rg = reinterpret_cast<int8_t *>(a.R) + (long long)rep * g.plane_stride;
  uint32_t *Sg = a.S + (long long)rep * g.bits_stride;
  {
    uint8_t *R0 = smem + o_R0, *C0 = smem + o_C0;
    const int wc = L + 4, ncell = (nrow + 4) * wc;
    for (int e = tid; e < ncell; e += nthr) {
      const int rr = e / wc - 2, cc = e % wc - 2;
      int grow = row_start + rr, gcol = cc;
      grow += (grow < 0) ? L : 0; grow -= (grow >= L) ? L : 0;
      gcol += (gcol < 0) ? L : 0; gcol -= (gcol >= L) ? L : 0;
      const int idx = (rr + 2) * pitch + RG + cc;
      R0[idx] = (uint8_t)Rg[(long long)(grow + GH) * g.pitchB + CPAD + gcol];
      const uint32_t w = Sg[(long long)(grow + GH) * g.pitchW + WPAD + (gcol >> 5)];
      C0[idx] = (uint8_t)(((w >> (gcol & 31)) & 1u) ^ 1u);
    }
    float *sQf = reinterpret_cast<float *>(sQ);
    for (int e = tid; e < nrow * L; e += nthr) {
      const int rr = e / L, cc = e % L;
      const float4 v = Qg[(long long)(row_start + rr) * L + cc];
      const int o = (rr * QR + (cc >> 2)) * 4 + (cc & 3);
      sQf[o] = v.x;
      sQf[(q_plane * 4) + o] = v.y;
      sQf[(q_plane * 8) + o] = v.z;
      sQf[(q_plane * 12) + o] = v.w;
    }
  }
  const size_t img_stride = (size_t)6 * nb;
  unsigned char *smem_up, *smem_dn;
  if constexpr (GRID) {
    smem_up = a.gimg + (size_t)up * img_stride - o_code0;
    smem_dn = a.gimg + (size_t)down * img_stride - o_code0;
  } else {
    smem_up = cluster.map_shared_rank(smem, up);
    smem_dn = cluster.map_shared_rank(smem, down);
  }
  __syncthreads();
  if constexpr (!GRID) cluster.sync();

  const int w_r0 = tid / W, w_c0 = tid % W, w_dr = nthr / W, w_dc = nthr % W;
  const int q_r0 = tid / QR, q_c0 = tid % QR, q_dr = nthr / QR, q_dc = nthr % QR;
  const long long n_sites = (long long)L * L;

  double *s_ring = reinterpret_cast<double *>(smem + lay.ring);
  int ring_first = -1, ring_last = -1;
  auto flush_ring = [&]() {
    if (ring_first < 0) return;
    for (int r = ring_first; r <= ring_last; ++r) {
      double *row = a.stats + ((long long)rep * a.cap + r) * NSTAT;
      if (lane < RES_NRED) row[lane] = s_ring[(r % RES_RING) * RES_RAW + lane];
      if (lane == RES_NRED) row[RES_RAW_GMAX] = s_ring[(r % RES_RING) * RES_RAW + RES_NRED];
    }
    ring_first = -1;
  };
  auto do_fold = [&](int fs, float fgm) {
    double f = 0.0;
    if (lane < RES_NRED)
      for (int k = 0; k < CS; ++k) f += s_part[(fs & 1) * (RES_CS_MAX * RES_NRED) + k * RES_NRED + lane];
    if (lane == RES_NRED) f = (double)fgm;
    if (lane <= RES_NRED) s_ring[(fs % RES_RING) * RES_RAW + lane] = f;
    if (ring_first < 0) ring_first = fs;
    ring_last = fs;
    __syncwarp();
    if (fs - ring_first == RES_RING - 1) flush_ring();
  };
  auto grid_fold = [&](int first, int last) {
    const int fs = first + rank;
    if (fs > last) return;
    double *scr = reinterpret_cast<double *>(s_N);
    const int P = min(nwarp, 16);
    if (warp < P && lane < RES_NRED) {
      const double *pp = a.gpart + ((size_t)(fs % RES_RING) * CS) * RES_NRED + lane;
      double f = 0.0;
#pragma unroll 4
      for (int k = warp; k < CS; k += P) f += __ldcg(pp + (size_t)k * RES_NRED);
      scr[warp * 32 + lane] = f;
    }
    __syncthreads();
    if (warp == 0) {
      double f = 0.0;
      if (lane < RES_NRED)
        for (int j = 0; j < P; ++j) f += scr[j * 32 + lane];
      double *row = a.stats + ((long long)rep * a.cap + fs) * NSTAT;
      if (lane < RES_NRED) row[lane] = f;
      if (lane == RES_NRED) row[RES_RAW_GMAX] = (double)__ldcg(a.gmaxtab + (long long)rep * a.cap + fs);
    }
    __syncthreads();
  };
  int gfold_first = 0;
  int pend_s = -1, last_s = -1;
  float pend_gm = 0.0f;

  int stop = a.stop_at[rep];
  int cur = 0;
#ifdef SPGG_RES_TRACE
  long long trace_acc[8] = {0, 0, 0, 0, 0, 0, 0, 0};
  long long trace_t = clock64();
#endif
  for (int s = 0; s <= a.n_steps; ++s) {
    const int j = a.t0 + s;
    if (stop >= 0 && j > stop) break;
    const bool upd = s > 0;
    const bool sel = (s < a.n_steps) && !(stop >= 0 && j == stop);
    const uint32_t thr = sel ? __ldg(a.thr_tab + (long long)(s + 1) * g.n_rep + rep) : 0u;
    const uint8_t *codeC = smem + o_code0 + cur * nb;
    const uint8_t *Rc = smem + o_R0 + cur * nb;
    const uint8_t *Cc = smem + o_C0 + cur * nb;
    const int o_code_n = o_code0 + (cur ^ 1) * nb, o_R_n = o_R0 + (cur ^ 1) * nb, o_C_n = o_C0 + (cur ^ 1) * nb;

    {
      const uint32_t *Cw = reinterpret_cast<const uint32_t *>(Cc);
      uint32_t *Nw = reinterpret_cast<uint32_t *>(s_N);
      int rr = w_r0, wq = w_c0;
      while (rr < nrow + 2) {
        const int i4 = (rr + 1) * W + wq;
        const uint32_t c = Cw[i4];
        const uint32_t lw = __funnelshift_l(Cw[i4 - 1], c, 8), rw = __funnelshift_r(c, Cw[i4 + 1], 8);
        Nw[i4] = c + Cw[i4 - W] + Cw[i4 + W] + lw + rw;
        rr += w_dr; wq += w_dc;
        if (wq >= W) { wq -= W; rr += 1; }
      }
      if (upd && !GRID) {
        const uint32_t *cw = reinterpret_cast<const uint32_t *>(codeC);
        float4 *vw = reinterpret_cast<float4 *>(s_val);
        rr = w_r0; wq = w_c0;
        while (rr < nrow + 2 * M) {
          const int i4 = (rr + 2 - M) * W + wq;
          const uint32_t c = cw[i4];
          vw[i4] = make_float4(s_tab[(c >> 1) & 127u], s_tab[(c >> 9) & 127u], s_tab[(c >> 17) & 127u],
                               s_tab[c >> 25]);
          rr += w_dr; wq += w_dc;
          if (wq >= W) { wq -= W; rr += 1; }
        }
      }
    }
    __syncthreads();
    RES_STAMP(0);

    float inv_den = 0.0f, gm = 0.0f;
    if (upd) {
      float lmax = 0.0f;
      int rr = q_r0, qc = q_c0;
      while (rr < nrow) {
        const int base = (rr + 2) * pitch + RG + 4 * qc;
        ValWin<M> w;
        if constexpr (GRID) load_win_code<M, false>(w, codeC, s_tab, base, pitch);
        else load_win<M, false>(w, s_val, base, pitch);
#pragma unroll
        for (int k = 0; k < 4; ++k) {
          if (FULL || 4 * qc + k < L) {
            const float vx = w.c[2 + k];
#pragma unroll
            for (int z = 0; z < NK; ++z) {
              if (z == 1 || z == 3 || z == 5 || z == 7 || z == 10 || z == 11) continue;
              const float d = fabsf(__fsub_rn(win_nbr<M>(w, k, z), vx));
              lmax = d > lmax ? d : lmax;
            }
          }
        }
        rr += q_dr; qc += q_dc;
        if (qc >= QR) { qc -= QR; rr += 1; }
      }
      const unsigned wm = __reduce_max_sync(0xffffffffu, __float_as_uint(lmax));
      if (lane == 0) atomicMax(&s_redi[RES_NI], wm);
      __syncthreads();
      RES_STAMP(1);
      if constexpr (GRID) {
        if (tid == 0)
          atomicMax(reinterpret_cast<unsigned *>(a.gmaxtab) + (long long)rep * a.cap + s, s_redi[RES_NI]);
        grid.sync();
        RES_STAMP(2);
        gm = __ldcg(a.gmaxtab + (long long)rep * a.cap + s);
      } else {
        if (tid < CS) {
          float *dst = reinterpret_cast<float *>(cluster.map_shared_rank(smem, tid) + lay.gmx);
          dst[rank] = __uint_as_float(s_redi[RES_NI]);
        }
        cluster.barrier_arrive();
// ... 156 lines not shown
              }
              if (qc == QR - 1) {
                *reinterpret_cast<uint32_t *>(basep + o_code_n + at - L) = codew;
                *reinterpret_cast<uint32_t *>(basep + o_R_n + at - L) = rneww;
                *reinterpret_cast<uint32_t *>(basep + o_C_n + at - L) = coopw;
              }
            };
            putw(smem, base);
            if (rr < 2) putw(smem_up, (nrow_up + rr + 2) * pitch + RG + 4 * qc);
            if (rr >= nrow - 2) putw(smem_dn, (rr - nrow + 2) * pitch + RG + 4 * qc);
          } else {
            for (int k = 0; k < nvalid; ++k) {
              const int col = 4 * qc + k;
              const uint8_t cnew = (uint8_t)(codew >> (8 * k)), rnew = (uint8_t)(rneww >> (8 * k)),
                            Cnew = (uint8_t)(coopw >> (8 * k));
              const int gdx = (col < GC) ? L : ((col >= L - GC) ? -L : 0);
              auto put = [&](unsigned char *basep, int at) {
                basep[o_code_n + at] = cnew; basep[o_R_n + at] = rnew; basep[o_C_n + at] = Cnew;
                if (gdx) {
                  basep[o_code_n + at + gdx] = cnew; basep[o_R_n + at + gdx] = rnew; basep[o_C_n + at + gdx] = Cnew;
                }
              };
              put(smem, base + k);
              if (rr < 2) put(smem_up, (nrow_up + rr + 2) * pitch + RG + col);
              if (rr >= nrow - 2) put(smem_dn, (rr - nrow + 2) * pitch + RG + col);
            }
          }
        }
        if constexpr (upd) {
#pragma unroll
          for (int z = 0; z < 4; ++z) sQ[z * q_plane + qi] = make_float4(qv[z][0], qv[z][1], qv[z][2], qv[z][3]);
        }
        rr += q_dr; qc += q_dc;
        if (qc >= QR) { qc -= QR; rr += 1; }
      }
    };
    if (upd && sel) phase3(std::true_type{}, std::true_type{});
    else if (upd) phase3(std::true_type{}, std::false_type{});
    else if (sel) phase3(std::false_type{}, std::true_type{});
    else phase3(std::false_type{}, std::false_type{});

    RES_STAMP(3);
    {
      float v[32];
#pragma unroll
      for (int z = 0; z < 4; ++z) {
        v[z] = (float)((pk_n >> (8 * z)) & 0xffu);
        v[4 + z] = (float)(unsigned)((pk_sn >> (16 * z)) & 0xffffull);
        v[18 + z] = tq[z];
        v[22 + z] = tqc[z];
        v[28 + z] = 0.0f;
      }
#pragma unroll
      for (int z = 0; z < 6; ++z) v[8 + z] = (float)(unsigned)((pk_grp >> (10 * z)) & 0x3ffull);
      v[14] = (float)n_best; v[15] = (float)n_best2; v[16] = (float)n_sel_coop; v[17] = (float)tri;
      v[26] = tni; v[27] = tratio;
#pragma unroll
      for (int lvl = 0; lvl < 5; ++lvl) {
        const int o = 16 >> lvl, half = 16 >> lvl;
        const bool hi = (lane & o) != 0;
#pragma unroll
        for (int i = 0; i < half; ++i) {
          const float keep = hi ? v[i + half] : v[i];
          const float send = hi ? v[i] : v[i + half];
          v[i] = keep + __shfl_xor_sync(0xffffffffu, send, o);
        }
      }
      if (lane < RES_NRED) s_redf[warp * 32 + lane] = v[0];
    }
    __syncthreads();
    if (tid < RES_NRED) {
      double x = 0.0;
      for (int w = 0; w < nwarp; ++w) x += (double)s_redf[w * 32 + tid];
      if constexpr (GRID) {
        a.gpart[((size_t)(s % RES_RING) * CS + rank) * RES_NRED + tid] = x;
        if (tid == 16 && x != 0.0) atomicAdd(a.gnsel + s, (unsigned)x);
      } else {
        double *dst = reinterpret_cast<double *>(cluster.map_shared_rank(smem, 0) + lay.part);
        dst[(s & 1) * (RES_CS_MAX * RES_NRED) + rank * RES_NRED + tid] = x;
        if (tid == 16)
          for (int k = 0; k < CS; ++k)
            reinterpret_cast<unsigned *>(cluster.map_shared_rank(smem, k) + lay.nsel)[rank] = (unsigned)x;
      }
    }
    RES_STAMP(4);
    if constexpr (GRID) {
      grid.sync();
      RES_STAMP(5);
      if (sel) gnsel_v = __ldcg(a.gnsel + s);
      if (sel) {
        const uint32_t *img = reinterpret_cast<const uint32_t *>(a.gimg + (size_t)rank * img_stride);
        uint32_t *pl = reinterpret_cast<uint32_t *>(smem + o_code0);
        const int nbw = nb >> 2;
        for (int r12 = warp; r12 < 12; r12 += nwarp) {
          const int z = r12 >> 2, gr = r12 & 3;
          const int prow_ = (gr < 2) ? gr : nrow + gr;
          const int row_at = (2 * z + (cur ^ 1)) * nbw + prow_ * W;
          for (int w0 = lane; w0 < W; w0 += 32 * 8) {
            uint32_t tmp[8];
#pragma unroll
            for (int u = 0; u < 8; ++u)
              if (w0 + 32 * u < W) tmp[u] = __ldcg(img + row_at + w0 + 32 * u);
#pragma unroll
            for (int u = 0; u < 8; ++u)
              if (w0 + 32 * u < W) pl[row_at + w0 + 32 * u] = tmp[u];
          }
        }
        __syncthreads();
      }
      if ((s % RES_RING) == RES_RING - 1) {
        grid_fold(gfold_first, s);
        gfold_first = s + 1;
      }
    } else {
      cluster.sync();
      RES_STAMP(5);
    }

    if (sel) {
      long long tot = 0;
      if constexpr (GRID) {
        tot = gnsel_v;
      } else {
        for (int k = 0; k < CS; ++k) tot += s_nsel[k];
      }
      if (tot == 0 || tot == n_sites) stop = j + 1;
      cur ^= 1;
    }
    last_s = s;
    if constexpr (!GRID) { pend_s = s; pend_gm = gm; }
    if (tid <= RES_NI) s_redi[tid] = 0u;
    RES_STAMP(6);
  }

  if constexpr (GRID) {
    if (last_s >= gfold_first) grid_fold(gfold_first, last_s);
  } else if (rank == 0 && warp == 0) {
    if (pend_s >= 0) do_fold(pend_s, pend_gm);
    flush_ring();
  }

  if (rank == 0 && tid == 0) a.stop_at[rep] = stop;
#ifdef SPGG_RES_TRACE
  if (tid == 0 && a.trace)
    for (int z = 0; z < 8; ++z) a.trace[(long long)blockIdx.x * 8 + z] = trace_acc[z];
#endif
  {
    const uint8_t *Rc = smem + o_R0 + cur * nb;
    const uint8_t *Cc = smem + o_C0 + cur * nb;
    const float *sQf = reinterpret_cast<const float *>(sQ);
    for (int e = tid; e < nrow * L; e += nthr) {
      const int rr = e / L, cc = e % L;
      const int o = (rr * QR + (cc >> 2)) * 4 + (cc & 3);
      Qg[(long long)(row_start + rr) * L + cc] =
          make_float4(sQf[o], sQf[(q_plane * 4) + o], sQf[(q_plane * 8) + o], sQf[(q_plane * 12) + o]);
      store_cell<int8_t>(Rg, g, row_start + rr, cc, (int8_t)Rc[(rr + 2) * pitch + RG + cc]);
    }
    const int nW = (L + 31) >> 5;
    for (int e = tid; e < nrow * nW; e += nthr) {
      const int rr = e / nW, wi = e % nW;
      uint32_t word = 0;
      const int c0 = wi * 32, n = min(32, L - c0);
      for (int b = 0; b < n; ++b) word |= (uint32_t)(Cc[(rr + 2) * pitch + RG + c0 + b] ^ 1u) << b;
      store_bits_word(Sg, g, row_start + rr, wi, word);
    }
  }
}

__global__ void k_resident_rows(const RepConst *rcs, double *stats, int n_rep, int cap, int n_rows) {
  const int i = blockIdx.x * blockDim.x + threadIdx.x;
  if (i >= n_rep * n_rows) return;
  const int rep = i / n_rows, r = i - rep * n_rows;
  const RepConst &rc = rcs[rep];
  double *row = stats + ((long long)rep * cap + r) * NSTAT;
  double f[RES_NRED];
#pragma unroll
  for (int z = 0; z < RES_NRED; ++z) f[z] = row[z];
  const double gm = row[RES_RAW_GMAX];
  double s[NSTAT];
#pragma unroll
  for (int z = 0; z < NSTAT; ++z) s[z] = 0.0;
  s[ST_SUM_R] = f[17] * rc.rq;
  if (r > 0) {
    const double nc[4] = {f[0], f[1], f[2], f[3]};
    double Pc[4];
    for (int z = 0; z < 4; ++z) {
      const double C = (z >> 1) ? 1.0 : 0.0;
      Pc[z] = ((rc.rc * f[4 + z] / 5.0 - 5.0 * rc.cost * C * nc[z]) - rc.lo * nc[z]) / rc.span;
    }
    s[ST_NC_OLD] = nc[2] + nc[3];
    s[ST_N_CD] = nc[2];
    s[ST_N_DC] = nc[1];
    s[ST_NC_NEW] = nc[1] + nc[3];
    s[ST_SUM_P] = Pc[0] + Pc[1] + Pc[2] + Pc[3];
    s[ST_SUM_P_C] = Pc[2] + Pc[3];
    s[ST_SUM_P_D] = Pc[0] + Pc[1];
    s[ST_SUM_WP_P] = rc.wP * s[ST_SUM_P];
    s[ST_SUM_REW_C] = rc.wP * (Pc[1] + Pc[3]) + rc.wR * 0.5 * (nc[1] + nc[3]);
    s[ST_SUM_REW_D] = rc.wP * (Pc[0] + Pc[2]);
    s[ST_SUM_RATIO] = f[27];
    for (int z = 0; z < 6; ++z) s[ST_GROUP0 + z] = f[8 + z];
    for (int z = 0; z < 4; ++z) {
      s[ST_SUM_Q + z] = f[18 + z];
      s[ST_SUM_Q_C + z] = f[22 + z];
      s[ST_SUM_Q_D + z] = f[18 + z] - f[22 + z];
    }
    s[ST_SUM_NI] = f[26];
    s[ST_N_BEST_POS] = f[14];
    s[ST_N_BEST_2ND] = f[15];
    s[ST_GMAX] = gm;
  }
#pragma unroll
  for (int z = 0; z < NSTAT; ++z) row[z] = s[z];
}

}
```

Before: 129.0 billion.

## Store int8-mode Q-table in lane-blocked SoA layout per 128-column tile

Changes the global Q-table layout for the F32/I8 mode from per-site float4 (AoS) to a tile-blocked structure-of-arrays layout where each action component is contiguous across 32 lanes. The fast TMA kernel drops the 128B swizzle and per-lane XOR offsets, reading each Q component with conflict-free strided shared-memory accesses instead of swizzled float4/float2 loads. All other kernels (generic, lean, resident, init, import/export, digest) switch to a shared q_idx indexing helper, and allocation pads columns to the tile width. This removes swizzle address arithmetic and bank conflicts, but turns vector loads into scalar ones in the non-TMA paths and relaxes shared-memory alignment from 1024 to 128 bytes.

Result: faster. 131.6 billion (median of 6 runs) (+2.0%).

```diff
diff --git a/neighbor-aware-reinforcement-learning-fosters-cooperation-in-spatial-public-goods-games-_b200/csrc/spgg_capi.cu b/neighbor-aware-reinforcement-learning-fosters-cooperation-in-spatial-public-goods-games-_b200/csrc/spgg_capi.cu
--- a/neighbor-aware-reinforcement-learning-fosters-cooperation-in-spatial-public-goods-games-_b200/csrc/spgg_capi.cu
+++ b/neighbor-aware-reinforcement-learning-fosters-cooperation-in-spatial-public-goods-games-_b200/csrc/spgg_capi.cu
@@ -131,6 +131,7 @@
   size_t elem_Q() const { return mode == MODE_F64 ? 8 : 4; }
   size_t elem_val() const { return mode == MODE_F64 ? 8 : 4; }
   int nq() const { return params[0].algorithm == SPGG_ALGO_DOUBLE_QLEARNING ? 8 : 4; }
+  size_t q_rep_bytes() const { return (size_t)q_rep_elems(g, nq(), mode == MODE_F32_I8) * elem_Q(); }
 };
 
 static bool int8_quantum(const spgg_params_t &p, double *rq, int *gi, int *li, int *mn, int *mx) {
@@ -280,7 +281,7 @@
   return SPGG_OK;
 }
 
-static int make_map_q(CUtensorMap *map, void *base, uint64_t L, uint64_t n_rows, uint64_t n_rep) {
+static int make_map_q(CUtensorMap *map, void *base, uint64_t Lq, uint64_t n_rows, uint64_t n_rep) {
   static PFN_cuTensorMapEncodeTiled_v12000 encode = nullptr;
   if (!encode) {
     void *fn = nullptr;
@@ -289,12 +290,12 @@
     if (!fn || q != cudaDriverEntryPointSuccess) return fail(SPGG_E_CUDA, "cuTensorMapEncodeTiled not available");
     encode = (PFN_cuTensorMapEncodeTiled_v12000)fn;
   }
-  const cuuint64_t dims[4] = {128, L / 8, n_rows, n_rep};
-  const cuuint64_t strides[3] = {128, L * 16, n_rows * L * 16};
+  const cuuint64_t dims[4] = {128, Lq / 8, n_rows, n_rep};
+  const cuuint64_t strides[3] = {128, Lq * 16, n_rows * Lq * 16};
   const cuuint32_t box[4] = {128, TC / 8, (cuuint32_t)FastSmem<1>::kRowsPerWarp, 1};
   const cuuint32_t estr[4] = {1, 1, 1, 1};
   CUresult r = encode(map, CU_TENSOR_MAP_DATA_TYPE_UINT8, 4, base, dims, strides, box, estr,
-                      CU_TENSOR_MAP_INTERLEAVE_NONE, CU_TENSOR_MAP_SWIZZLE_128B,
+                      CU_TENSOR_MAP_INTERLEAVE_NONE, CU_TENSOR_MAP_SWIZZLE_NONE,
                       CU_TENSOR_MAP_L2_PROMOTION_L2_128B, CU_TENSOR_MAP_FLOAT_OOB_FILL_NONE);
   if (r != CUDA_SUCCESS) return fail(SPGG_E_CUDA, "cuTensorMapEncodeTiled (Q) failed (%d)", (int)r);
   return SPGG_OK;
@@ -502,7 +503,7 @@
   if (h->fast && (g.site_stride / ((long long)g.ctas_per_rep * FTHREADS)) > 60000) h->fast = false;
   h->spec = h->fast && getenv("SPGG_NO_SPEC") == nullptr;
 
-  const size_t nQ = (size_t)n_replicas * g.site_stride * h->nq() * h->elem_Q();
+  const size_t nQ = (size_t)n_replicas * h->q_rep_bytes();
   const size_t nR = (size_t)n_replicas * g.plane_stride * h->elem_R();
   const size_t nC = (size_t)n_replicas * g.plane_stride * h->elem_code();
   const size_t nS = (size_t)n_replicas * g.bits_stride * 4;
@@ -538,7 +539,7 @@
       if (!e) e = make_map(&fm.st_code, h->d_code[i ^ 1], (uint64_t)g.pitchB, nrows, n_replicas, (uint64_t)g.plane_stride, TC, FTR, (uint64_t)(CPAD + g.L));
       if (!e) e = make_map(&fm.st_R, h->d_R[i ^ 1], (uint64_t)g.pitchB, nrows, n_replicas, (uint64_t)g.plane_stride, TC, FTR, (uint64_t)(CPAD + g.L));
       if (!e) e = make_map(&fm.st_S, h->d_S[i ^ 1], (uint64_t)g.pitchW * 4, nrows, n_replicas, (uint64_t)g.bits_stride * 4, TC / 8, FTR);
-      if (!e) e = make_map_q(&h->qmaps[i], h->d_Qb[(i == 1 && h->spec) ? 1 : 0], (uint64_t)g.L, (uint64_t)g.rows, (uint64_t)n_replicas);
+      if (!e) e = make_map_q(&h->qmaps[i], h->d_Qb[(i == 1 && h->spec) ? 1 : 0], (uint64_t)(g.L + TC - 1) / TC * TC, (uint64_t)g.rows, (uint64_t)n_replicas);
       if (e) { free_all(h); delete h; return e; }
     }
   }
@@ -657,7 +658,7 @@
           }
           const int qsrc = k >= 0 ? h->pend_q_after[(size_t)k] : h->pend_qcur0;
           if (qsrc != h->qcur) {
-            const size_t qb = (size_t)h->g.site_stride * h->nq() * h->elem_Q();
+            const size_t qb = h->q_rep_bytes();
             CUDA_TRY(cudaMemcpy((char *)h->d_Qb[h->qcur] + (size_t)r * qb, (char *)h->d_Qb[qsrc] + (size_t)r * qb, qb,
                                 cudaMemcpyDeviceToDevice));
           }
diff --git a/neighbor-aware-reinforcement-learning-fosters-cooperation-in-spatial-public-goods-games-_b200/csrc/spgg_fast.cuh b/neighbor-aware-reinforcement-learning-fosters-cooperation-in-spatial-public-goods-games-_b200/csrc/spgg_fast.cuh
--- a/neighbor-aware-reinforcement-learning-fosters-cooperation-in-spatial-public-goods-games-_b200/csrc/spgg_fast.cuh
+++ b/neighbor-aware-reinforcement-learning-fosters-cooperation-in-spatial-public-goods-games-_b200/csrc/spgg_fast.cuh
@@ -39,8 +39,8 @@
   static constexpr int kRowsPerWarp = FTR / (FTHREADS / 32);
   static constexpr int kQBufs = 2;
   static constexpr int kQBufBytes = kRowsPerWarp * TC * 16;
-  static constexpr int kOffQ = (kOffRed + 8 * NSTAT * 8 + 1023) / 1024 * 1024;
-  static constexpr int kTotal = kOffQ + (FTHREADS / 32) * kQBufs * kQBufBytes + 1024;
+  static constexpr int kOffQ = (kOffRed + 8 * NSTAT * 8 + 127) / 128 * 128;
+  static constexpr int kTotal = kOffQ + (FTHREADS / 32) * kQBufs * kQBufBytes + 128;
 };
 
 __device__ __forceinline__ uint32_t smem_u32(const void *p) {
@@ -138,8 +138,8 @@
   const Geom &g = a.g;
   const int rep = blockIdx.x / g.ctas_per_rep, cta = blockIdx.x % g.ctas_per_rep;
 
-  extern __shared__ __align__(1024) unsigned char smem_fast[];
-  unsigned char *smem = smem_fast + ((1024u - (smem_u32(smem_fast) & 1023u)) & 1023u);
+  extern __shared__ __align__(128) unsigned char smem_fast[];
+  unsigned char *smem = smem_fast + ((128u - (smem_u32(smem_fast) & 127u)) & 127u);
   uint32_t *wC = reinterpret_cast<uint32_t *>(smem + SM::kOffC);
   float *sm_val = reinterpret_cast<float *>(smem + SM::kOffVal);
   float *sm_tab = reinterpret_cast<float *>(smem + SM::kOffTab);
@@ -170,8 +170,6 @@
     sm_ratio[i] = s_rc.ratiotab[i];
   }
   const RepConst &rc = s_rc;
-
-  float4 *Qp = reinterpret_cast<float4 *>(a.Q) + (long long)rep * g.site_stride;
 
   float inv_den = 0.f, gm_used = 0.f;
   if (upd) {
@@ -224,10 +222,6 @@
     mbar_expect_tx(&qbar[buf], SM::kQBufBytes);
     tma_load_4d_hint(sQ + buf * SM::kQBufBytes, &tm.q_ld, &qbar[buf], 0, col8, row, rep, pol);
   };
-  int qoff[4];
-#pragma unroll
-  for (int k = 0; k < 4; ++k)
-    qoff[k] = (lane >> 1) * 128 + ((((lane & 1) * 4 + k) ^ ((lane >> 1) & 7)) << 4);
   if (lane == 0 && cta < n_tiles) q_issue((tx * TC) >> 3, ty * FTR + warp * SM::kRowsPerWarp, 0);
 
   int tiles_done = 0, stage = 0;
@@ -377,7 +371,7 @@
           vl[0] = 0.f; vl[1] = sm_val[vb - 1]; vr[0] = sm_val[vb + 4]; vr[1] = 0.f;
         }
       }
-      unsigned char *qbuf = sQ + qb * SM::kQBufBytes + r2 * (TC * 16);
+      unsigned char *qsite = sQ + qb * SM::kQBufBytes + r2 * (TC * 16) + lane * 4;
       uint32_t coopW = 0, rnewW = 0;
       float qfin[4];
       int eidx[4];
@@ -390,11 +384,11 @@
         const uint32_t eoffW = ((codeW & 0x01010101u) << 3) | ((((codeW >> 1) & 0x01010101u) ^ 0x01010101u) << 2);
 #pragma unroll
         for (int k = 0; k < 4; ++k) {
-          const unsigned char *qs = qbuf + qoff[k];
-          eidx[k] = (int)__byte_perm(eoffW, 0, 0x4440 + k);
+          const unsigned char *qs = qsite + k * 128;
+          eidx[k] = (int)__byte_perm(eoffW, 0, 0x4440 + k) << 7;
           qe[k] = *reinterpret_cast<const float *>(qs + eidx[k]);
-          const float2 nrow = *reinterpret_cast<const float2 *>(qs + __byte_perm(rowoffW, 0, 0x4440 + k));
-          na[k] = nrow.x; nb_[k] = nrow.y;
+          const unsigned char *nr = qs + ((int)__byte_perm(rowoffW, 0, 0x4440 + k) << 7);
+          na[k] = *reinterpret_cast<const float *>(nr); nb_[k] = *reinterpret_cast<const float *>(nr + 512);
         }
 #pragma unroll
         for (int k = 0; k < 4; ++k) {
@@ -442,10 +436,12 @@
           }
         }
 #pragma unroll
-        for (int k = 0; k < 4; ++k) *reinterpret_cast<float *>(qbuf + qoff[k] + eidx[k]) = qfin[k];
+        for (int k = 0; k < 4; ++k) *reinterpret_cast<float *>(qsite + k * 128 + eidx[k]) = qfin[k];
 #pragma unroll
         for (int k = 0; k < 4; ++k) {
-          const float4 qn = *reinterpret_cast<const float4 *>(qbuf + qoff[k]);
+          const float *qv = reinterpret_cast<const float *>(qsite + k * 128);
+          float4 qn;
+          qn.x = qv[0]; qn.y = qv[128]; qn.z = qv[256]; qn.w = qv[384];
           const float m = ((codeW >> (8 * k + 2)) & 1u) ? 1.0f : 0.0f;
           if (lv) {
             sq0 += qn.x; sq1 += qn.y; sq2 += qn.z; sq3 += qn.w;
@@ -456,8 +452,9 @@
       if (sel) {
 #pragma unroll
         for (int k = 0; k < 4; ++k) {
-          const float2 grow = *reinterpret_cast<const float2 *>(
-              qbuf + qoff[k] + __byte_perm(rowoffW, 0, 0x4440 + k));
+          const unsigned char *gr = qsite + k * 128 + ((int)__byte_perm(rowoffW, 0, 0x4440 + k) << 7);
+          float2 grow;
+          grow.x = *reinterpret_cast<const float *>(gr); grow.y = *reinterpret_cast<const float *>(gr + 512);
           const bool explore = (w4[k] >> 8) < thr;
           const int rnd = (int)(w4[k] & 1u);
           const int greedy = (grow.y > grow.x) ? 1 : 0;
diff --git a/neighbor-aware-reinforcement-learning-fosters-cooperation-in-spatial-public-goods-games-_b200/csrc/spgg_kernels.cuh b/neighbor-aware-reinforcement-learning-fosters-cooperation-in-spatial-public-goods-games-_b200/csrc/spgg_kernels.cuh
--- a/neighbor-aware-reinforcement-learning-fosters-cooperation-in-spatial-public-goods-games-_b200/csrc/spgg_kernels.cuh
+++ b/neighbor-aware-reinforcement-learning-fosters-cooperation-in-spatial-public-goods-games-_b200/csrc/spgg_kernels.cuh
@@ -55,6 +55,17 @@
   long long bits_stride;
   long long site_stride;
 };
+
+__host__ __device__ __forceinline__ long long q_rep_elems(const Geom &g, int nq, bool lane_blocked) {
+  return lane_blocked ? (long long)g.rows * ((g.L + TC - 1) / TC * TC) * nq : g.site_stride * nq;
+}
+template <class Md>
+__device__ __forceinline__ long long q_idx(const Geom &g, int row, int col, int z, int nq) {
+  if constexpr (Md::kLaneQ)
+    return ((long long)row * ((g.L + TC - 1) / TC) + (col >> 7)) * (nq * TC) + z * TC + (col & 3) * 32 + ((col >> 2) & 31);
+  else
+    return ((long long)row * g.L + col) * nq + z;
+}
 
 #ifndef SPGG_MAX_RING
 #define SPGG_MAX_RING 16
@@ -145,14 +156,17 @@
 struct ModeF32I8 {
   typedef float Q; typedef int8_t R; typedef uint8_t Code; typedef float Val;
   static constexpr bool kFp64 = false;
+  static constexpr bool kLaneQ = true;
 };
 struct ModeF32F {
   typedef float Q; typedef float R; typedef uint8_t Code; typedef float Val;
   static constexpr bool kFp64 = false;
+  static constexpr bool kLaneQ = false;
 };
 struct ModeF64 {
   typedef double Q; typedef double R; typedef uint32_t Code; typedef double Val;
   static constexpr bool kFp64 = true;
+  static constexpr bool kLaneQ = false;
 };
 
 template <class Md>
@@ -709,7 +723,7 @@
 
   const double *vtab = a.valtab ? a.valtab + ((size_t)rep << (VALTAB_BITS + 1)) : nullptr;
   const bool dq = (a.algo == 3);
-  QT *Qp = reinterpret_cast<QT *>(a.Q) + (long long)rep * g.site_stride * (dq ? 8 : 4);
+  QT *Qp = reinterpret_cast<QT *>(a.Q) + (long long)rep * q_rep_elems(g, dq ? 8 : 4, Md::kLaneQ);
   const RT *R_in = reinterpret_cast<const RT *>(a.R_in) + (long long)rep * g.plane_stride;
   RT *R_out = reinterpret_cast<RT *>(a.R_out) + (long long)rep * g.plane_stride;
   const Code *code_in = reinterpret_cast<const Code *>(a.code_in) + (long long)rep * g.plane_stride;
@@ -793,13 +807,16 @@
           QT t1[4], t2[4];
           if (dq) {
 #pragma unroll
-            for (int z = 0; z < 4; ++z) { t1[z] = Qp[site * 8 + z]; t2[z] = Qp[site * 8 + 4 + z]; }
+            for (int z = 0; z < 4; ++z) { t1[z] = Qp[q_idx<Md>(g, i, col, z, 8)]; t2[z] = Qp[q_idx<Md>(g, i, col, 4 + z, 8)]; }
             q0_ = q_mean(t1[0], t2[0]); q1_ = q_mean(t1[1], t2[1]);
             q2_ = q_mean(t1[2], t2[2]); q3_ = q_mean(t1[3], t2[3]);
           } else if constexpr (Md::kFp64) {
             const double2 lo2 = reinterpret_cast<const double2 *>(Qp)[site * 2];
             const double2 hi2 = reinterpret_cast<const double2 *>(Qp)[site * 2 + 1];
             q0_ = lo2.x; q1_ = lo2.y; q2_ = hi2.x; q3_ = hi2.y;
+          } else if constexpr (Md::kLaneQ) {
+            q0_ = Qp[q_idx<Md>(g, i, col, 0, 4)]; q1_ = Qp[q_idx<Md>(g, i, col, 1, 4)];
+            q2_ = Qp[q_idx<Md>(g, i, col, 2, 4)]; q3_ = Qp[q_idx<Md>(g, i, col, 3, 4)];
           } else {
             const float4 v = reinterpret_cast<const float4 *>(Qp)[site];
             q0_ = v.x; q1_ = v.y; q2_ = v.z; q3_ = v.w;
@@ -966,10 +983,13 @@
           if (upd) {
             if (dq) {
 #pragma unroll
-              for (int z = 0; z < 4; ++z) { Qp[site * 8 + z] = t1[z]; Qp[site * 8 + 4 + z] = t2[z]; }
+              for (int z = 0; z < 4; ++z) { Qp[q_idx<Md>(g, i, col, z, 8)] = t1[z]; Qp[q_idx<Md>(g, i, col, 4 + z, 8)] = t2[z]; }
             } else if constexpr (Md::kFp64) {
               reinterpret_cast<double2 *>(Qp)[site * 2] = make_double2(q0_, q1_);
               reinterpret_cast<double2 *>(Qp)[site * 2 + 1] = make_double2(q2_, q3_);
+            } else if constexpr (Md::kLaneQ) {
+              Qp[q_idx<Md>(g, i, col, 0, 4)] = q0_; Qp[q_idx<Md>(g, i, col, 1, 4)] = q1_;
+              Qp[q_idx<Md>(g, i, col, 2, 4)] = q2_; Qp[q_idx<Md>(g, i, col, 3, 4)] = q3_;
             } else {
               reinterpret_cast<float4 *>(Qp)[site] = make_float4(q0_, q1_, q2_, q3_);
             }
@@ -1070,7 +1090,7 @@
                               uint32_t seed_hi, int nq) {
   typedef typename Md::Q QT;
   typedef typename Md::R RT;
-  QT *Qp = reinterpret_cast<QT *>(Q) + (long long)rep * g.site_stride * nq;
+  QT *Qp = reinterpret_cast<QT *>(Q) + (long long)rep * q_rep_elems(g, nq, Md::kLaneQ);
   RT *Rp = reinterpret_cast<RT *>(R) + (long long)rep * g.plane_stride;
   uint32_t *Sp = S + (long long)rep * g.bits_stride;
   const long long n_sites = g.site_stride;
@@ -1083,7 +1103,7 @@
 #pragma unroll
       for (int z = 0; z < 4; ++z) {
         const double uu = (double)(w[z] >> 8) * (1.0 / 16777216.0);
-        Qp[x * nq + 4 * t + z] = (QT)(-0.01 + 0.02 * uu);
+        Qp[q_idx<Md>(g, i, j, 4 * t + z, nq)] = (QT)(-0.01 + 0.02 * uu);
       }
     }
   }
@@ -1111,7 +1131,7 @@
                               unsigned long long *info, int nq) {
   typedef typename Md::Q QT;
   typedef typename Md::R RT;
-  QT *Qp = reinterpret_cast<QT *>(Qd) + (long long)rep * g.site_stride * nq;
+  QT *Qp = reinterpret_cast<QT *>(Qd) + (long long)rep * q_rep_elems(g, nq, Md::kLaneQ);
   RT *Rp = reinterpret_cast<RT *>(Rd) + (long long)rep * g.plane_stride;
   uint32_t *Sp = Sd + (long long)rep * g.bits_stride;
   const int lane = threadIdx.x & 31;
@@ -1141,8 +1161,7 @@
       } else {
         rv = (RT)r;
       }
-      const long long site = (long long)i * g.L + col;
-      for (int z = 0; z < nq; ++z) Qp[site * nq + z] = (QT)Q[src * nq + z];
+      for (int z = 0; z < nq; ++z) Qp[q_idx<Md>(g, i, col, z, nq)] = (QT)Q[src * nq + z];
     }
     const uint32_t word = __ballot_sync(0xffffffffu, valid && bit);
     const uint32_t vmask = __ballot_sync(0xffffffffu, valid);
@@ -1159,7 +1178,7 @@
                               const void *Qd, const void *Rd, const uint32_t *Sd, double rq, int nq) {
   typedef typename Md::Q QT;
   typedef typename Md::R RT;
-  const QT *Qp = reinterpret_cast<const QT *>(Qd) + (long long)rep * g.site_stride * nq;
+  const QT *Qp = reinterpret_cast<const QT *>(Qd) + (long long)rep * q_rep_elems(g, nq, Md::kLaneQ);
   const RT *Rp = reinterpret_cast<const RT *>(Rd) + (long long)rep * g.plane_stride;
   const uint32_t *Sp = Sd + (long long)rep * g.bits_stride;
   const long long n = (long long)nrows * g.L;
@@ -1173,8 +1192,7 @@
       R[e] = (sizeof(RT) == 1) ? (double)rv * rq : (double)rv;
     }
     if (Q) {
-      const long long site = (long long)i * g.L + col;
-      for (int z = 0; z < nq; ++z) Q[e * nq + z] = (double)Qp[site * nq + z];
+      for (int z = 0; z < nq; ++z) Q[e * nq + z] = (double)Qp[q_idx<Md>(g, i, col, z, nq)];
     }
   }
 }
@@ -1188,7 +1206,7 @@
                                double rq, unsigned long long *out) {
   typedef typename Md::Q QT;
   typedef typename Md::R RT;
-  const QT *Qp = reinterpret_cast<const QT *>(Qd) + (long long)rep * g.site_stride * nq;
+  const QT *Qp = reinterpret_cast<const QT *>(Qd) + (long long)rep * q_rep_elems(g, nq, Md::kLaneQ);
   const RT *Rp = reinterpret_cast<const RT *>(Rd) + (long long)rep * g.plane_stride;
   const uint32_t *Sp = Sd + (long long)rep * g.bits_stride;
   unsigned long long dS = 0, dR = 0, dQ = 0;
@@ -1204,7 +1222,7 @@
     if (sizeof(RT) == 1) rv *= rq;
     dR += hR * ((unsigned long long)__double_as_longlong(rv) + 1ull);
     for (int z = 0; z < nq; ++z) {
-      const double qv = (double)Qp[e * nq + z];
+      const double qv = (double)Qp[q_idx<Md>(g, i, col, z, nq)];
       dQ += digest_mix(key * 3 + 3 + ((unsigned long long)(z + 1) << 58)) * ((unsigned long long)__double_as_longlong(qv) + 1ull);
     }
   }
diff --git a/neighbor-aware-reinforcement-learning-fosters-cooperation-in-spatial-public-goods-games-_b200/csrc/spgg_lean.cuh b/neighbor-aware-reinforcement-learning-fosters-cooperation-in-spatial-public-goods-games-_b200/csrc/spgg_lean.cuh
--- a/neighbor-aware-reinforcement-learning-fosters-cooperation-in-spatial-public-goods-games-_b200/csrc/spgg_lean.cuh
+++ b/neighbor-aware-reinforcement-learning-fosters-cooperation-in-spatial-public-goods-games-_b200/csrc/spgg_lean.cuh
@@ -133,7 +133,7 @@
   const RepConst &rc = s_rc;
   const double *vtab = a.valtab ? a.valtab + ((size_t)rep << (VALTAB_BITS + 1)) : nullptr;
 
-  QT *Qp = reinterpret_cast<QT *>(a.Q) + (long long)rep * g.site_stride * 4;
+  QT *Qp = reinterpret_cast<QT *>(a.Q) + (long long)rep * q_rep_elems(g, 4, Md::kLaneQ);
   const RT *R_in = reinterpret_cast<const RT *>(a.R_in) + (long long)rep * g.plane_stride;
   RT *R_out = reinterpret_cast<RT *>(a.R_out) + (long long)rep * g.plane_stride;
   const Code *code_in = reinterpret_cast<const Code *>(a.code_in) + (long long)rep * g.plane_stride;
@@ -171,9 +171,9 @@
         constexpr int kLineSites = 128 / (int)(4 * sizeof(QT));
         const int lines = TC / kLineSites;
         for (int e = threadIdx.x; e < g.TR * lines; e += blockDim.x) {
-          const int rr = e / lines, cs = ncol + (e - rr * lines) * kLineSites;
+          const int rr = e / lines, ln = e - rr * lines, cs = ncol + ln * kLineSites;
           if (nrow + rr < g.rows && cs < g.L)
-            asm volatile("prefetch.global.L2 [%0];" ::"l"(Qp + ((long long)(nrow + rr) * g.L + cs) * 4));
+            asm volatile("prefetch.global.L2 [%0];" ::"l"(Qp + q_idx<Md>(g, nrow + rr, ncol, 0, 4) + ln * (128 / (int)sizeof(QT))));
         }
       }
     }
@@ -221,12 +221,15 @@
 #pragma unroll
       for (int k4 = kb; k4 < kb + SPGG_LEAN_BATCH; ++k4) {
         const bool valid = FULL || (c0 + 32 * k4 + lane < g.L);
-        const long long site = site_row + 32 * k4;
+        [[maybe_unused]] const long long site = site_row + 32 * k4;
         if (valid) {
           if constexpr (Md::kFp64) {
             const double2 lo2 = reinterpret_cast<const double2 *>(Qp)[site * 2];
             const double2 hi2 = reinterpret_cast<const double2 *>(Qp)[site * 2 + 1];
             q[k4][0] = lo2.x; q[k4][1] = lo2.y; q[k4][2] = hi2.x; q[k4][3] = hi2.y;
+          } else if constexpr (Md::kLaneQ) {
+#pragma unroll
+            for (int z = 0; z < 4; ++z) q[k4][z] = Qp[q_idx<Md>(g, i, c0 + 32 * k4 + lane, z, 4)];
           } else {
             const float4 v = reinterpret_cast<const float4 *>(Qp)[site];
             q[k4][0] = v.x; q[k4][1] = v.y; q[k4][2] = v.z; q[k4][3] = v.w;
@@ -249,7 +252,7 @@
         const int sidx = sr * SMW + sc;
         int a_new = 0;
         if (valid) {
-          const long long site = site_row + 32 * k4;
+          [[maybe_unused]] const long long site = site_row + 32 * k4;
           QT q0_ = q[k4][0], q1_ = q[k4][1], q2_ = q[k4][2], q3_ = q[k4][3];
           const RT r_old = sm_R[sidx];
           const int Ccur = sm_C[sidx];
@@ -352,6 +355,9 @@
           if constexpr (Md::kFp64) {
             reinterpret_cast<double2 *>(Qp)[site * 2] = make_double2(q0_, q1_);
             reinterpret_cast<double2 *>(Qp)[site * 2 + 1] = make_double2(q2_, q3_);
+          } else if constexpr (Md::kLaneQ) {
+            Qp[q_idx<Md>(g, i, col, 0, 4)] = q0_; Qp[q_idx<Md>(g, i, col, 1, 4)] = q1_;
+            Qp[q_idx<Md>(g, i, col, 2, 4)] = q2_; Qp[q_idx<Md>(g, i, col, 3, 4)] = q3_;
           } else {
             reinterpret_cast<float4 *>(Qp)[site] = make_float4(q0_, q1_, q2_, q3_);
           }
diff --git a/neighbor-aware-reinforcement-learning-fosters-cooperation-in-spatial-public-goods-games-_b200/csrc/spgg_resident.cuh b/neighbor-aware-reinforcement-learning-fosters-cooperation-in-spatial-public-goods-games-_b200/csrc/spgg_resident.cuh
--- a/neighbor-aware-reinforcement-learning-fosters-cooperation-in-spatial-public-goods-games-_b200/csrc/spgg_resident.cuh
+++ b/neighbor-aware-reinforcement-learning-fosters-cooperation-in-spatial-public-goods-games-_b200/csrc/spgg_resident.cuh
@@ -215,7 +215,7 @@
   }
   const RepConst &rc = s_rc;
 
-  float4 *Qg = reinterpret_cast<float4 *>(a.Q) + (long long)rep * g.site_stride;
+  float *Qg = reinterpret_cast<float *>(a.Q) + (long long)rep * q_rep_elems(g, 4, ModeF32I8::kLaneQ);
   int8_t *Rg = reinterpret_cast<int8_t *>(a.R) + (long long)rep * g.plane_stride;
   uint32_t *Sg = a.S + (long long)rep * g.bits_stride;
   {
@@ -234,12 +234,9 @@
     float *sQf = reinterpret_cast<float *>(sQ);
     for (int e = tid; e < nrow * L; e += nthr) {
       const int rr = e / L, cc = e % L;
-      const float4 v = Qg[(long long)(row_start + rr) * L + cc];
       const int o = (rr * QR + (cc >> 2)) * 4 + (cc & 3);
-      sQf[o] = v.x;
-      sQf[(q_plane * 4) + o] = v.y;
-      sQf[(q_plane * 8) + o] = v.z;
-      sQf[(q_plane * 12) + o] = v.w;
+#pragma unroll
+      for (int z = 0; z < 4; ++z) sQf[(q_plane * 4 * z) + o] = Qg[q_idx<ModeF32I8>(g, row_start + rr, cc, z, 4)];
     }
   }
   const size_t img_stride = (size_t)6 * nb;
@@ -702,8 +699,8 @@
     for (int e = tid; e < nrow * L; e += nthr) {
       const int rr = e / L, cc = e % L;
       const int o = (rr * QR + (cc >> 2)) * 4 + (cc & 3);
-      Qg[(long long)(row_start + rr) * L + cc] =
-          make_float4(sQf[o], sQf[(q_plane * 4) + o], sQf[(q_plane * 8) + o], sQf[(q_plane * 12) + o]);
+#pragma unroll
+      for (int z = 0; z < 4; ++z) Qg[q_idx<ModeF32I8>(g, row_start + rr, cc, z, 4)] = sQf[(q_plane * 4 * z) + o];
       store_cell<int8_t>(Rg, g, row_start + rr, cc, (int8_t)Rc[(rr + 2) * pitch + RG + cc]);
     }
     const int nW = (L + 31) >> 5;
```
